# hmetaxa/MVTopicModel

Hardware: AMD Instinct MI355X
Metric: gibbs_tokens_per_sec (higher is better)
Workload: dtype f64

## Files before the change

### include/mvhdp.h

```cpp
#ifndef MVHDP_H
#define MVHDP_H

#include <stddef.h>
#include <stdint.h>

#ifdef __cplusplus
extern "C" {
#endif

#define MVHDP_MAX_MODALITIES 8
#define MVHDP_MAX_TOPICS     2048
#define MVHDP_UNASSIGNED_TOPIC (-1)

typedef enum {
    MVHDP_OK = 0,
    MVHDP_ERR_INVALID_ARG   = -1,
    MVHDP_ERR_STATE         = -2,
    MVHDP_ERR_HIP           = -3,
    MVHDP_ERR_NO_DEVICE     = -4,
    MVHDP_ERR_NEGATIVE_COUNT= -5,
    MVHDP_ERR_UNSUPPORTED   = -6
} mvhdp_status;

typedef struct mvhdp_ctx* mvhdp_handle;
// ... 26 lines not shown
    int64_t word_ftree_mass_cnt;
    int64_t oov_skipped;
    int64_t aborted_docs;
    int64_t exact_fallbacks;
    int32_t activated_topic;
    int32_t activated_modality;
    int64_t activation_key;
    double  sweep_kernel_ms;
    double  total_ms;
    int32_t activations;
    int32_t reserved;
} mvhdp_sweep_stats;

#define MVHDP_ACT_DOC_SHIFT   34
#define MVHDP_ACT_VIEW_SHIFT  31
#define MVHDP_ACT_POS_SHIFT   11
#define MVHDP_ACT_TOPIC_MASK  0x7ffLL
#define MVHDP_ACT_VIEW_MASK   0x7LL
#define MVHDP_ACT_KEY(doc, view, pos, topic) \
    (((int64_t)(doc) << MVHDP_ACT_DOC_SHIFT) | ((int64_t)(view) << MVHDP_ACT_VIEW_SHIFT) | ((int64_t)(pos) << MVHDP_ACT_POS_SHIFT) | (int64_t)(topic))
#define MVHDP_ACT_KEY_TOPIC(key) ((int32_t)((key) & MVHDP_ACT_TOPIC_MASK))
#define MVHDP_ACT_KEY_VIEW(key)  ((int32_t)(((key) >> MVHDP_ACT_VIEW_SHIFT) & MVHDP_ACT_VIEW_MASK))
#define MVHDP_ACT_KEY_NONE INT64_MAX

typedef struct {
    double* tok_dbg[MVHDP_MAX_MODALITIES];
    int32_t n_trace;
    const int64_t* trace_doc;
    const int32_t* trace_view;
    const int32_t* trace_pos;
    double* trace_out;
} mvhdp_debug;

#define MVHDP_SWEEP_REUSE_TREES 0x1u
#define MVHDP_SWEEP_NO_APPLY    0x2u
#define MVHDP_SWEEP_EXACT_CHAIN 0x4u
#define MVHDP_SWEEP_GENERIC_KERNEL 0x8u
#define MVHDP_SWEEP_FROZEN      0x10u

#define MVHDP_SWEEP_LIVE        0x20u
#define MVHDP_SWEEP_LIVE_SEGMENTS(n) (((uint32_t)(n) & 0xffu) << 16)

#define MVHDP_SWEEP_SEGMENT_APPLY 0x40u

#define MVHDP_SWEEP_SEGMENT_OVERLAP 0x80u

#define MVHDP_SWEEP_ONLY_SEGMENT(s) ((((uint32_t)(s) + 1u) & 0xffu) << 24)

#define MVHDP_SWEEP_SHARD_BIRTHS 0x200u

typedef enum {
    MVHDP_BUF_COUNTS = 0,
    MVHDP_BUF_DELTA  = 1,
    MVHDP_BUF_BIRTH_KEYS = 2
} mvhdp_buffer;

int mvhdp_create(const mvhdp_config* cfg, mvhdp_handle* out);
int mvhdp_destroy(mvhdp_handle h);
const char* mvhdp_last_error(mvhdp_handle h);
const char* mvhdp_version(void);

int mvhdp_set_corpus(mvhdp_handle h, int32_t m, int64_t num_docs,
                     const int64_t* doc_off , const int32_t* tokens );
int mvhdp_set_assignments(mvhdp_handle h, int32_t m, const int32_t* z );
int mvhdp_set_view_presence(mvhdp_handle h, int32_t m, const uint8_t* present );
int mvhdp_get_assignments(mvhdp_handle h, int32_t m, int32_t* z );

int mvhdp_set_hyper(mvhdp_handle h, const mvhdp_hyper* hy);
int mvhdp_get_alpha(mvhdp_handle h, double* alpha , uint8_t* inactive );
int mvhdp_build_counts(mvhdp_handle h);
int mvhdp_build_trees(mvhdp_handle h);
int mvhdp_build_inference_trees(mvhdp_handle h);
int mvhdp_init_assignments_from_trees(mvhdp_handle h, uint64_t seed);
int mvhdp_get_counts(mvhdp_handle h, int32_t m, int32_t* n_wk , int32_t* n_k );
int mvhdp_set_counts(mvhdp_handle h, int32_t m, const int32_t* n_wk, const int32_t* n_k);
int mvhdp_get_tree(mvhdp_handle h, int32_t m, int32_t type, double* tree );
int mvhdp_get_doc_topic_hist(mvhdp_handle h, int32_t m, int32_t* hist , int32_t hist_len,
                             int32_t* doc_len_counts , int32_t len_len);

int mvhdp_get_count_histogram(mvhdp_handle h, int32_t m, int32_t* hist, int32_t len);
int mvhdp_view_overlap_sums(mvhdp_handle h, double* sums );
int mvhdp_model_log_likelihood(mvhdp_handle h, double* log_likelihood );
int mvhdp_gamma_doc_statistics(mvhdp_handle h, int32_t m, double gamma_m, uint64_t seed, uint32_t round, double* qs, double* qw);
int mvhdp_dp_table_statistics(mvhdp_handle h, int32_t m, const int32_t* hist , int32_t hist_len, const double* conc ,
                              uint64_t seed, uint32_t round, double* mk , uint8_t* active );
int mvhdp_antoniak_draws(mvhdp_handle h, int32_t n, const int32_t* items , const double* conc , uint64_t seed, uint32_t round, int32_t* tables );
int mvhdp_doc_topic_proportions(mvhdp_handle h, const double* view_weights , int64_t d0, int64_t d1, double* out );

#define MVHDP_DIAG_MAX_TOP_WORDS 64
#define MVHDP_DIAG_PROPORTIONS   7
#define MVHDP_DIAG_TOKENS             0
#define MVHDP_DIAG_DOCUMENT_ENTROPY   1
#define MVHDP_DIAG_WORD_LENGTH        2
#define MVHDP_DIAG_COHERENCE          3
#define MVHDP_DIAG_NORM_DISCR_WEIGHT  4
#define MVHDP_DIAG_DISCR_WEIGHT       5
#define MVHDP_DIAG_UNIFORM_DIST       6
#define MVHDP_DIAG_CORPUS_DIST        7
#define MVHDP_DIAG_EFF_NUM_WORDS      8
#define MVHDP_DIAG_TOKEN_DOC_DIFF     9
#define MVHDP_DIAG_RANK_1_DOCS       10
#define MVHDP_DIAG_ALLOCATION_RATIO  11
#define MVHDP_DIAG_ALLOCATION_COUNT  12
#define MVHDP_DIAG_ROWS              13
typedef struct {
    int32_t num_top_words;
    const int32_t* word_length;
// ... 162 lines not shown
```

### mvtopicmodel_amd/csrc/mvhdp_api.hip

```cpp
#include "mvhdp_ctx.h"

static thread_local std::string g_create_error;

static std::mutex g_reg_mutex;
static std::set<mvhdp_ctx*>* g_live = nullptr;
static bool g_exiting = false, g_atexit_registered = false;
static void release_device_resources(mvhdp_ctx* h);

static void mvhdp_at_exit()
{
    std::lock_guard<std::mutex> lk(g_reg_mutex);
    g_exiting = true;
    if (g_live) for (mvhdp_ctx* h : *g_live) release_device_resources(h);
}

static void register_handle(mvhdp_ctx* h)
{
    std::lock_guard<std::mutex> lk(g_reg_mutex);
    if (!g_live) g_live = new std::set<mvhdp_ctx*>();
    g_live->insert(h);
    if (!g_atexit_registered) { atexit(mvhdp_at_exit); g_atexit_registered = true; }
}

bool mvhdp_is_live(mvhdp_ctx* h)
{
    std::lock_guard<std::mutex> lk(g_reg_mutex);
    return g_live && g_live->count(h) != 0;
}

static void read_environment(mvhdp_ctx* h)
{
    if (const char* f = getenv("MVHDP_FORCE_RMAX")) { const int v = atoi(f); if (v == 1 || v == 2 || v == 4 || v == 8 || v == 16 || v == 32) h->tu.force_primary = v; }
    if (const char* f = getenv("MVHDP_NARROW")) h->tu.narrow = atoi(f) != 0 ? -1 : 0;
    if (const char* f = getenv("MVHDP_SINGLE_STREAM")) h->tu.single_stream = atoi(f) != 0;
    if (const char* f = getenv("MVHDP_SIDE_PRIORITY")) h->side_priority = atoi(f);
    if (const char* f = getenv("MVHDP_LIVE16")) h->tu.live16 = atoi(f);
    if (const char* f = getenv("MVHDP_LIVE_OVERLAP")) h->tu.live_overlap = atoi(f);
    if (const char* f = getenv("MVHDP_LIVE_ROWS")) h->tu.live_rows = atoi(f);
    if (const char* f = getenv("MVHDP_LIVE_ROWS_THETA")) h->tu.live_rows_theta = atof(f);
    if (const char* f = getenv("MVHDP_COEF_LDS_KB")) h->tu.coef_lds_max_bytes = std::max(0, std::min(64, atoi(f))) * 1024;
    if (const char* f = getenv("MVHDP_LIVE_ROWS_SEGMENTS")) h->tu.live_rows_segments = std::max(1, std::min(255, atoi(f)));
    if (const char* f = getenv("MVHDP_WIDEST_ON_MAIN")) h->tu.widest_on_main = atoi(f) != 0;
    if (const char* f = getenv("MVHDP_NARROW_WIDE")) h->tu.narrow_wide = atoi(f) != 0;
    if (const char* f = getenv("MVHDP_LIVE_TREE_EVERY")) h->live_tree_every = std::max(1, atoi(f));
    if (const char* f = getenv("MVHDP_GATE_PCT")) { const int v = atoi(f); if (v >= 5 && v <= 95) h->gate_pct = v; }
    if (const char* f = getenv("MVHDP_FOUR_ROUND_ON_C")) h->tu.four_round_on_c = atoi(f);
    if (const char* f = getenv("MVHDP_DELTA16")) h->tu.delta16 = atoi(f) != 0;
    if (const char* f = getenv("MVHDP_FORK_DELAY_US")) h->tu.fork_delay_us = std::max(0, std::min(1000, atoi(f)));
    if (const char* f = getenv("MVHDP_FORCE_MODE")) { if (!strcmp(f, "serial")) h->tu.single_stream = 1; }
    if (const char* f = getenv("MVHDP_PRIMARY_MIN_SHARE")) { const double v = atof(f); if (v > 0.0 && v <= 1.0) h->tu.primary_min_share = v; }
    if (const char* t = getenv("MVHDP_WALK_THETA")) {
        int m = 0;
        for (const char* q = t; *q && m < MVHDP_MAXM; m++) {
            h->tu.walk_theta[m] = atof(q);
            while (*q && *q != ',') q++;
            if (*q == ',') q++;
        }
        for (; m < MVHDP_MAXM; m++) h->tu.walk_theta[m] = 0.0;
        h->tu.walk_fixed = 1;
    }
    h->dbg_env = getenv("MVHDP_DEBUG") != nullptr;
}

extern "C" const char* mvhdp_version(void) { return "mvhdp 0.1 (gfx950)"; }

extern "C" const char* mvhdp_last_error(mvhdp_handle h) { return (h && mvhdp_is_live(h)) ? h->err.c_str() : g_create_error.c_str(); }

extern "C" int mvhdp_create(const mvhdp_config* cfg, mvhdp_handle* out)
{
    if (!cfg || !out) { g_create_error = "null argument"; return MVHDP_ERR_INVALID_ARG; }
    *out = nullptr;
    const int K = cfg->num_topics, M = cfg->num_modalities;
    if (K < 1 || K > MVHDP_MAX_TOPICS || M < 1 || M > MVHDP_MAX_MODALITIES) {
        g_create_error = "num_topics must be in [1,2048] and num_modalities in [1,8]";
        return MVHDP_ERR_INVALID_ARG;
    }
    for (int m = 0; m < M; m++) if (cfg->num_types[m] < 1) { g_create_error = "num_types[m] must be >= 1"; return MVHDP_ERR_INVALID_ARG; }
    for (int m = 0; m < M; m++) if (cfg->num_types[m] >= (1 << 29)) { g_create_error = "num_types[m] must be below 2^29"; return MVHDP_ERR_INVALID_ARG; }
    if (cfg->doc_id_base < 0 || cfg->doc_id_base >= (1LL << 29)) { g_create_error = "doc_id_base out of range"; return MVHDP_ERR_INVALID_ARG; }
    int ndev = 0;
    if (hipGetDeviceCount(&ndev) != hipSuccess || ndev <= 0 || cfg->device < 0 || cfg->device >= ndev) {
        g_create_error = "no usable HIP device (the sweep has no CPU fallback)";
        return MVHDP_ERR_NO_DEVICE;
    }
    hipDeviceProp_t prop;
    if (hipGetDeviceProperties(&prop, cfg->device) != hipSuccess) { g_create_error = "hipGetDeviceProperties failed"; return MVHDP_ERR_HIP; }
    if (strncmp(prop.gcnArchName, "gfx950", 6) != 0) {
        g_create_error = std::string("device is ") + prop.gcnArchName + ", this library is built for gfx950 only";
        return MVHDP_ERR_NO_DEVICE;
    }
    mvhdp_ctx* h = new mvhdp_ctx();
    register_handle(h);
    h->cfg = *cfg;
    h->device = cfg->device;
    h->num_cus = prop.multiProcessorCount;
    h->max_lds = 160 * 1024;
// ... 10 lines not shown
    CREATE_HIP(hipStreamCreateWithFlags(&h->stream, hipStreamNonBlocking));
    h->own_stream = true;
    for (auto& e : h->ev) CREATE_HIP(hipEventCreate(&e));
    const int64_t nrows = mm.rowbase[M];
    const size_t cbytes = (size_t)(nrows * K + (int64_t)M * K + MVHDP_TAIL_WORDS) * sizeof(int32_t);
    CREATE_HIP(hipMalloc(&mm.counts, cbytes));
    CREATE_HIP(hipMalloc(&mm.delta, cbytes));
    CREATE_HIP(hipMemset(mm.counts, 0, cbytes));
    CREATE_HIP(hipMalloc(&mm.counts16, (size_t)nrows * K * sizeof(uint16_t) + 64));
    CREATE_HIP(hipMemset(mm.counts16, 0, (size_t)nrows * K * sizeof(uint16_t)));
    CREATE_HIP(hipMalloc(&mm.delta16, (size_t)(nrows * K + 2) * sizeof(uint16_t)));
    CREATE_HIP(hipMemsetD16(mm.delta16, (unsigned short)0x8000, (size_t)(nrows * K + 2)));
    CREATE_HIP(hipMalloc(&mm.heavy, (size_t)nrows));
    CREATE_HIP(hipMemset(mm.heavy, 1, (size_t)nrows));
    CREATE_HIP(hipMemset(mm.delta, 0, cbytes));
    CREATE_HIP(hipMalloc(&mm.trees, (size_t)nrows * 2 * K * sizeof(double)));
    CREATE_HIP(hipMalloc(&mm.root, (size_t)nrows * sizeof(double)));
    CREATE_HIP(hipMalloc(&mm.mass0, (size_t)nrows * sizeof(float)));
    CREATE_HIP(hipMemset(mm.mass0, 0, (size_t)nrows * sizeof(float)));
    CREATE_HIP(hipMalloc(&mm.coef, (size_t)M * (((K + 7) & ~7) + K + 8) * sizeof(float)));
    {
        const int nlev = (K > 1) ? (32 - __builtin_clz((unsigned)(K - 1))) : 0;
        mm.dt_f = nlev ? ((nlev - 1) % 3) + 1 : 0;
        mm.dt_nbd = 1; mm.dt_base[0] = 0; mm.dt_depth[0] = 0;
        int nblk = 1;
        for (int dep = mm.dt_f; nlev && dep < nlev; dep += 3) {
            mm.dt_base[mm.dt_nbd] = nblk; mm.dt_depth[mm.dt_nbd] = dep; mm.dt_nbd++;
            nblk += 1 << dep;
        }
        mm.dt_nblk = nblk;
        CREATE_HIP(hipMalloc(&mm.dtab, (size_t)nrows * nblk * 8 * sizeof(double)));
    }
    CREATE_HIP(hipMalloc(&h->d_alpha, (size_t)M * (K + 1) * sizeof(double)));
    CREATE_HIP(hipMalloc(&h->d_inactive, (size_t)K));
    CREATE_HIP(hipMemset(h->d_inactive, 0, (size_t)K));
    CREATE_HIP(hipMalloc(&h->d_births, (size_t)(2 + 2 * K) * sizeof(int32_t)));
    CREATE_HIP(hipMemset(h->d_births, 0, (size_t)(2 + 2 * K) * sizeof(int32_t)));
    CREATE_HIP(hipMalloc(&h->d_birth_keys, (size_t)K * sizeof(long long)));
    CREATE_HIP(hipMalloc(&h->d_birth_table, (size_t)K * sizeof(long long)));
    {
        const std::vector<long long> none((size_t)K, LLONG_MAX);
        CREATE_HIP(hipMemcpy(h->d_birth_table, none.data(), (size_t)K * sizeof(long long), hipMemcpyHostToDevice));
    }
    CREATE_HIP(hipMalloc(&h->d_ctl, CTL_WORDS * sizeof(unsigned long long)));
    CREATE_HIP(hipMemset(h->d_ctl, 0, CTL_WORDS * sizeof(unsigned long long)));
    h->d_stats = h->d_ctl;
    h->d_act_key = (long long*)(h->d_ctl + ST_COUNT);
    h->d_ovf_meta = (unsigned int*)(h->d_ctl + ST_COUNT + 1);
    h->d_doc_counter = h->d_ctl + ST_COUNT + 1 + META_WORDS64;
    CREATE_HIP(hipHostMalloc((void**)&h->h_ctl, CTL_WORDS * sizeof(unsigned long long), hipHostMallocDefault));
    for (int c = 0; c < MVHDP_N_CLASSES; c++)
        for (int f = 0; f < 3; f++) { h->regs.regs[c][f] = mvhdp_sweep_kernel_regs(c, f); h->regs.regs_mix[c][f] = mvhdp_sweep_kernel_regs(c, f ? f : 1, true); }
    read_environment(h);
    mm.alpha = h->d_alpha;
    mm.inactive = h->d_inactive;
    h->h_alpha.assign((size_t)M * (K + 1), 0.0);
    h->h_inactive.assign((size_t)K, 0);
    h->wt.init_defaults(K);
    h->wt_mix.init_defaults(K);
    *out = h;
    return MVHDP_OK;
}

static void release_device_resources(mvhdp_ctx* h)
{
    if (h->device_released) return;
    h->device_released = true;
    hipSetDevice(h->device);
    if (h->stream) hipStreamSynchronize(h->stream);
    auto fr = [](auto*& p) { if (p) { hipFree((void*)p); p = nullptr; } };
    for (int m = 0; m < MVHDP_MAXM; m++) { fr(h->d_doc_off[m]); fr(h->d_tok[m]); fr(h->d_z[m]); fr(h->d_carry[m]); fr(h->d_present[m]); }
    fr(h->mm.counts); fr(h->mm.delta16); fr(h->mm.counts16); fr(h->mm.heavy); fr(h->mm.delta); fr(h->mm.trees); fr(h->mm.root); fr(h->mm.coef); fr(h->mm.mass0); fr(h->d_births); fr(h->d_birth_keys); fr(h->d_birth_table); fr(h->mm.dtab); fr(h->mm.p);
    fr(h->d_alpha); fr(h->d_inactive); fr(h->d_ctl);
    fr(h->d_mix); fr(h->d_mix32); h->mm.mix = nullptr; h->mm.mix32 = nullptr; h->mix_lambda = 0.0;
    mvhdp_emb_free(h);
    if (h->h_ctl) { hipHostFree(h->h_ctl); h->h_ctl = nullptr; }
    h->d_stats = nullptr; h->d_act_key = nullptr; h->d_doc_counter = nullptr; h->d_ovf_meta = nullptr;
    fr(h->d_doc_order); fr(h->d_lists); fr(h->d_nslots); fr(h->d_stats_many); fr(h->d_heavy_list); fr(h->d_heavy_ctl);
    if (h->ev_rf_go) { hipEventDestroy(h->ev_rf_go); h->ev_rf_go = nullptr; }
    if (h->ev_rf_done) { hipEventDestroy(h->ev_rf_done); h->ev_rf_done = nullptr; }
    if (h->rf_stream) { hipStreamDestroy(h->rf_stream); h->rf_stream = nullptr; }
    fr(h->ov.counts2); fr(h->ov.counts16_2); fr(h->ov.dtab2); fr(h->ov.root2); fr(h->ov.trees2); fr(h->ov.delta2); fr(h->ov.delta3); fr(h->ov.ctl2); fr(h->ov.lists2);
    for (auto& e : h->ov.ev_seg) if (e) { hipEventDestroy(e); e = nullptr; }
    if (h->ov.ev_start) { hipEventDestroy(h->ov.ev_start); h->ov.ev_start = nullptr; }
    if (h->ov.x1) { hipStreamDestroy(h->ov.x1); h->ov.x1 = nullptr; }
    if (h->ov.xa) { hipStreamDestroy(h->ov.xa); h->ov.xa = nullptr; }
    for (auto& e : h->ev_many) if (e) { hipEventDestroy(e); e = nullptr; }
    for (auto& e : h->ev) if (e) { hipEventDestroy(e); e = nullptr; }
    if (h->ev_fork) { hipEventDestroy(h->ev_fork); h->ev_fork = nullptr; }
    for (auto& e : h->ev_join) if (e) { hipEventDestroy(e); e = nullptr; }
    for (auto& st : h->side) if (st) { hipStreamDestroy(st); st = nullptr; }
    if (h->own_stream && h->stream) hipStreamDestroy(h->stream);
    h->stream = nullptr;
}

extern "C" int mvhdp_destroy(mvhdp_handle h)
{
    if (!h) return MVHDP_OK;
    bool exiting;
    {
        std::lock_guard<std::mutex> lk(g_reg_mutex);
        if (!g_live || g_live->erase(h) == 0) return MVHDP_ERR_INVALID_ARG;
        exiting = g_exiting;
    }
    if (!exiting) release_device_resources(h);
    delete h;
    return MVHDP_OK;
}

extern "C" int mvhdp_set_stream(mvhdp_handle h, void* hip_stream)
{
    CHECK_H(h);
    HIPC(h, hipSetDevice(h->device));
    HIPC(h, hipStreamSynchronize(h->stream));
    if (h->own_stream) { hipStreamDestroy(h->stream); h->own_stream = false; }
    if (hip_stream) h->stream = (hipStream_t)hip_stream;
    else { HIPC(h, hipStreamCreateWithFlags(&h->stream, hipStreamNonBlocking)); h->own_stream = true; }
    return MVHDP_OK;
}

extern "C" int mvhdp_synchronize(mvhdp_handle h)
{
    CHECK_H(h);
    HIPC(h, hipSetDevice(h->device));
    HIPC(h, hipStreamSynchronize(h->stream));
// ... 497 lines not shown
    if (activated_topic >= 0) {
        h->have_trees = false;
        int rc = apply_activation(h, activated_topic, activated_modality);
        if (rc) return rc;
    }
    if (neg) FAIL(h, MVHDP_ERR_NEGATIVE_COUNT, "a topic count went below zero (UPD:202-215)");
    return MVHDP_OK;
}

extern "C" int mvhdp_trees_current(mvhdp_handle h)
{
    CHECK_H(h);
    return h->have_trees ? 1 : 0;
}

static int ensure_slot_counts(mvhdp_ctx* h)
{
    MvModel& mm = h->mm;
    if (mm.D > 0 && !h->d_nslots) {
        HIPC(h, hipMalloc(&h->d_nslots, (size_t)mm.D * sizeof(uint16_t)));
        mm.nslots = h->d_nslots;
        h->nslots_valid = false;
    }
    if (h->nslots_valid) return MVHDP_OK;
    unsigned long long hist[MVHDP_HIST_BINS + MVHDP_ENT_BINS] = {0};
    HIPC(h, hipMemsetAsync(h->d_ovf_meta, 0, META_BYTES, h->stream));
    HIPC(h, mvhdp_launch_slot_hist(mm, (unsigned long long*)h->d_ovf_meta + META_HIST, h->stream));
    HIPC(h, hipMemcpyAsync(hist, (unsigned long long*)h->d_ovf_meta + META_HIST, sizeof hist, hipMemcpyDeviceToHost, h->stream));
    HIPC(h, hipStreamSynchronize(h->stream));
    std::copy(hist, hist + MVHDP_HIST_BINS, h->last_hist);
    std::copy(hist + MVHDP_HIST_BINS, hist + MVHDP_HIST_BINS + MVHDP_ENT_BINS, h->last_ent);
    h->nslots_valid = true;
    return MVHDP_OK;
}

static void fill_plan_in(mvhdp_ctx* h, uint32_t flags, bool debug, bool batch, PlanIn& in)
{
    const MvModel& mm = h->mm;
    in.K = mm.K; in.M = mm.M; in.D = mm.D;
    in.mdt = compute_max_doc_tokens(h);
    in.have_order = h->d_doc_order != nullptr && !h->tokens_desc.empty();
    for (int c = 0; c < 5; c++)
        in.n_longer[c] = in.have_order ? (int64_t)(std::upper_bound(h->tokens_desc.begin(), h->tokens_desc.end(), (int64_t)64 << c, std::greater<int64_t>()) - h->tokens_desc.begin()) : mm.D;
    std::copy(h->last_hist, h->last_hist + MVHDP_HIST_BINS, in.tok_hist);
    std::copy(h->last_ent, h->last_ent + MVHDP_ENT_BINS, in.ent_hist);
    in.flags = flags; in.debug = debug; in.batch = batch;
    in.trees_current = h->have_trees;
    in.unassigned = false;
    for (int m = 0; m < mm.M; m++) in.unassigned = in.unassigned || h->unassigned[m];
    in.first_inactive = mm.first_inactive;
    in.vectors_mix = mm.mix != nullptr && !(flags & MVHDP_SWEEP_FROZEN);
    in.num_cus = h->num_cus; in.max_lds = h->max_lds;
    in.regs = h->regs;
}

static int alloc_debug(mvhdp_ctx* h, const mvhdp_debug* dbg, DebugBufs& db)
{
    const int K = h->mm.K, M = h->mm.M;
    hipStream_t s = h->stream;
    for (int m = 0; m < M; m++) {
        if (dbg->tok_dbg[m] && h->N[m] > 0) {
            void* p = nullptr;
            hipError_t e = hipMalloc(&p, (size_t)h->N[m] * 4 * sizeof(double));
            if (e != hipSuccess) { db.release(); HIPC(h, e); }
            db.to_free.push_back(p);
            hipMemsetAsync(p, 0, (size_t)h->N[m] * 4 * sizeof(double), s);
            db.tok_dbg[m] = (double*)p;
        }
    }
    if (dbg->n_trace > 0) {
        void *a = nullptr, *b = nullptr, *c = nullptr, *o = nullptr;
        const size_t n = (size_t)dbg->n_trace;
        if (hipMalloc(&a, n * 8) != hipSuccess || hipMalloc(&b, n * 4) != hipSuccess ||
            hipMalloc(&c, n * 4) != hipSuccess || hipMalloc(&o, n * (K + 1) * 8) != hipSuccess) {
            for (void* q : {a, b, c, o}) if (q) hipFree(q);
            db.release(); FAIL(h, MVHDP_ERR_HIP, "debug trace allocation failed");
        }
        db.to_free.push_back(a); db.to_free.push_back(b); db.to_free.push_back(c); db.to_free.push_back(o);
        hipMemcpyAsync(a, dbg->trace_doc, n * 8, hipMemcpyHostToDevice, s);
        hipMemcpyAsync(b, dbg->trace_view, n * 4, hipMemcpyHostToDevice, s);
        hipMemcpyAsync(c, dbg->trace_pos, n * 4, hipMemcpyHostToDevice, s);
        hipMemsetAsync(o, 0, n * (K + 1) * 8, s);
        db.n_trace = dbg->n_trace;
        db.trace_doc = (const int64_t*)a; db.trace_view = (const int32_t*)b; db.trace_pos = (const int32_t*)c;
        db.trace_out = (double*)o;
    }
    return MVHDP_OK;
}

struct SegCtl {
    unsigned int* class_counts;
    unsigned long long* qheads;
    int32_t* lists;
};

static hipError_t launch_segment_kernels(mvhdp_ctx* h, const SweepPlan& p, const MvModel& mk_in, const SweepLaunch& sl, int seg, hipStream_t s,
                                         const SegCtl& ctl, unsigned long long* d_stats)
{
    const MvModel& mm = h->mm;
    MvModel mk = mk_in;
    if (p.frozen) { mk.mix = nullptr; mk.mix32 = nullptr; }
    const int nseg = p.nseg;
    hipError_t e = hipSuccess;
    auto step = [&](hipError_t r) { if (e == hipSuccess) e = r; };
    auto share = [&](int64_t P) -> int64_t { return P > seg ? (P - seg + nseg - 1) / nseg : 0; };
    const int64_t n_seg = share(mm.D);
// ... 412 lines not shown
}

static void learn_from_sweep(mvhdp_ctx* h, const SweepPlan& p, const unsigned long long* hs, const unsigned long long* meta_hist, double kernel_ms, bool comparable)
{
    const MvModel& mm = h->mm;
    bool any_walk = false;
    for (int c = 0; c < MVHDP_N_CLASSES; c++) any_walk = any_walk || (p.cls[c].used && p.cls[c].walk);
    WalkTuner& wt = walk_tuner_of(h, p.flags);
    if (any_walk) wt.measured(mm.M, p.nseg, hs + ST_VIEW_BASE);
    if (mm.D > 0 && p.only_seg >= 0) {
        if (meta_hist[MVHDP_HIST_BINS + MVHDP_N_CLASSES] != 0) h->nslots_valid = false;
    } else if (mm.D > 0) {
        std::copy(meta_hist, meta_hist + MVHDP_HIST_BINS, h->last_hist);
        std::copy(meta_hist + MVHDP_HIST_BINS, meta_hist + MVHDP_HIST_BINS + MVHDP_ENT_BINS, h->last_ent);
        h->nslots_valid = h->last_ent[MVHDP_N_CLASSES] == 0;
    }
    if (h->dbg_env) {
        fprintf(stderr, "[mvhdp] walk threshold %.2f (base %.2f, phase %d, dir %+d, group %d); tree branch %.4f of tokens, walked on demand %.4f; per view tree share:",
                (double)wt.walk_probe_i / MVHDP_WALK_BINS, (double)wt.walk_i / MVHDP_WALK_BINS, wt.walk_phase, wt.walk_dir, wt.walk_cls,
                (double)hs[ST_TREE] / std::max<double>(1.0, (double)hs[ST_TOKENS]), (double)hs[ST_ONDEMAND] / std::max<double>(1.0, (double)hs[ST_TOKENS]));
        for (int m = 0; m < mm.M; m++) {
            const double n = std::max<double>(1.0, (double)hs[ST_VIEW_BASE + m * MVHDP_VIEW_STATS]);
            fprintf(stderr, " %.3f", hs[ST_VIEW_BASE + m * MVHDP_VIEW_STATS + 1] / n);
        }
        fprintf(stderr, "\n");
        if (hs[ST_T_TOTAL])
            fprintf(stderr, "[mvhdp] wave cycles: queue %.1f%% prologue %.1f%% view setup %.1f%% chunk head %.1f%% tokens %.1f%% chunk end %.1f%% | %.0f cycles per token per wave\n",
                    100.0 * hs[ST_T_QUEUE] / hs[ST_T_TOTAL], 100.0 * hs[ST_T_PROLOGUE] / hs[ST_T_TOTAL], 100.0 * hs[ST_T_VIEW] / hs[ST_T_TOTAL],
                    100.0 * hs[ST_T_CHUNK_HEAD] / hs[ST_T_TOTAL], 100.0 * hs[ST_T_TOKENS] / hs[ST_T_TOTAL], 100.0 * hs[ST_T_CHUNK_END] / hs[ST_T_TOTAL],
                    (double)hs[ST_T_TOTAL] / std::max<double>(1.0, (double)hs[ST_TOKENS]));
        if (hs[ST_T_ROWS])
            fprintf(stderr, "[mvhdp] live rows: %.0f cycles per tree-branch token, %.0f of them until the row is there (%.1f%% of the waves' time; %llu such tokens)\n",
                    (double)hs[ST_T_ROWS] / std::max<double>(1.0, (double)hs[ST_ONDEMAND]), (double)hs[ST_T_ROWS_WAIT] / std::max<double>(1.0, (double)hs[ST_ONDEMAND]),
                    100.0 * hs[ST_T_ROWS] / hs[ST_T_TOTAL], hs[ST_ONDEMAND]);
        if (hs[ST_N_WAVES])
            fprintf(stderr, "[mvhdp] cycles per token in a wave's first / second / later entities: %.0f / %.0f / %.0f (tokens %llu / %llu / %llu); per wave: block init %.0f cycles, wait + flush at the end %.0f, whole wave %.0f\n",
                    (double)hs[ST_T_ENT0] / std::max<double>(1.0, (double)hs[ST_N_ENT0]), (double)hs[ST_T_ENT1] / std::max<double>(1.0, (double)hs[ST_N_ENT1]),
                    (double)hs[ST_T_ENT2] / std::max<double>(1.0, (double)hs[ST_N_ENT2]), hs[ST_N_ENT0], hs[ST_N_ENT1], hs[ST_N_ENT2],
                    (double)hs[ST_T_INIT] / hs[ST_N_WAVES], (double)hs[ST_T_FLUSH] / hs[ST_N_WAVES], (double)hs[ST_T_TOTAL] / hs[ST_N_WAVES]);
    }
    const double tokens = (double)hs[ST_TOKENS];
    wt.observe(comparable && tokens > 0, p.walk_cfg, mm.M, tokens > 0 ? kernel_ms * 1e6 / tokens : 0.0);
}

static void debug_print_plan(const mvhdp_ctx* h, const SweepPlan& p, uint32_t sweep_idx)
{
    double tot = 0, b1 = 0, b2 = 0;
    for (int b = 0; b < MVHDP_HIST_BINS; b++) { tot += (double)h->last_hist[b]; if (b < 1) b1 += (double)h->last_hist[b]; if (b < 2) b2 += (double)h->last_hist[b]; }
    fprintf(stderr, "[mvhdp] sweep %u: %s primary class %d, routed prefix %lld, S_cap %d, %d segment(s); tokens in lists <=64: %.4f <=128: %.4f; kernels:",
            sweep_idx, p.fast ? "register-resident" : "generic", p.pc, (long long)p.H, p.S_cap, p.nseg, b1 / std::max(1.0, tot), b2 / std::max(1.0, tot));
    for (int c = 0; c < MVHDP_N_CLASSES; c++)
        if (p.cls[c].used)
            fprintf(stderr, " [class %d %s grid %d wpb %d lds %zu stream %d%s%s theta0 %.2f ents %llu]", c, p.cls[c].fast ? "fast" : "generic", p.cls[c].grid, p.cls[c].wpb, p.cls[c].lds,
                    p.cls[c].stream, p.cls[c].walk ? " walk" : "", p.cls[c].narrow ? " narrow" : "", p.cls[c].theta[0], (unsigned long long)h->last_ent[c]);
    fprintf(stderr, "\n");
}

static int sweep_preconditions(mvhdp_ctx* h, uint32_t flags)
{
    if ((flags & MVHDP_SWEEP_SHARD_BIRTHS) && (!(flags & MVHDP_SWEEP_LIVE) || (flags & MVHDP_SWEEP_FROZEN) || (flags >> 24) != 0))
        FAIL(h, MVHDP_ERR_INVALID_ARG, "sweep: SHARD_BIRTHS goes with LIVE, not with FROZEN or ONLY_SEGMENT");
    int rc = require_corpus(h); if (rc) return rc;
    if (!h->have_hyper) FAIL(h, MVHDP_ERR_STATE, "sweep before set_hyper");
    if (!h->have_counts) FAIL(h, MVHDP_ERR_STATE, "sweep before build_counts/set_counts");
    if ((flags & (MVHDP_SWEEP_REUSE_TREES | MVHDP_SWEEP_FROZEN)) && !h->have_trees) FAIL(h, MVHDP_ERR_STATE, "REUSE_TREES / FROZEN without trees");
    if (h->rows_applied >= 0) FAIL(h, MVHDP_ERR_STATE, "sweep: an mvhdp_apply_delta_begin bracket is open (call mvhdp_apply_delta_end)");
    if (h->delta_pending && !(flags & MVHDP_SWEEP_FROZEN))
        FAIL(h, MVHDP_ERR_STATE, "sweep: the previous NO_APPLY sweep's deltas have not been applied (mvhdp_apply_delta)");
    if (h->counts_stale && !(flags & MVHDP_SWEEP_FROZEN))
        FAIL(h, MVHDP_ERR_STATE, "sweep: the assignments were replaced after the counts were built (call mvhdp_build_counts, mvhdp_set_counts or mvhdp_counts_written first)");
    return MVHDP_OK;
}

static int set_generic_lds(mvhdp_ctx* h, const SweepPlan& p)
{
    size_t lds = 0;
    for (int c = 0; c < MVHDP_N_CLASSES; c++) if (p.cls[c].used && !p.cls[c].fast) lds = std::max(lds, p.cls[c].lds);
    if (lds > 65536 && lds > h->lds_attr_set) { HIPC(h, mvhdp_sweep_set_max_lds(lds)); h->lds_attr_set = lds; }
    return MVHDP_OK;
}

int mvhdp_sweep_begin(mvhdp_ctx* h, uint32_t sweep_idx, uint64_t seed, uint32_t flags, const double* p_override, const mvhdp_debug* dbg, PendingSweep& ps)
{
    int rc = sweep_preconditions(h, flags); if (rc) return rc;
    HIPC(h, hipSetDevice(h->device));
    hipStream_t s = h->stream;
    rc = ensure_slot_counts(h); if (rc) return rc;
    ps.flags = flags; ps.dbg = dbg; ps.debug = dbg != nullptr; ps.oc = SweepOutcome();
    PlanIn in; fill_plan_in(h, flags, ps.debug, false, in);
    plan_sweep(in, h->tu, walk_tuner_of(h, flags), ps.p);
    if (ps.p.err) FAIL(h, ps.p.err, ps.p.msg);
    rc = set_generic_lds(h, ps.p); if (rc) return rc;
    if (h->dbg_env) debug_print_plan(h, ps.p, sweep_idx);
    if (ps.debug) { rc = alloc_debug(h, dbg, ps.db); if (rc) return rc; }
    HIPC(h, hipEventRecord(h->ev[0], s));
    ps.births = sweep_births(ps.p, flags, h->mm);
    rc = enqueue_sweep(h, ps.p, sweep_idx, seed, p_override, ps.debug ? &ps.db : nullptr, h->d_stats, h->ev[1], h->ev[2], ps.oc);
    if (rc) { ps.db.release(); return rc; }
    if ((flags & MVHDP_SWEEP_NO_APPLY) && !ps.p.frozen) {
        hipError_t e = mvhdp_launch_birth_table(ps.births ? h->d_births : nullptr, h->d_birth_keys, h->d_act_key, h->mm.K, h->d_birth_table, s);
        if (e != hipSuccess) { ps.db.release(); HIPC(h, e); }
    }
    hipError_t e = hipMemcpyAsync(h->h_ctl, h->d_ctl, (ST_COUNT + 1 + META_WORDS64) * sizeof(unsigned long long), hipMemcpyDeviceToHost, s);
    if (e != hipSuccess) { ps.db.release(); HIPC(h, e); }
    ps.open = true;
    return MVHDP_OK;
}
// ... 159 lines not shown
    return ret;
}

extern "C" int mvhdp_get_tuning(mvhdp_handle h, mvhdp_tuning* t)
{
    CHECK_H(h);
    if (!t) FAIL(h, MVHDP_ERR_INVALID_ARG, "get_tuning: null");
    memset(t, 0, sizeof *t);
    t->force_primary = h->tu.force_primary; t->narrow = h->tu.narrow; t->walk_fixed = h->tu.walk_fixed;
    t->single_stream = h->tu.single_stream; t->primary_min_share = h->tu.primary_min_share; t->live16 = h->tu.live16;
    t->single_wave = h->tu.single_wave; t->live_overlap = h->tu.live_overlap; t->live_rows = h->tu.live_rows;
    for (int m = 0; m < MVHDP_MAX_MODALITIES; m++) { t->walk_theta[m] = h->tu.walk_theta[m]; t->tree_branch_share[m] = h->wt.walk_f[m]; }
    for (int g = 0; g < WALK_GROUPS; g++) t->learnt_walk_step[g] = g == h->wt.walk_cls ? h->wt.walk_i : h->wt.walk_i_by[g];
    t->learnt_walk_step[3] = -1;
    return MVHDP_OK;
}

extern "C" int mvhdp_set_tuning(mvhdp_handle h, const mvhdp_tuning* t)
{
    CHECK_H(h);
    if (!t) FAIL(h, MVHDP_ERR_INVALID_ARG, "set_tuning: null");
    const int fp = t->force_primary;
    if (!(fp == 0 || fp == 1 || fp == 2 || fp == 4 || fp == 8 || fp == 16 || fp == 32)) FAIL(h, MVHDP_ERR_INVALID_ARG, "set_tuning: force_primary must be 0, 1, 2, 4, 8, 16 or 32");
    if (t->primary_min_share < 0.0 || t->primary_min_share > 1.0) FAIL(h, MVHDP_ERR_INVALID_ARG, "set_tuning: primary_min_share outside [0, 1]");
    for (int g = 0; g < WALK_GROUPS; g++) if (t->learnt_walk_step[g] < -1 || t->learnt_walk_step[g] > MVHDP_WALK_BINS) FAIL(h, MVHDP_ERR_INVALID_ARG, "set_tuning: learnt_walk_step outside [-1, 20]");
    h->tu.force_primary = fp; h->tu.narrow = t->narrow; h->tu.walk_fixed = t->walk_fixed ? 1 : 0;
    h->tu.single_stream = t->single_stream ? 1 : 0;
    h->tu.live16 = t->live16 < 0 ? -1 : (t->live16 ? 1 : 0);
    h->tu.single_wave = t->single_wave ? 1 : 0;
    h->tu.live_overlap = t->live_overlap < 0 ? -1 : (t->live_overlap ? 1 : 0);
    h->tu.live_rows = t->live_rows < 0 ? -1 : (t->live_rows ? 1 : 0);
    h->tu.primary_min_share = t->primary_min_share > 0.0 ? t->primary_min_share : 0.10;
    for (int m = 0; m < MVHDP_MAX_MODALITIES; m++) h->tu.walk_theta[m] = t->walk_theta[m];
    if (t->learnt_walk_step[0] >= 0 || t->learnt_walk_step[1] >= 0 || t->learnt_walk_step[2] >= 0) h->wt.restore(t->learnt_walk_step, t->tree_branch_share, h->mm.M);
    return MVHDP_OK;
}

extern "C" int mvhdp_plan_probe(const mvhdp_plan_input* pi, const mvhdp_tuning* t, mvhdp_plan_output* po)
{
    if (!pi || !po) return MVHDP_ERR_INVALID_ARG;
    PlanIn in;
    in.K = pi->num_topics; in.M = pi->num_modalities; in.D = pi->num_entities; in.mdt = pi->max_entity_tokens;
    if (in.K < 1 || in.K > MVHDP_MAX_TOPICS || in.M < 1 || in.M > MVHDP_MAX_MODALITIES || in.D < 0) return MVHDP_ERR_INVALID_ARG;
    in.have_order = true;
    for (int c = 0; c < 5; c++) in.n_longer[c] = pi->entities_longer_than[c];
    for (int b = 0; b < MVHDP_HIST_BINS; b++) in.tok_hist[b] = pi->tokens_by_list_rounds[b];
    for (int b = 0; b < MVHDP_ENT_BINS; b++) in.ent_hist[b] = pi->entities_by_class[b];
    in.flags = pi->flags; in.debug = pi->debug != 0; in.batch = pi->batch != 0; in.trees_current = pi->trees_current != 0;
    in.first_inactive = pi->inactive_topics ? 0 : -1;
    in.num_cus = pi->num_cus > 0 ? pi->num_cus : 256;
    for (int c = 0; c < MVHDP_N_CLASSES; c++) for (int f = 0; f < 3; f++) in.regs.regs[c][f] = pi->kernel_registers[c][f];
    for (int c = 0; c < MVHDP_N_CLASSES; c++) for (int f = 0; f < 3; f++) in.regs.regs_mix[c][f] = pi->kernel_registers_mix[c][f] > 0 ? pi->kernel_registers_mix[c][f] : pi->kernel_registers[c][f];
    in.vectors_mix = pi->vectors_mix != 0 && !(pi->flags & MVHDP_SWEEP_FROZEN);
    PlanTuning tu;
    WalkTuner wt;
    wt.init_defaults(in.K);
    if (t) {
        tu.force_primary = t->force_primary; tu.narrow = t->narrow; tu.walk_fixed = t->walk_fixed; tu.single_stream = t->single_stream;
        tu.live16 = t->live16; tu.single_wave = t->single_wave ? 1 : 0; tu.live_overlap = t->live_overlap; tu.live_rows = t->live_rows;
        if (t->primary_min_share > 0) tu.primary_min_share = t->primary_min_share;
        for (int m = 0; m < MVHDP_MAX_MODALITIES; m++) tu.walk_theta[m] = t->walk_theta[m];
        if (t->learnt_walk_step[0] >= 0 || t->learnt_walk_step[1] >= 0 || t->learnt_walk_step[2] >= 0) wt.restore(t->learnt_walk_step, t->tree_branch_share, in.M);
    }
    SweepPlan p;
    plan_sweep(in, tu, wt, p);
    memset(po, 0, sizeof *po);
    po->status = p.err;
    if (p.err) return MVHDP_OK;
    po->segments = p.nseg; po->primary_class = p.pc; po->routed_prefix = p.H; po->register_resident = p.fast ? 1 : 0;
    po->need_full_trees = p.need_full ? 1 : 0; po->dominant_class = p.dominant;
    for (int c = 0; c < MVHDP_N_CLASSES; c++) {
        po->class_used[c] = p.cls[c].used ? 1 : 0; po->class_map[c] = p.class_map[c];
        po->class_stream[c] = p.cls[c].stream; po->class_grid[c] = p.cls[c].grid; po->class_lds_bytes[c] = (int64_t)p.cls[c].lds;
        po->class_walk[c] = p.cls[c].walk; po->class_narrow[c] = p.cls[c].narrow; po->class_register_resident[c] = p.cls[c].fast ? 1 : 0;
        po->class_theta0[c] = p.cls[c].theta[0];
    }
    po->delta16 = p.delta16 ? 1 : 0;
    po->live_rows = p.live_rows ? 1 : 0;
    return MVHDP_OK;
}

extern "C" int mvhdp_tuner_probe(int32_t num_modalities, const double* tree_branch_share, const double* u1_hist, const double* ns_by_step ,
                                 int32_t n_sweeps, int32_t group, int32_t* steps_out )
{
    if (!tree_branch_share || !ns_by_step || !steps_out || num_modalities < 1 || num_modalities > MVHDP_MAX_MODALITIES || n_sweeps < 0) return MVHDP_ERR_INVALID_ARG;
    WalkTuner wt;
    if (group < 0 || group >= WALK_GROUPS) return MVHDP_ERR_INVALID_ARG;
    for (int m = 0; m < num_modalities; m++) wt.walk_f[m] = tree_branch_share[m];
    for (int b = 0; b < MVHDP_WALK_BINS; b++) wt.walk_hist[b] = u1_hist ? u1_hist[b] : 0.0;
    for (int i = 0; i < n_sweeps; i++) {
        double theta[WALK_GROUPS][MVHDP_MAXM]; bool measure;
        wt.propose(group, num_modalities, theta, &measure);
        steps_out[i] = wt.walk_probe_i;
        wt.observe(true, 1, num_modalities, ns_by_step[std::max(0, std::min(MVHDP_WALK_BINS, wt.walk_probe_i))]);
    }
    return MVHDP_OK;
}

extern "C" int mvhdp_get_view_weights(mvhdp_handle h, double* p)
{
    CHECK_H(h);
    MvModel& mm = h->mm;
    if (!p) FAIL(h, MVHDP_ERR_INVALID_ARG, "get_view_weights: null");
    if (mm.M == 1) { for (int64_t d = 0; d < mm.D; d++) p[d] = 1.0; return MVHDP_OK; }
    if (!mm.p) FAIL(h, MVHDP_ERR_STATE, "get_view_weights before the first sweep");
    HIPC(h, hipSetDevice(h->device));
    HIPC(h, hipStreamSynchronize(h->stream));
    HIPC(h, hipMemcpy(p, mm.p, (size_t)mm.D * mm.M * mm.M * sizeof(double), hipMemcpyDeviceToHost));
    return MVHDP_OK;
}

extern "C" int mvhdp_device_buffer(mvhdp_handle h, mvhdp_buffer which, void** dev_ptr, size_t* bytes)
{
    CHECK_H(h);
    if (!dev_ptr || !bytes) FAIL(h, MVHDP_ERR_INVALID_ARG, "device_buffer: null");
    size_t b = (size_t)counts_len(h) * sizeof(int32_t);
    if (which == MVHDP_BUF_COUNTS) { *dev_ptr = h->mm.counts; *bytes = b; return MVHDP_OK; }
    if (which == MVHDP_BUF_DELTA) { *dev_ptr = h->mm.delta; *bytes = b; return MVHDP_OK; }
    if (which == MVHDP_BUF_BIRTH_KEYS) { *dev_ptr = h->d_birth_table; *bytes = (size_t)h->mm.K * sizeof(long long); return MVHDP_OK; }
    FAIL(h, MVHDP_ERR_INVALID_ARG, "device_buffer: unknown buffer");
}

extern "C" int mvhdp_counts_written(mvhdp_handle h)
{
    CHECK_H(h);
    h->have_counts = true; h->have_trees = false; h->counts_stale = false;
    return MVHDP_OK;
}

static double log_gamma_stirling_host(double z)
{
    const double HALF_LOG_TWO_PI = std::log(6.283185307179586) / 2.0;
    int shift = 0;
    while (z < 2.0) { z = z + 1; shift++; }
    double result = HALF_LOG_TWO_PI + (z - 0.5) * std::log(z) - z + 1 / (12.0 * z) - 1 / (360.0 * z * z * z)
                    + 1 / (1260.0 * z * z * z * z * z);
    while (shift > 0) { shift--; z = z - 1; result = result - std::log(z); }
    return result;
}

extern "C" int mvhdp_get_count_histogram(mvhdp_handle h, int32_t m, int32_t* hist, int32_t len)
{
    CHECK_H(h);
    MvModel& mm = h->mm;
    if (m < 0 || m >= mm.M || !hist || len < 1) FAIL(h, MVHDP_ERR_INVALID_ARG, "get_count_histogram: bad argument");
    if (!h->have_counts) FAIL(h, MVHDP_ERR_STATE, "get_count_histogram before build_counts/set_counts");
    HIPC(h, hipSetDevice(h->device));
    int32_t* d = nullptr;
    HIPC(h, hipMalloc(&d, (size_t)len * sizeof(int32_t)));
    hipError_t e = mvhdp_launch_count_hist(mm, m, d, len, h->stream);
    if (e == hipSuccess) e = hipMemcpyAsync(hist, d, (size_t)len * sizeof(int32_t), hipMemcpyDeviceToHost, h->stream);
    if (e == hipSuccess) e = hipStreamSynchronize(h->stream);
    hipFree(d);
    HIPC(h, e);
    return MVHDP_OK;
}

int mvhdp_view_overlap_accumulate(mvhdp_ctx* h, double* acc)
{
    MvModel& mm = h->mm;
    int rc = require_corpus(h); if (rc) return rc;
    const int M = mm.M;
    if (mm.D == 0) return MVHDP_OK;
    HIPC(h, hipSetDevice(h->device));
    double* d = nullptr;
    const size_t n = (size_t)M * M * mm.D;
    HIPC(h, hipMalloc(&d, n * sizeof(double)));
    std::vector<double> host(n);
    hipError_t e = mvhdp_launch_view_overlap(mm, d, h->stream);
    if (e == hipSuccess) e = hipMemcpyAsync(host.data(), d, n * sizeof(double), hipMemcpyDeviceToHost, h->stream);
    if (e == hipSuccess) e = hipStreamSynchronize(h->stream);
    hipFree(d);
    HIPC(h, e);
// ... 206 lines not shown
```

### mvtopicmodel_amd/csrc/mvhdp_device.h

```cpp
#pragma once
#include <hip/hip_runtime.h>
#include <stdint.h>

#define MVHDP_MAXM 8
#define MVHDP_WALK_BINS 20
#define MVHDP_VIEW_STATS (2 + MVHDP_WALK_BINS)

struct MvModel {
    int32_t K, M;
    int32_t V[MVHDP_MAXM];
    int64_t rowbase[MVHDP_MAXM + 1];
    int64_t D;
    int64_t doc_id_base;
    const int64_t* doc_off[MVHDP_MAXM];
    const int32_t* tok[MVHDP_MAXM];
    int32_t* z[MVHDP_MAXM];
    const uint8_t* present[MVHDP_MAXM];
    uint16_t* nslots;
    int32_t* counts;
    uint16_t* delta16;
    uint16_t* counts16;
    uint8_t* heavy;
    int32_t* delta;
    double* trees;
    double* root;
    float* coef;
    float* mass0;
    double* dtab;
    int32_t dt_nblk, dt_nbd, dt_f;
    int32_t dt_base[6], dt_depth[6];
    const double* alpha;
    const uint8_t* inactive;
    double alpha_sum[MVHDP_MAXM], beta[MVHDP_MAXM], beta_sum[MVHDP_MAXM], gamma[MVHDP_MAXM];
    double p_a[MVHDP_MAXM][MVHDP_MAXM], p_b[MVHDP_MAXM][MVHDP_MAXM];
    double* p;
    int32_t first_inactive;
    const double* mix;
    const float* mix32;
    double oml;
};

#define MVHDP_SL_STRICT_LIVE 0x8000u
#define MVHDP_ROW_HEAVY 1
#define MVHDP_ROW_BIG 2

struct SweepLaunch {
    uint32_t sweep_idx;
    uint32_t seed_lo, seed_hi;
    uint32_t flags;
    int32_t  S_cap;
    int32_t  waves_per_block;
    uint32_t block_shared_bytes;
    int32_t  nk_global;
    uint32_t wave_bytes;
    unsigned long long* stats;
    long long* act_key;
    int32_t* births;
    long long* birth_keys;
    unsigned long long* doc_counter;
    const int32_t* q_list;
    const unsigned int* q_list_count;
    const int32_t* q_order;
    int64_t q_order_start, q_order_count, q_order_stride;
    double walk_theta[MVHDP_MAXM];
    int32_t walk;
    int32_t narrow;
    int32_t delta16;
    int32_t live16;
    int32_t live_rows;
    int32_t coef_lds;
    unsigned long long* slot_hist;
    double* tok_dbg[MVHDP_MAXM];
    int32_t n_trace;
    const int64_t* trace_doc; const int32_t* trace_view; const int32_t* trace_pos;
    double* trace_out;
};

enum {
    ST_TOKENS = 0, ST_CHANGED, ST_NEW, ST_DOC, ST_TREE, ST_OOV, ST_ABORT, ST_FALLBACK, ST_NEGATIVE, ST_MISCLASS, ST_ONDEMAND,
    ST_VIEW_BASE, ST_VIEW_LAST = ST_VIEW_BASE + MVHDP_VIEW_STATS * MVHDP_MAXM - 1,
    ST_T_QUEUE, ST_T_PROLOGUE, ST_T_VIEW, ST_T_CHUNK_HEAD, ST_T_TOKENS, ST_T_CHUNK_END, ST_T_TOTAL,
    ST_T_ENT0, ST_T_ENT1, ST_T_ENT2, ST_N_ENT0, ST_N_ENT1, ST_N_ENT2, ST_T_INIT, ST_T_FLUSH, ST_N_WAVES, ST_T_ROWS, ST_T_ROWS_WAIT,
    ST_COUNT
};

size_t mvhdp_sweep_wave_bytes(int M, int S_cap);

hipError_t mvhdp_launch_build_counts(const MvModel& mm, const int64_t* n_tokens_per_view, hipStream_t s);
hipError_t mvhdp_launch_build_trees(const MvModel& mm, bool inference_leaves, bool write_full, hipStream_t s, bool beside_samplers = false);
hipError_t mvhdp_launch_build_trees_rows(const MvModel& mm, bool inference_leaves, bool write_full, int64_t row_begin, int64_t row_end,
                                         bool apply_first, unsigned long long* negatives, hipStream_t s);
hipError_t mvhdp_launch_build_trees_from_mirror(const MvModel& mm, bool write_full, hipStream_t s, bool beside_samplers = false);
hipError_t mvhdp_launch_widen_mirror(const MvModel& mm, hipStream_t s);
hipError_t mvhdp_launch_live_rows_prepare(const MvModel& mm, bool from_mirror, bool with_heavy_trees, int32_t* heavy_list, unsigned int* heavy_ctl, int heavy_cap, int batch_cells, hipStream_t s);
hipError_t mvhdp_launch_heavy_refresh(const MvModel& mm, const int32_t* heavy_list, const unsigned int* ctl, int heavy_cap, int blocks, hipStream_t s);
hipError_t mvhdp_launch_set_u32(unsigned int* p, unsigned int v, hipStream_t s);
hipError_t mvhdp_launch_apply_nk(const MvModel& mm, unsigned long long* negatives, hipStream_t s);
// ... 119 lines not shown
```

### mvtopicmodel_amd/csrc/mvhdp_group.hip

```cpp
#include "mvhdp_ctx.h"

#include <dlfcn.h>
#include <rccl/rccl.h>

#include <map>

namespace {

struct Rccl {
    void* lib = nullptr;
    std::string path, why;
    ncclResult_t (*GetVersion)(int*) = nullptr;
    ncclResult_t (*GetUniqueId)(ncclUniqueId*) = nullptr;
    ncclResult_t (*CommInitRank)(ncclComm_t*, int, ncclUniqueId, int) = nullptr;
    ncclResult_t (*CommInitAll)(ncclComm_t*, int, const int*) = nullptr;
    ncclResult_t (*CommDestroy)(ncclComm_t) = nullptr;
    ncclResult_t (*AllReduce)(const void*, void*, size_t, ncclDataType_t, ncclRedOp_t, ncclComm_t, hipStream_t) = nullptr;
    ncclResult_t (*GroupStart)() = nullptr;
    ncclResult_t (*GroupEnd)() = nullptr;
    const char* (*GetErrorString)(ncclResult_t) = nullptr;
};

std::mutex g_rccl_mutex;
Rccl g_rccl;
// ... 18 lines not shown
        if (g_rccl.lib) break;
        void* l = dlopen(n.c_str(), RTLD_NOW | RTLD_LOCAL);
        if (!l) { errs += std::string(dlerror() ? dlerror() : "?") + "; "; continue; }
        g_rccl.lib = l; g_rccl.path = n;
    }
    if (!g_rccl.lib) { g_rccl.why = "RCCL could not be opened: " + errs; return nullptr; }
#define SYM(field, name) do { *(void**)(&g_rccl.field) = dlsym(g_rccl.lib, name); \
        if (!g_rccl.field) { g_rccl.why = std::string("RCCL lacks ") + name; dlclose(g_rccl.lib); g_rccl.lib = nullptr; return nullptr; } } while (0)
    SYM(GetVersion, "ncclGetVersion"); SYM(GetUniqueId, "ncclGetUniqueId"); SYM(CommInitRank, "ncclCommInitRank");
    SYM(CommInitAll, "ncclCommInitAll"); SYM(CommDestroy, "ncclCommDestroy"); SYM(AllReduce, "ncclAllReduce");
    SYM(GroupStart, "ncclGroupStart"); SYM(GroupEnd, "ncclGroupEnd"); SYM(GetErrorString, "ncclGetErrorString");
#undef SYM
    return &g_rccl;
}

__global__ __launch_bounds__(256) void add_into_kernel(int32_t* __restrict__ dst, const int32_t* __restrict__ src, int64_t n)
{
    const int64_t stride = (int64_t)gridDim.x * blockDim.x;
    for (int64_t i = (int64_t)blockIdx.x * blockDim.x + threadIdx.x; i < n; i += stride) dst[i] += src[i];
}

hipError_t launch_add_into(int32_t* dst, const int32_t* src, int64_t n, hipStream_t s)
{
    int grid = (int)std::min<int64_t>((n + 255) / 256, 8192);
    if (grid < 1) grid = 1;
    hipLaunchKernelGGL(add_into_kernel, dim3(grid), dim3(256), 0, s, dst, src, n);
    return hipGetLastError();
}

__global__ void set_word_kernel(int32_t* p, int32_t v) { *p = v; }

__global__ __launch_bounds__(256) void min_births_kernel(long long* __restrict__ dst, const long long* __restrict__ src, int K, int first)
{
    const int k = blockIdx.x * blockDim.x + threadIdx.x;
    if (k >= K) return;
    const long long v = src ? src[k] : 0x7fffffffffffffffLL;
    dst[k] = first ? v : (v < dst[k] ? v : dst[k]);
}

hipError_t launch_min_births(long long* dst, const long long* src, int K, bool first, hipStream_t s)
{
    hipLaunchKernelGGL(min_births_kernel, dim3((K + 255) / 256), dim3(256), 0, s, dst, src, K, first ? 1 : 0);
    return hipGetLastError();
}

__global__ __launch_bounds__(256) void pack_rows_kernel(const int32_t* __restrict__ delta, const uint8_t* __restrict__ heavy, const int64_t* __restrict__ woff,
                                                        int32_t* __restrict__ xp, int64_t r0, int64_t r1, int K)
{
    const int lane = threadIdx.x & 63;
    const int64_t wstride = (int64_t)gridDim.x * (blockDim.x >> 6);
    for (int64_t row = r0 + (int64_t)blockIdx.x * (blockDim.x >> 6) + (threadIdx.x >> 6); row < r1; row += wstride) {
        const int32_t* d = delta + row * K;
        int32_t* o = xp + woff[row];
        if (heavy[row] == 0) {
            const int nw = (K + 1) >> 1;
            for (int j = lane; j < nw; j += 64) { const int a = d[2 * j], b = (2 * j + 1 < K) ? d[2 * j + 1] : 0; o[j] = a + b * 65536; }
        } else for (int k = lane; k < K; k += 64) o[k] = d[k];
    }
}

__global__ __launch_bounds__(256) void unpack_rows_kernel(int32_t* __restrict__ delta, const uint8_t* __restrict__ heavy, const int64_t* __restrict__ woff,
                                                          const int32_t* __restrict__ xp, int64_t r0, int64_t r1, int K)
{
    const int lane = threadIdx.x & 63;
    const int64_t wstride = (int64_t)gridDim.x * (blockDim.x >> 6);
    for (int64_t row = r0 + (int64_t)blockIdx.x * (blockDim.x >> 6) + (threadIdx.x >> 6); row < r1; row += wstride) {
        int32_t* d = delta + row * K;
        const int32_t* o = xp + woff[row];
        if (heavy[row] == 0) {
            const int nw = (K + 1) >> 1;
            for (int j = lane; j < nw; j += 64) {
                const int w = o[j];
                const int a = (int)(short)(w & 0xffff);
                d[2 * j] = a;
                if (2 * j + 1 < K) d[2 * j + 1] = (w - a) >> 16;
            }
        } else for (int k = lane; k < K; k += 64) d[k] = o[k];
    }
}

__global__ __launch_bounds__(256) void add_remote_kernel(int32_t* __restrict__ counts, const int32_t* __restrict__ sum, const int32_t* __restrict__ own, int64_t n)
{
    const int64_t stride = (int64_t)gridDim.x * blockDim.x;
    for (int64_t i = (int64_t)blockIdx.x * blockDim.x + threadIdx.x; i < n; i += stride) { const int d = sum[i] - own[i]; if (d) counts[i] += d; }
}

struct DeviceGuard {
    int prev = -1;
    DeviceGuard() { if (hipGetDevice(&prev) != hipSuccess) prev = -1; }
    ~DeviceGuard() { if (prev >= 0) hipSetDevice(prev); }
};

}

enum { XSCRATCH_BYTES = 1 << 20 };

struct mvhdp_group_ctx {
    std::vector<mvhdp_ctx*> members;
    std::vector<int> leader_of;
    std::vector<int> leaders;
    std::vector<ncclComm_t> comms;
    std::vector<hipEvent_t> ev_swept;
    std::vector<hipEvent_t> ev_reduced;
    std::vector<long long*> d_key;
    std::vector<long long*> d_btab;
    hipEvent_t ev_x0 = nullptr, ev_x1 = nullptr;
    int nranks = 1, rank0 = 0;
    bool multi_process = false;
    bool rccl_used = false;
    int rccl_version = 0;
    int chunks = 4;
    double last_exchange_ms = 0.0;
    long long sweeps = 0;
    std::vector<int32_t*> xbuf, sbuf;
    std::vector<hipStream_t> comm;
    std::vector<hipEvent_t> ev_xfer;
    bool async_pending = false;
    bool abort_raised = false;
    std::vector<int> by_entity;
    bool pack_on = false;
    bool pack_ready = false;
    bool pack_allowed = true;
// ... 268 lines not shown
        if (li == i) continue;
        mvhdp_ctx *h = g->members[i], *L = g->members[li];
        x.hip(hipSetDevice(L->device), "hipSetDevice");
        x.hip(hipStreamWaitEvent(L->stream, g->ev_swept[i], 0), "hipStreamWaitEvent");
        x.hip(launch_add_into(counts ? L->mm.counts : L->mm.delta, counts ? h->mm.counts : h->mm.delta, counts_len_of(L), L->stream), "add_into_kernel");
    }
    return x.rc;
}

static int allreduce_range(mvhdp_group_ctx* g, bool counts, int64_t e0, int64_t e1)
{
    if (e1 <= e0 || g->comms.empty()) return MVHDP_OK;
    XErr x{g};
    leaders_allreduce(g, x, (size_t)(e1 - e0), ncclInt32, ncclSum, "ncclAllReduce", [&](size_t l) {
        mvhdp_ctx* L = g->members[g->leaders[l]];
        return (counts ? L->mm.counts : L->mm.delta) + e0;
    });
    return x.rc;
}

static int fan_out_range(mvhdp_group_ctx* g, bool counts, int64_t e0, int64_t e1)
{
    if (e1 <= e0 || g->members.size() == g->leaders.size()) return MVHDP_OK;
    XErr x{g};
    for (size_t l = 0; l < g->leaders.size(); l++) {
        mvhdp_ctx* L = g->members[g->leaders[l]];
        x.hip(hipSetDevice(L->device), "hipSetDevice");
        x.hip(hipEventRecord(g->ev_reduced[l], L->stream), "hipEventRecord");
        for (size_t i = 0; i < g->members.size(); i++) {
            if (g->leader_of[i] != g->leaders[l] || (int)i == g->leaders[l]) continue;
            mvhdp_ctx* h = g->members[i];
            x.hip(hipStreamWaitEvent(h->stream, g->ev_reduced[l], 0), "hipStreamWaitEvent");
            const int32_t* src = (counts ? L->mm.counts : L->mm.delta) + e0;
            int32_t* dst = (counts ? h->mm.counts : h->mm.delta) + e0;
            x.hip(hipMemcpyAsync(dst, src, (size_t)(e1 - e0) * sizeof(int32_t), hipMemcpyDeviceToDevice, h->stream), "hipMemcpyAsync");
            x.hip(hipEventRecord(g->ev_swept[i], h->stream), "hipEventRecord");
            x.hip(hipStreamWaitEvent(L->stream, g->ev_swept[i], 0), "hipStreamWaitEvent");
        }
    }
    return x.rc;
}

static int pack_prepare(mvhdp_group_ctx* g)
{
    if (g->pack_ready || !g->pack_allowed) return MVHDP_OK;
    for (mvhdp_ctx* h : g->members) for (int m = 0; m < h->mm.M; m++) if (h->unassigned[m]) return MVHDP_OK;
    mvhdp_ctx* L0 = g->members[g->leaders[0]];
    const int64_t rows = L0->mm.rowbase[L0->mm.M];
    const int K = L0->mm.K;
    if (rows <= 0) return MVHDP_OK;
    std::vector<uint8_t> cls((size_t)rows);
    GHIP(g, hipSetDevice(L0->device));
    GHIP(g, hipMemcpy(cls.data(), L0->mm.heavy, (size_t)rows, hipMemcpyDeviceToHost));
    g->woff.assign((size_t)rows + 1, 0);
    for (int64_t r = 0; r < rows; r++) g->woff[(size_t)r + 1] = g->woff[(size_t)r] + (cls[(size_t)r] == 0 ? (K + 1) / 2 : K);
    if (g->d_woff.empty()) { g->d_woff.assign(g->leaders.size(), nullptr); g->d_cls.assign(g->leaders.size(), nullptr); g->xpack.assign(g->leaders.size(), nullptr); }
    for (size_t l = 0; l < g->leaders.size(); l++) {
        mvhdp_ctx* L = g->members[g->leaders[l]];
        GHIP(g, hipSetDevice(L->device));
        if (!g->d_woff[l]) GHIP(g, hipMalloc(&g->d_woff[l], (size_t)(rows + 1) * sizeof(int64_t)));
        if (!g->d_cls[l]) GHIP(g, hipMalloc(&g->d_cls[l], (size_t)rows));
        if (!g->xpack[l]) GHIP(g, hipMalloc(&g->xpack[l], (size_t)rows * K * sizeof(int32_t)));
        GHIP(g, hipMemcpy(g->d_woff[l], g->woff.data(), (size_t)(rows + 1) * sizeof(int64_t), hipMemcpyHostToDevice));
        GHIP(g, hipMemcpy(g->d_cls[l], cls.data(), (size_t)rows, hipMemcpyHostToDevice));
    }
    g->pack_hash = (int32_t)(g->woff[(size_t)rows] % 4091) + 1;
    g->pack_ready = true;
    return MVHDP_OK;
}

static void pack_reset(mvhdp_group_ctx* g) { g->pack_on = false; g->pack_ready = false; g->pack_hash = 0; g->sweeps_since_counts = 0; }

static int allreduce_rows_packed(mvhdp_group_ctx* g, int64_t r0, int64_t r1)
{
    XErr x{g};
    const int64_t w0 = g->woff[(size_t)r0], w1 = g->woff[(size_t)r1];
    const int K = g->members[0]->mm.K;
    const int grid = (int)std::min<int64_t>((r1 - r0 + 3) / 4, 8192);
    for (size_t l = 0; l < g->leaders.size(); l++) {
        mvhdp_ctx* L = g->members[g->leaders[l]];
        x.hip(hipSetDevice(L->device), "hipSetDevice");
        hipLaunchKernelGGL(pack_rows_kernel, dim3(std::max(grid, 1)), dim3(256), 0, L->stream, L->mm.delta, g->d_cls[l], g->d_woff[l], g->xpack[l], r0, r1, K);
        x.hip(hipGetLastError(), "pack_rows_kernel");
    }
    if (!g->comms.empty() && w1 > w0)
        leaders_allreduce(g, x, (size_t)(w1 - w0), ncclInt32, ncclSum, "ncclAllReduce", [&](size_t l) { return g->xpack[l] + w0; });
    for (size_t l = 0; l < g->leaders.size(); l++) {
        mvhdp_ctx* L = g->members[g->leaders[l]];
        x.hip(hipSetDevice(L->device), "hipSetDevice");
        hipLaunchKernelGGL(unpack_rows_kernel, dim3(std::max(grid, 1)), dim3(256), 0, L->stream, L->mm.delta, g->d_cls[l], g->d_woff[l], g->xpack[l], r0, r1, K);
        x.hip(hipGetLastError(), "unpack_rows_kernel");
    }
    g->last_exchange_bytes += (w1 - w0) * (long long)sizeof(int32_t);
    return x.rc;
}

extern "C" int mvhdp_group_build_counts(mvhdp_group g)
{
    CHECK_G(g);
    DeviceGuard dg;
    if (g->async_pending) {
        for (size_t l = 0; l < g->leaders.size(); l++) { hipSetDevice(g->members[g->leaders[l]]->device); hipStreamSynchronize(g->comm[l]); }
        g->async_pending = false;
    }
    const int n = (int)g->members.size();
    const int64_t len = counts_len_of(g->members[0]);
// ... 600 lines not shown
```

### mvtopicmodel_amd/csrc/mvhdp_kernels.hip

```cpp
#include "mvhdp_device.h"
#include "../../include/mvhdp.h"

#include "mvhdp_wave.h"
#include <algorithm>

__global__ __launch_bounds__(256) void build_counts_kernel(MvModel mm, int m, int64_t n_tokens)
{
    extern __shared__ int nk_local[];
    const int K = mm.K;
    for (int i = threadIdx.x; i < K; i += blockDim.x) nk_local[i] = 0;
    __syncthreads();
    int32_t* nwk = mm.counts;
    const int64_t stride = (int64_t)gridDim.x * blockDim.x;
    for (int64_t i = (int64_t)blockIdx.x * blockDim.x + threadIdx.x; i < n_tokens; i += stride) {
        int topic = mm.z[m][i];
        if (topic == MVHDP_UNASSIGNED_TOPIC) continue;
        int type = mm.tok[m][i];
        if (type < 0 || type >= mm.V[m] || topic < 0 || topic >= K) continue;
        atomicAdd(&nk_local[topic], 1);
        atomicAdd(&nwk[(mm.rowbase[m] + type) * K + topic], 1);
    }
    __syncthreads();
    int32_t* nk = mm.counts + mm.rowbase[mm.M] * K + (int64_t)m * K;
    for (int i = threadIdx.x; i < K; i += blockDim.x)
        if (nk_local[i]) atomicAdd(&nk[i], nk_local[i]);
}

hipError_t mvhdp_launch_build_counts(const MvModel& mm, const int64_t* n_tokens, hipStream_t s)
{
    const int K = mm.K;
    size_t total = (size_t)(mm.rowbase[mm.M] * K + (int64_t)mm.M * K) * sizeof(int32_t);
    hipError_t e = hipMemsetAsync(mm.counts, 0, total, s);
    if (e != hipSuccess) return e;
    for (int m = 0; m < mm.M; m++) {
        if (n_tokens[m] <= 0) continue;
        int64_t blocks = (n_tokens[m] + 255) / 256;
        int grid = (int)(blocks < 2048 ? blocks : 2048);
        hipLaunchKernelGGL(build_counts_kernel, dim3(grid), dim3(256), (size_t)K * sizeof(int), s, mm, m, n_tokens[m]);
        e = hipGetLastError();
        if (e != hipSuccess) return e;
    }
    return hipSuccess;
}

template <bool COHERENT = false>
__device__ __forceinline__ void tree_from_leaves(const MvModel& mm, int64_t row, double* t, int lane, bool write_full)
{
    const int K = mm.K;
    if (lane == 0) t[0] = 0.0;
    __syncthreads();
    if (K > 1) {
        int dmax = 31 - __clz(K - 1);
        for (int d = dmax; d >= 0; d--) {
            int lo = 1 << d, hi = min(2 << d, K);
            for (int i = lo + lane; i < hi; i += WAVE) t[i] = t[2 * i] + t[2 * i + 1];
            __syncthreads();
        }
    }
    if (write_full) {
        double* out = mm.trees + row * 2 * K;
        for (int i = lane; i < 2 * K; i += WAVE) out[i] = t[i];
    }
    if (lane == 0) { if (COHERENT) __hip_atomic_store(&mm.root[row], t[1], __ATOMIC_RELAXED, __HIP_MEMORY_SCOPE_AGENT); else mm.root[row] = t[1]; }
    double* dt = mm.dtab + row * (int64_t)mm.dt_nblk * 8;
    double2* o = (double2*)dt;
    for (int u = lane; u < mm.dt_nblk * 4; u += WAVE) {
        const int x = u >> 2, j = u & 3;
        int base = 0, dep = 0;
        if (x >= 1) {
            base = 1; dep = mm.dt_f;
            while (x >= base + (1 << dep)) { base += 1 << dep; dep += 3; }
        }
        const int b = (1 << dep) + (x - base);
        double v2[2];
#pragma unroll
        for (int h = 0; h < 2; h++) {
            const int q = 2 * j + h;
            const int node = (q == 0) ? b : (q < 3) ? 2 * b + (q - 1) : 4 * b + (q - 3);
            v2[h] = (q == 7) ? ((x == 0) ? t[1] : 0.0) : ((node < K) ? t[2 * node] : 0.0);
        }
        if (COHERENT) {
            __hip_atomic_store(&dt[2 * u], v2[0], __ATOMIC_RELAXED, __HIP_MEMORY_SCOPE_AGENT);
            __hip_atomic_store(&dt[2 * u + 1], v2[1], __ATOMIC_RELAXED, __HIP_MEMORY_SCOPE_AGENT);
        } else o[u] = make_double2(v2[0], v2[1]);
    }
    __syncthreads();
}

template <int TB, bool MIX = false>
__global__ __launch_bounds__(64) void build_trees_kernel(MvModel mm, bool inference_leaves, bool write_full, int64_t row_begin, int64_t row_end,
                                                         bool apply_first, unsigned long long* negatives, bool from_mirror, bool only_heavy = false)
{
    extern __shared__ double t[];
    const int K = mm.K, lane = threadIdx.x;
    const int64_t nrows = mm.rowbase[mm.M];
    const int32_t* nk_all = mm.counts + nrows * K;
    int neg = 0;
    __builtin_amdgcn_s_setprio(3);
    for (int64_t row = row_begin + blockIdx.x; row < row_end; row += gridDim.x) {
        if (only_heavy && mm.heavy[row] != MVHDP_ROW_HEAVY) continue;
        int m = 0;
        while (m + 1 < mm.M && row >= mm.rowbase[m + 1]) m++;
        int32_t* cnt = mm.counts + row * K;
        int32_t* dl = mm.delta + row * K;
        const int32_t* nk = nk_all + (int64_t)m * K;
        const double* al = mm.alpha + (int64_t)m * (K + 1);
        const double beta = mm.beta[m], beta_sum = mm.beta_sum[m], gamma = mm.gamma[m];
        uint16_t* c16 = mm.counts16 + row * K;
        const bool light_src = from_mirror && mm.heavy[row] != MVHDP_ROW_HEAVY;
        const bool mixed = MIX && m == 0 && !inference_leaves;
        const double* mixrow = mixed ? mm.mix + row * K : nullptr;
        bool hv = false;
        if (!from_mirror) {
            long long sum = 0;
            for (int k0 = 0; k0 < K; k0 += WAVE * TB) {
                int cv[TB], dv[TB];
#pragma unroll
                for (int u = 0; u < TB; u++) {
                    const int k = k0 + u * WAVE + lane;
                    cv[u] = (k < K) ? cnt[k] : 0;
                    dv[u] = (apply_first && k < K) ? dl[k] : 0;
                }
#pragma unroll
                for (int u = 0; u < TB; u++) {
                    const int k = k0 + u * WAVE + lane;
                    if (k < K) {
                        int c = cv[u];
                        if (apply_first) {
                            const int d = dv[u];
                            if (d) { c += d; cnt[k] = c; dl[k] = 0; neg += c < 0; }
                        }
                        sum += c < 0 ? 70000 : c;
                    }
                }
            }
#pragma unroll
            for (int sft = 32; sft >= 1; sft >>= 1) sum += __shfl_xor(sum, sft, WAVE);
            hv = sum > 65534;
            if (lane == 0) mm.heavy[row] = hv ? MVHDP_ROW_HEAVY : (sum > 32767 ? MVHDP_ROW_BIG : 0);
        }
        for (int k0 = 0; k0 < K; k0 += WAVE * TB) {
            int cv[TB], nkv[TB];
            double alv[TB], mxv[TB];
            bool inact[TB];
#pragma unroll
            for (int u = 0; u < TB; u++) {
                const int k = k0 + u * WAVE + lane;
                const bool in = k < K;
                mxv[u] = (MIX && mixed && in) ? mixrow[k] : 0.0;
                cv[u] = in ? (light_src ? (int)c16[k] : cnt[k]) : 0;
                nkv[u] = in ? nk[k] : 0;
                alv[u] = (in && !inference_leaves) ? al[k] : 0.0;
                inact[u] = in && !inference_leaves && mm.inactive[k];
            }
#pragma unroll
            for (int u = 0; u < TB; u++) {
                const int k = k0 + u * WAVE + lane;
                if (k < K) {
                    const int c = cv[u];
                    if (light_src) cnt[k] = c;
                    else if (!from_mirror) c16[k] = hv ? (uint16_t)65535 : (uint16_t)c;
                    double leaf;
                    if (inference_leaves) {
                        leaf = ((double)c + beta) / ((double)nkv[u] + beta_sum);
                    } else if (inact[u]) {
                        leaf = 0.0;
                    } else {
                        double p_wt = ((double)c + beta) / ((double)nkv[u] + beta_sum);
                        if (MIX && mixed) p_wt = mxv[u] + mm.oml * p_wt;
                        leaf = gamma * alv[u] * p_wt;
                    }
                    t[K + k] = leaf;
                }
            }
        }
        tree_from_leaves(mm, row, t, lane, write_full);
    }
    if (apply_first && negatives) {
#pragma unroll
        for (int sft = 32; sft >= 1; sft >>= 1) neg += __shfl_xor(neg, sft, WAVE);
        if (lane == 0 && neg) atomicAdd(negatives, (unsigned long long)neg);
    }
}

#define LAUNCH_TREES(TB, ...) do { if (mm.mix) hipLaunchKernelGGL((build_trees_kernel<TB, true>), __VA_ARGS__); \
                                   else hipLaunchKernelGGL((build_trees_kernel<TB, false>), __VA_ARGS__); } while (0)

hipError_t mvhdp_launch_build_trees(const MvModel& mm, bool inference_leaves, bool write_full, hipStream_t s, bool beside_samplers)
{
    if (!beside_samplers) return mvhdp_launch_build_trees_rows(mm, inference_leaves, write_full, 0, mm.rowbase[mm.M], false, nullptr, s);
    const int64_t nrows = mm.rowbase[mm.M];
    if (nrows <= 0) return hipSuccess;
    int grid = (int)(nrows < 65536 ? nrows : 65536);
    LAUNCH_TREES(1, dim3(grid), dim3(64), (size_t)2 * mm.K * sizeof(double), s, mm, inference_leaves, write_full,
                       (int64_t)0, nrows, false, (unsigned long long*)nullptr, false);
    return hipGetLastError();
}

hipError_t mvhdp_launch_build_trees_rows(const MvModel& mm, bool inference_leaves, bool write_full, int64_t row_begin, int64_t row_end,
                                         bool apply_first, unsigned long long* negatives, hipStream_t s)
{
    int64_t nrows = row_end - row_begin;
    if (nrows <= 0) return hipSuccess;
    int grid = (int)(nrows < 65536 ? nrows : 65536);
    if (mm.K > 512)
        LAUNCH_TREES(8, dim3(grid), dim3(64), (size_t)2 * mm.K * sizeof(double), s, mm, inference_leaves, write_full,
                           row_begin, row_end, apply_first, negatives, false);
    else
        LAUNCH_TREES(4, dim3(grid), dim3(64), (size_t)2 * mm.K * sizeof(double), s, mm, inference_leaves, write_full,
                           row_begin, row_end, apply_first, negatives, false);
    return hipGetLastError();
}

hipError_t mvhdp_launch_build_trees_from_mirror(const MvModel& mm, bool write_full, hipStream_t s, bool beside_samplers)
{
    const int64_t nrows = mm.rowbase[mm.M];
    if (nrows <= 0) return hipSuccess;
    int grid = (int)(nrows < 65536 ? nrows : 65536);
    if (beside_samplers)
        LAUNCH_TREES(1, dim3(grid), dim3(64), (size_t)2 * mm.K * sizeof(double), s, mm, false, write_full,
                           (int64_t)0, nrows, false, (unsigned long long*)nullptr, true);
    else if (mm.K > 512)
        LAUNCH_TREES(8, dim3(grid), dim3(64), (size_t)2 * mm.K * sizeof(double), s, mm, false, write_full,
                           (int64_t)0, nrows, false, (unsigned long long*)nullptr, true);
    else
        LAUNCH_TREES(4, dim3(grid), dim3(64), (size_t)2 * mm.K * sizeof(double), s, mm, false, write_full,
                           (int64_t)0, nrows, false, (unsigned long long*)nullptr, true);
    return hipGetLastError();
}

__global__ __launch_bounds__(256) void apply2_nk_kernel(int32_t* nk_dst, const int32_t* __restrict__ dA, int32_t* __restrict__ dB, int n, unsigned long long* negatives)
{
    const int i = blockIdx.x * blockDim.x + threadIdx.x;
    if (i >= n) return;
    int d = dA[i];
    if (dB) { const int d2 = dB[i]; if (d2) { d += d2; dB[i] = 0; } }
    if (d) { const int c = nk_dst[i] + d; nk_dst[i] = c; if (c < 0 && negatives) atomicAdd(negatives, 1ull); }
}

__global__ __launch_bounds__(256) void apply2_counts_kernel(MvModel mm, const int32_t* __restrict__ dA, int32_t* __restrict__ dB, bool use_mirror,
                                                           int64_t n_cells, int64_t n_all, unsigned long long* negatives)
{
    const int64_t stride = (int64_t)gridDim.x * blockDim.x;
    unsigned int* m32 = (unsigned int*)mm.counts16;
    const int K = mm.K;
    int neg = 0;
    __builtin_amdgcn_s_setprio(3);
    for (int64_t i = (int64_t)blockIdx.x * blockDim.x + threadIdx.x; i < n_all; i += stride) {
        int d = dA[i];
        if (dB) { const int d2 = dB[i]; if (d2) { d += d2; dB[i] = 0; } }
        if (!d) continue;
        const int old = __hip_atomic_fetch_add(&mm.counts[i], d, __ATOMIC_RELAXED, __HIP_MEMORY_SCOPE_AGENT);
        neg += old + d < 0;
        if (use_mirror && i < n_cells && mm.heavy[i / K] != MVHDP_ROW_HEAVY) __hip_atomic_fetch_add(&m32[i >> 1], (unsigned int)d << ((i & 1) * 16), __ATOMIC_RELAXED, __HIP_MEMORY_SCOPE_AGENT);
    }
    if (neg && negatives) atomicAdd(negatives, (unsigned long long)neg);
}

hipError_t mvhdp_launch_apply2_counts(const MvModel& dst, const int32_t* dA, int32_t* dB, bool use_mirror, unsigned long long* negatives, hipStream_t s)
{
    const int64_t cells = dst.rowbase[dst.M] * dst.K, all = cells + (int64_t)dst.M * dst.K;
    int grid = (int)std::min<int64_t>((all + 255) / 256, 4096);
    if (grid < 1) grid = 1;
    hipLaunchKernelGGL(apply2_counts_kernel, dim3(grid), dim3(256), 0, s, dst, dA, dB, use_mirror, cells, all, negatives);
    return hipGetLastError();
}

__global__ __launch_bounds__(256) void apply_sparse_kernel(MvModel mm, int32_t* __restrict__ d, bool use_mirror, int64_t n_cells, int64_t n_all)
{
    const int64_t stride = (int64_t)gridDim.x * blockDim.x;
    unsigned int* m32 = (unsigned int*)mm.counts16;
    const int K = mm.K;
    for (int64_t i = (int64_t)blockIdx.x * blockDim.x + threadIdx.x; i < n_all; i += stride) {
        const int dl = d[i];
        if (!dl) continue;
        mm.counts[i] += dl;
        d[i] = 0;
        if (use_mirror && i < n_cells && mm.heavy[i / K] != MVHDP_ROW_HEAVY) __hip_atomic_fetch_add(&m32[i >> 1], (unsigned int)dl << ((i & 1) * 16), __ATOMIC_RELAXED, __HIP_MEMORY_SCOPE_AGENT);
    }
}

hipError_t mvhdp_launch_apply_sparse(const MvModel& dst, int32_t* d, bool use_mirror, hipStream_t s)
{
    const int64_t cells = dst.rowbase[dst.M] * dst.K, all = cells + (int64_t)dst.M * dst.K;
    int grid = (int)std::min<int64_t>((all + 255) / 256, 8192);
    if (grid < 1) grid = 1;
    hipLaunchKernelGGL(apply_sparse_kernel, dim3(grid), dim3(256), 0, s, dst, d, use_mirror, cells, all);
    return hipGetLastError();
}

__global__ __launch_bounds__(64) void gate_kernel(const unsigned long long* qhead, unsigned long long threshold)
{
    const unsigned long long t0 = __builtin_amdgcn_s_memrealtime();
    for (int i = 0; i < 4000000; i++) {
        const unsigned long long v = __hip_atomic_load(qhead, __ATOMIC_RELAXED, __HIP_MEMORY_SCOPE_AGENT);
        if (v >= threshold) break;
        if (__builtin_amdgcn_s_memrealtime() - t0 > 200000000ull) break;
        __builtin_amdgcn_s_sleep(32);
    }
}

hipError_t mvhdp_launch_gate(const unsigned long long* qhead, unsigned long long threshold, hipStream_t s)
{
    hipLaunchKernelGGL(gate_kernel, dim3(1), dim3(64), 0, s, qhead, threshold);
    return hipGetLastError();
}

__global__ __launch_bounds__(256) void widen_mirror_kernel(MvModel mm)
{
    const int K = mm.K;
    const int64_t nrows = mm.rowbase[mm.M];
    const int lane = threadIdx.x & 63;
    const int64_t wstride = (int64_t)gridDim.x * (blockDim.x >> 6);
    for (int64_t row = (int64_t)blockIdx.x * (blockDim.x >> 6) + (threadIdx.x >> 6); row < nrows; row += wstride) {
        if (mm.heavy[row] == MVHDP_ROW_HEAVY) continue;
        const uint16_t* c16 = mm.counts16 + row * K;
        int32_t* cnt = mm.counts + row * K;
        for (int k = lane; k < K; k += WAVE) cnt[k] = (int)c16[k];
    }
}

hipError_t mvhdp_launch_widen_mirror(const MvModel& mm, hipStream_t s)
{
    const int64_t nrows = mm.rowbase[mm.M];
    if (nrows <= 0) return hipSuccess;
    int64_t blocks = (nrows + 3) / 4;
    hipLaunchKernelGGL(widen_mirror_kernel, dim3((unsigned int)(blocks < 16384 ? blocks : 16384)), dim3(256), 0, s, mm);
    return hipGetLastError();
}

__global__ __launch_bounds__(64) void live_coef_kernel(MvModel mm)
{
    const int K = mm.K, Kp = (K + 7) & ~7, m = blockIdx.x;
    const int32_t* nk = mm.counts + mm.rowbase[mm.M] * K + (int64_t)m * K;
    float* cf = mm.coef + (int64_t)m * Kp;
    float* smp = mm.coef + (int64_t)mm.M * Kp + (int64_t)m * K;
    for (int k = threadIdx.x; k < Kp; k += blockDim.x)
        cf[k] = (k >= K || mm.inactive[k]) ? 0.0f : (float)(mm.gamma[m] * mm.alpha[(int64_t)m * (K + 1) + k] / ((double)nk[k] + mm.beta_sum[m]));
    __syncthreads();
    if (threadIdx.x == 0) {
        const float beta32 = (float)mm.beta[m];
        float run = 0.0f;
        for (int k = 0; k < K; k++) { run += cf[k] * beta32; smp[k] = run; }
    }
}

template <int TB>
__global__ __launch_bounds__(64) void live_rows_prepare_kernel(MvModel mm, bool from_mirror, int32_t* heavy_list, unsigned int* heavy_n, int heavy_cap, int batch_cells)
{
    const int K = mm.K, lane = threadIdx.x;
    const int64_t nrows = mm.rowbase[mm.M];
    for (int64_t row = blockIdx.x; row < nrows; row += gridDim.x) {
        int m = 0;
        while (m + 1 < mm.M && row >= mm.rowbase[m + 1]) m++;
        const int32_t* cnt = mm.counts + row * K;
        uint16_t* c16 = mm.counts16 + row * K;
        const int Kp = (K + 7) & ~7;
        const float* cf = mm.coef + (int64_t)m * Kp;
        const float smp_total = mm.coef[(int64_t)mm.M * Kp + (int64_t)m * K + K - 1];
        const bool light_src = from_mirror && mm.heavy[row] != MVHDP_ROW_HEAVY;
        bool hv = false;
        if (!from_mirror) {
            long long sum = 0;
            for (int k0 = 0; k0 < K; k0 += WAVE * TB) {
                int cv[TB];
#pragma unroll
                for (int u = 0; u < TB; u++) { const int k = k0 + u * WAVE + lane; cv[u] = (k < K) ? cnt[k] : 0; }
#pragma unroll
                for (int u = 0; u < TB; u++) sum += cv[u] < 0 ? 70000 : cv[u];
            }
#pragma unroll
            for (int sft = 32; sft >= 1; sft >>= 1) sum += __shfl_xor(sum, sft, WAVE);
            hv = sum > 65534;
            if (lane == 0) mm.heavy[row] = hv ? MVHDP_ROW_HEAVY : (sum > 32767 ? MVHDP_ROW_BIG : 0);
        }
        double acc = 0.0, acc0 = 0.0;
        for (int k0 = 0; k0 < K; k0 += WAVE * TB) {
            int cv[TB];
            float fv[TB];
#pragma unroll
            for (int u = 0; u < TB; u++) {
                const int k = k0 + u * WAVE + lane;
                const bool in = k < K;
                cv[u] = in ? (light_src ? (int)c16[k] : cnt[k]) : 0;
                fv[u] = in ? cf[k] : 0.0f;
            }
#pragma unroll
            for (int u = 0; u < TB; u++) {
                const int k = k0 + u * WAVE + lane;
                if (k < K) {
                    if (!from_mirror) c16[k] = hv ? (uint16_t)65535 : (uint16_t)cv[u];
                    const double t = (double)fv[u] * (double)cv[u];
                    acc += t;
                    if (k < batch_cells) acc0 += t;
                }
            }
        }
#pragma unroll
        for (int sft = 32; sft >= 1; sft >>= 1) { acc += __shfl_xor(acc, sft, WAVE); acc0 += __shfl_xor(acc0, sft, WAVE); }
        if (lane == 0) { mm.root[row] = (double)smp_total + acc; mm.mass0[row] = (float)acc0; }
        if (lane == 0 && heavy_list && mm.heavy[row] == MVHDP_ROW_HEAVY) {
            const unsigned int i = atomicAdd(heavy_n, 1u);
            if ((int)i < heavy_cap) heavy_list[i] = (int32_t)row;
        }
    }
}

__global__ __launch_bounds__(64) void heavy_refresh_kernel(MvModel mm, const int32_t* heavy_list, const unsigned int* ctl , int heavy_cap, bool write_full)
{
    extern __shared__ double t[];
    const int K = mm.K, lane = threadIdx.x;
    const int64_t nrows = mm.rowbase[mm.M];
    const int32_t* nk_all = mm.counts + nrows * K;
    const unsigned long long t0 = __builtin_amdgcn_s_memrealtime();
    const int n = min((int)__hip_atomic_load(&ctl[0], __ATOMIC_RELAXED, __HIP_MEMORY_SCOPE_AGENT), heavy_cap);
#ifdef MVHDP_REFRESH_PRINT
    if (blockIdx.x == 0 && lane == 0) printf("[refresher] %d heavy rows\n", n);
#endif
    for (int pass = 0; pass < 1000000; pass++) {
        for (int i = blockIdx.x; i < n; i += gridDim.x) {
            const int64_t row = heavy_list[i];
            int m = 0;
            while (m + 1 < mm.M && row >= mm.rowbase[m + 1]) m++;
            const int32_t* cnt = mm.counts + row * K;
            const int32_t* nk = nk_all + (int64_t)m * K;
            const double* al = mm.alpha + (int64_t)m * (K + 1);
            const double beta = mm.beta[m], beta_sum = mm.beta_sum[m], gamma = mm.gamma[m];
            for (int k = lane; k < K; k += WAVE) {
                const int c = __hip_atomic_load(&cnt[k], __ATOMIC_RELAXED, __HIP_MEMORY_SCOPE_AGENT);
                t[K + k] = mm.inactive[k] ? 0.0 : gamma * al[k] * (((double)c + beta) / ((double)nk[k] + beta_sum));
            }
            tree_from_leaves<true>(mm, row, t, lane, write_full);
        }
#ifdef MVHDP_REFRESH_SLEEP_ONLY
        if (__builtin_amdgcn_s_memrealtime() - t0 > 300000ull) break;
        __builtin_amdgcn_s_sleep(127);
        continue;
#endif
        if (n <= (int)blockIdx.x) break;
        if (__hip_atomic_load(&ctl[1], __ATOMIC_RELAXED, __HIP_MEMORY_SCOPE_AGENT) != 0u) break;
        if (__builtin_amdgcn_s_memrealtime() - t0 > 200000000ull) break;
    }
}

hipError_t mvhdp_launch_heavy_refresh(const MvModel& mm, const int32_t* heavy_list, const unsigned int* ctl, int heavy_cap, int blocks, hipStream_t s)
{
    hipLaunchKernelGGL(heavy_refresh_kernel, dim3(blocks), dim3(64), (size_t)2 * mm.K * sizeof(double), s, mm, heavy_list, ctl, heavy_cap, getenv("MVHDP_REFRESH_FULL") != nullptr);
    return hipGetLastError();
}

__global__ void set_u32_kernel(unsigned int* p, unsigned int v) { __hip_atomic_store(p, v, __ATOMIC_RELAXED, __HIP_MEMORY_SCOPE_AGENT); }
hipError_t mvhdp_launch_set_u32(unsigned int* p, unsigned int v, hipStream_t s)
{
    hipLaunchKernelGGL(set_u32_kernel, dim3(1), dim3(1), 0, s, p, v);
// ... 873 lines not shown
```

### mvtopicmodel_amd/csrc/mvhdp_plan.h

```cpp
#pragma once
#include <stdint.h>
#include <stddef.h>
#include <algorithm>
#include <cmath>
#include <cstring>

#include "mvhdp_device.h"
#include "../../include/mvhdp.h"

enum { PLAN_STREAM_MAIN = 0, PLAN_STREAM_A = 1, PLAN_STREAM_B = 2, PLAN_STREAM_C = 3, PLAN_STREAM_D = 4, PLAN_N_STREAMS = 5 };

struct PlanRegs { int regs[MVHDP_N_CLASSES][3]; int regs_mix[MVHDP_N_CLASSES][3]; };

struct PlanIn {
    int K = 0, M = 0;
    int64_t D = 0;
    int64_t mdt = 0;
    int64_t n_longer[5] = {0, 0, 0, 0, 0};
    bool have_order = false;
    unsigned long long tok_hist[MVHDP_HIST_BINS] = {0};
    unsigned long long ent_hist[MVHDP_ENT_BINS] = {0};
    uint32_t flags = 0;
    bool debug = false;
    bool batch = false;
    bool trees_current = false;
    bool unassigned = false;
    int first_inactive = -1;
    bool vectors_mix = false;
    int num_cus = 256;
    size_t max_lds = 160 * 1024;
    PlanRegs regs{};
};

struct ClassLaunch {
    bool used = false;
    bool fast = false;
    int r = 0;
    int S_cap = 0;
    uint32_t wave_bytes = 0;
    int wpb = 0;
    size_t lds = 0;
    int grid = 0;
    int stream = PLAN_STREAM_MAIN;
    int walk = 0, narrow = 0;
    double theta[MVHDP_MAXM] = {0};
};

struct SweepPlan {
    int err = 0;
    const char* msg = "";
    uint32_t flags = 0;
    bool live = false, seg_apply = false, frozen = false, debug = false;
    bool overlap = false;
    int nseg = 1;
    int only_seg = -1;
    int S_cap = 0;
    bool fast = false;
    int pc = 0;
    bool route = false;
    int64_t H = 0;
    ClassLaunch cls[MVHDP_N_CLASSES];
    int class_map[MVHDP_N_CLASSES] = {0, 1, 2, 3, 4, 5};
    bool need_full = false;
    int nk_global = 0;
    uint32_t block_shared_bytes = 0;
    bool delta16 = false;
    bool live16 = false;
    bool live_rows = false;
    bool coef_lds = false;
    int dominant = 0;
    int walk_cfg = 0;
};

static inline double plan_class_tokens(const unsigned long long* tok_hist, int c)
{
    double t = 0;
    for (int b = 0; b < MVHDP_HIST_BINS; b++) {
        const int rounds = b + 1;
        int cb = 0;
        while (cb < 5 && rounds > (1 << cb)) cb++;
        if (b == MVHDP_HIST_BINS - 1) cb = 5;
        if (cb == c) t += (double)tok_hist[b];
    }
    return t;
}

static inline int plan_blocks_per_cu(int regs, int threads, size_t lds)
{
    int r = (regs + 7) / 8 * 8;
    int waves_simd = r > 0 ? 512 / r : 8;
    waves_simd = std::max(1, std::min(8, waves_simd));
    const int wpb = threads / 64;
    int b = waves_simd * 4 / wpb;
    b = std::min(b, (int)((160 * 1024) / (lds > 0 ? lds : 1)));
    b = std::min(b, 32 / wpb);
    return std::max(1, b);
}

size_t mvhdp_sweep_wave_bytes(int M, int S_cap);
size_t mvhdp_sweep_fast_wave_bytes(int M, int S_cap, int rmax);

struct PlanTuning {
    int force_primary = 0;
    int narrow = -1;
    int walk_fixed = 0;
    double walk_theta[MVHDP_MAXM] = {0};
    double primary_min_share = 0.10;
    int single_stream = 0;
    int four_round_on_c = -1;
    int delta16 = 1;
    int narrow_wide = 1;
    int fork_delay_us = 0;
    int widest_on_main = 0;
    int live_overlap = -1;
    int single_wave = 0;
    int live16 = -1;
    int live_rows = -1;
    int live_rows_segments = 1;
    int coef_lds_max_bytes = 12 * 1024;
    double live_rows_theta = 0.3;
};

enum { WALK_GROUPS = 3 };
struct WalkTuner {
    int walk_i = 0, walk_probe_i = 0, walk_b_i = 0, walk_phase = 0, walk_dir = 1, walk_fails = 0, walk_wait = 4, walk_cfg = -1, walk_maxj = 6;
    bool walk_far = false;
    double walk_ns_a1 = 0.0, walk_ns_b = 0.0;
    int walk_cls = 2, walk_i_by[WALK_GROUPS] = {-1, -1, -1};
    int walk_default[WALK_GROUPS] = {0, 0, 0};

    void init_defaults(int K)
    {
        if (K >= 256) { walk_default[0] = 6; walk_default[1] = MVHDP_WALK_BINS; walk_default[2] = 9; }
        walk_i = walk_default[walk_cls];
    }
    int stored(int g) const { return walk_i_by[g] >= 0 ? walk_i_by[g] : walk_default[g]; }
    double walk_cap = 0.004;
    long long walk_idle_until = 0, walk_refresh_at = 0, sweeps_done = 0;
    double walk_f[MVHDP_MAXM] = {-1, -1, -1, -1, -1, -1, -1, -1};
    double walk_hist[MVHDP_WALK_BINS] = {0};

    bool controlled(int m) const { return walk_f[m] >= 0.0 && walk_f[m] < 0.35; }
    bool any_controlled(int M) const { for (int m = 0; m < M; m++) if (controlled(m)) return true; return false; }
    bool any_unknown(int M) const { for (int m = 0; m < M; m++) if (walk_f[m] < 0.0) return true; return false; }

    void propose(int grp, int M, double theta[WALK_GROUPS][MVHDP_MAXM], bool* measure)
    {
        if (grp != walk_cls) {
            walk_i_by[walk_cls] = walk_i;
            walk_i = stored(grp);
            walk_cls = grp;
            walk_phase = 0; walk_far = false;
        }
        const bool any = any_controlled(M);
        const int top = MVHDP_WALK_BINS;
        walk_probe_i = walk_i;
        if (walk_phase == 1 && any) {
            if (walk_far && walk_i < 4) walk_far = false;
            if (walk_far) walk_dir = -1;
            if (walk_dir > 0 && walk_i >= top) walk_dir = -1;
            if (walk_dir < 0 && walk_i <= 0) walk_dir = 1;
            if (walk_dir > 0) {
                int j = 1;
                double extra = walk_hist[walk_i];
// ... 201 lines not shown
    auto walk_of = [&](int c) { const int g = group_of(c); bool w = measure || in.debug || mirror_pays || in.vectors_mix; for (int m = 0; m < M; m++) w = w || theta[g][m] > 0.0; return w ? 1 : 0; };

    ClassLaunch gen;
    if (!geometry(false, 5, 0, gen)) return fail(MVHDP_ERR_UNSUPPORTED, "per-entity LDS state exceeds 160 KiB (K * modalities too large)");
    gen.used = false;
    if (fast) {
        ClassLaunch pg;
        if (!geometry(true, pc, walk_of(pc), pg)) fast = false;
    }
    p.fast = fast;
    p.pc = fast ? pc : 5;
    const bool four_on_c = tu.four_round_on_c > 0 || (tu.four_round_on_c < 0 && !unknown && tok[2] < 0.03 * tot);
    const int stream_of[MVHDP_N_CLASSES] = {PLAN_STREAM_C, PLAN_STREAM_C, four_on_c ? PLAN_STREAM_C : PLAN_STREAM_D, PLAN_STREAM_B, PLAN_STREAM_A, PLAN_STREAM_A};
    if (!fast) {
        p.cls[5] = gen; p.cls[5].used = true; p.cls[5].stream = PLAN_STREAM_MAIN;
        for (int c = 0; c < MVHDP_N_CLASSES; c++) p.class_map[c] = 5;
        p.route = false; p.H = 0;
        p.need_full = true;
    } else {
        p.H = (S_cap > (64 << pc)) ? (in.have_order ? in.n_longer[pc] : in.D) : 0;
        if (view_16 && pc >= 3) p.H = in.have_order ? std::max<int64_t>(p.H, in.n_longer[4]) : in.D;
        p.route = p.H > 0;
        for (int c = pc; c < MVHDP_N_CLASSES; c++) {
            const bool reachable = c == pc || (p.route && (c <= c_max || (c == 5 && view_16)));
            const bool populated = c == pc || unknown || in.ent_hist[c] != 0 || (c == 5 && view_16);
            if (!(reachable && populated)) continue;
            ClassLaunch g;
            const int w = walk_of(c);
            if (c < 5 && geometry(true, c, w, g)) { g.walk = w; }
            else { g = gen; g.walk = 0; }
            g.used = true;
            g.stream = (c == pc || tu.single_stream || tu.single_wave) ? PLAN_STREAM_MAIN : stream_of[c];
            for (int m = 0; m < MVHDP_MAXM; m++) g.theta[m] = theta[group_of(c)][m];
            p.cls[c] = g;
        }
        if (!tu.single_stream && !tu.single_wave && tu.widest_on_main) {
            int next = PLAN_STREAM_MAIN;
            for (int c = MVHDP_N_CLASSES - 1; c >= pc; c--) if (p.cls[c].used) { p.cls[c].stream = next; next = std::min(next + 1, (int)PLAN_STREAM_D); }
        }
        for (int c = 0; c < MVHDP_N_CLASSES; c++) {
            int t = std::max(c, pc);
            while (t < MVHDP_N_CLASSES && !p.cls[t].used) t++;
            p.class_map[c] = t < MVHDP_N_CLASSES ? t : -1;
        }
        p.need_full = in.debug;
        for (int c = pc; c < MVHDP_N_CLASSES; c++) if (p.cls[c].used && !p.cls[c].fast) p.need_full = true;
        if (p.route && p.class_map[5] < 0 && (c_max == 5 || view_16)) {
            p.cls[5] = gen; p.cls[5].used = true; p.cls[5].stream = tu.single_stream ? PLAN_STREAM_MAIN : PLAN_STREAM_A; p.class_map[5] = 5; p.need_full = true;
        }
    }
    if (mirror_ok && !p.live && p.cls[0].used && p.cls[0].fast && p.cls[0].walk) p.cls[0].narrow = 1;
    if (mirror_ok && !p.live && tu.narrow_wide && tu.narrow != 1)
        for (int c = 1; c < 5; c++) if (p.cls[c].used && p.cls[c].fast && p.cls[c].walk) p.cls[c].narrow = 1;
    p.delta16 = tu.delta16 != 0 && mirror_ok && !p.live && !p.frozen && !p.seg_apply && nseg == 1 && p.only_seg < 0 &&
                !(flags & MVHDP_SWEEP_NO_APPLY) && !in.unassigned;
    if (want_live16) {
        bool all_fast = true;
        for (int c = 0; c < MVHDP_N_CLASSES; c++) if (p.cls[c].used && !p.cls[c].fast) all_fast = false;
        if (all_fast) {
            p.live16 = true;
            for (int c = 0; c < MVHDP_N_CLASSES; c++) if (p.cls[c].used) { p.cls[c].walk = 1; p.cls[c].narrow = 1; }
        }
    }
    if (want_rows) {
        bool all_fast = p.fast;
        for (int c = 0; c < MVHDP_N_CLASSES; c++) if (p.cls[c].used && !p.cls[c].fast) all_fast = false;
        if (all_fast) {
            p.live_rows = true;
            p.need_full = false;
            for (int c = 0; c < MVHDP_N_CLASSES; c++)
                if (p.cls[c].used) {
                    p.cls[c].walk = 1;
                    for (int m = 0; m < MVHDP_MAXM; m++) p.cls[c].theta[m] = (m < M && wt.controlled(m)) ? tu.live_rows_theta : 0.0;
                }
        } else p.coef_lds = false;
    } else p.coef_lds = false;
    p.walk_cfg = (in.vectors_mix ? 1 << 21 : 0) + (p.live_rows ? 1 << 20 : 0) + (p.fast ? (1 << p.dominant) : 32) * 2 + (p.route ? 1 : 0) + 64 * nseg + (p.live ? 1 << 16 : 0) + (p.seg_apply ? 1 << 17 : 0) + (p.live16 ? 1 << 18 : 0) + (p.overlap ? 1 << 19 : 0);
}
```

### mvtopicmodel_amd/csrc/mvhdp_sweep_fast.hip

```cpp
#include "mvhdp_device.h"
#include "../../include/mvhdp.h"
#include "mvhdp_wave.h"

size_t mvhdp_sweep_fast_wave_bytes(int M, int S_cap, int rmax)
{
    size_t counts = (size_t)M * S_cap * (rmax >= 8 ? 2 : 4);
    size_t b = (size_t)(64 + 64 + 64 + 16 + S_cap) * 4 + counts;
    b += (size_t)M * M * 12;
    return (b + 15) & ~(size_t)15;
}

#ifndef MVHDP_LB1
#define MVHDP_LB1 1
#endif
#ifndef MVHDP_LB1W
#define MVHDP_LB1W 7
#endif
#ifndef MVHDP_LB2
#define MVHDP_LB2 7
#endif
#ifndef MVHDP_LB2_ROOMY
#define MVHDP_LB2_ROOMY 6
#endif
#ifndef MVHDP_LB4
#define MVHDP_LB4 4
#endif
#ifndef MVHDP_NB2_FROM
#define MVHDP_NB2_FROM 4
#endif
#ifndef MVHDP_LB16
#define MVHDP_LB16 1
#endif
#ifndef MVHDP_LB_ROWS
#define MVHDP_LB_ROWS 7
#endif
#ifndef MVHDP_LB_MIX
#define MVHDP_LB_MIX 6
#endif
#ifndef MVHDP_LB8
#define MVHDP_LB8 1
#endif
#ifndef MVHDP_GATHER_SC
#define MVHDP_GATHER_SC 0
#endif
template <typename T>
__device__ __forceinline__ int gather_cell(gptr_t p)
{
    const __attribute__((address_space(1))) T* q = (const __attribute__((address_space(1))) T*)p;
#if MVHDP_GATHER_SC == 1
    return (int)__hip_atomic_load(q, __ATOMIC_RELAXED, __HIP_MEMORY_SCOPE_AGENT);
#elif MVHDP_GATHER_SC == 3
    return (int)__hip_atomic_load(q, __ATOMIC_RELAXED, __HIP_MEMORY_SCOPE_SYSTEM);
#elif MVHDP_GATHER_SC == 4
    return (int)__builtin_nontemporal_load(q);
#else
    return (int)*q;
#endif
}
template <typename T>
__device__ __forceinline__ T gather_mix(gptr_t p) { return *(const __attribute__((address_space(1))) T*)p; }
#define W_HEAVY 0x40000000
#define W_BIG   0x20000000
#define W_ROW(w) ((w) & 0x1fffffff)
typedef unsigned int rowq_t __attribute__((ext_vector_type(4), aligned(4)));
typedef float coefq_t __attribute__((ext_vector_type(4)));

__device__ __forceinline__ int smoothing_sample_live(const float* __restrict__ smp, int K, float t, int lane)
{
    for (int k0 = 0; k0 < K; k0 += WAVE) {
        const int k = k0 + lane;
        const float p = (k < K) ? smp[k] : 3.0e38f;
        const unsigned long long hit = __builtin_amdgcn_ballot_w64(p > t && k < K);
        if (hit) return k0 + (int)__builtin_ctzll(hit);
    }
    return K - 1;
}

template <bool CELL16>
__device__ __forceinline__ rowq_t row_batch_load(gptr_t rowp, int K, int b, int lane)
{
    constexpr int CPL = CELL16 ? 8 : 4;
    const int k = (b * WAVE + lane) * CPL;
    rowq_t q = {0u, 0u, 0u, 0u};
    if (k < K) q = *(const __attribute__((address_space(1))) rowq_t*)(rowp + (unsigned int)k * (CELL16 ? 2u : 4u));
    return q;
}

typedef float f2_t __attribute__((ext_vector_type(2)));
template <bool CELL16>
__device__ __forceinline__ int row_batch_pick(rowq_t q, coefq_t c0, coefq_t c1, int kb, float base, float target, bool force, float& tot, bool& any)
{
    constexpr int CPL = CELL16 ? 8 : 4, NS = CPL / 2;
    f2_t n2[NS], k2[NS], A[NS];
    if (CELL16) {
        n2[0] = f2_t{(float)(q.x & 0xffffu), (float)(q.x >> 16)}; n2[1] = f2_t{(float)(q.y & 0xffffu), (float)(q.y >> 16)};
        n2[NS - 2] = f2_t{(float)(q.z & 0xffffu), (float)(q.z >> 16)}; n2[NS - 1] = f2_t{(float)(q.w & 0xffffu), (float)(q.w >> 16)};
        k2[0] = f2_t{c0.x, c0.y}; k2[1] = f2_t{c0.z, c0.w}; k2[NS - 2] = f2_t{c1.x, c1.y}; k2[NS - 1] = f2_t{c1.z, c1.w};
    } else {
        n2[0] = f2_t{(float)(int)q.x, (float)(int)q.y}; n2[NS - 1] = f2_t{(float)(int)q.z, (float)(int)q.w};
        k2[0] = f2_t{c0.x, c0.y}; k2[NS - 1] = f2_t{c0.z, c0.w};
    }
    A[0] = n2[0] * k2[0];
#pragma unroll
    for (int s = 1; s < NS; s++) A[s] = __builtin_elementwise_fma(n2[s], k2[s], A[s - 1]);
    const float ev = A[NS - 1].x;
    const float acc = ev + A[NS - 1].y;
    const float incl = wave_incl_scan_f_dpp(acc);
    tot = bcast_f(incl, 63);
    const unsigned long long pos = __builtin_amdgcn_ballot_w64(acc > 0.0f);
    any = pos != 0;
    if (!pos || !(force || base + tot > target)) return -1;
    const unsigned long long hit = force ? 0ull : (__builtin_amdgcn_ballot_w64(base + incl > target) & pos);
    const int hl = hit ? (int)__builtin_ctzll(hit) : 63 - (int)__builtin_clzll(pos);
    const float thr = target - (base + (hl > 0 ? bcast_f(incl, hl - 1) : 0.0f));
    int cnt = 0;
#pragma unroll
// ... 34 lines not shown
            c0 = *(const __attribute__((address_space(3))) coefq_t*)(cf_lds + kl);
            if (CELL16) c1 = *(const __attribute__((address_space(3))) coefq_t*)(cf_lds + kl + 4);
        }
        float tot; bool any;
#ifdef MVHDP_TIMING
        { unsigned int probe = q0.x; asm volatile("v_mov_b32 %0, %0" : "+v"(probe)); *t_after_wait = __builtin_amdgcn_s_memtime(); }
#endif
        const int r = row_batch_pick<CELL16>(q0, c0, c1, bq * WAVE * CPL, bbase, target, false, tot, any);
        if (r >= 0) return r;
        if (nb == 1) {
            if (any) return row_batch_pick<CELL16>(q0, c0, c1, 0, 0.0f, 0.0f, true, tot, any);
            return smoothing_sample_live(smp, K, u2f * S, lane);
        }
    } else if (TWOB && nb == 2) {
        const rowq_t q = have_q0 ? q0 : row_batch_load<CELL16>(rowp, K, bq, lane);
        const int kl = (bq * WAVE + lane) * CPL;
        coefq_t c0 = {0.0f, 0.0f, 0.0f, 0.0f}, c1 = {0.0f, 0.0f, 0.0f, 0.0f};
        if (kl >= K) { }
        else if (in_lds) {
            c0 = *(const __attribute__((address_space(3))) coefq_t*)(cf_lds + kl);
            if (CELL16) c1 = *(const __attribute__((address_space(3))) coefq_t*)(cf_lds + kl + 4);
        } else {
            c0 = *(const __attribute__((address_space(1))) coefq_t*)(cf_g + kl);
            if (CELL16) c1 = *(const __attribute__((address_space(1))) coefq_t*)(cf_g + kl + 4);
        }
        float tot; bool any;
        const int r = row_batch_pick<CELL16>(q, c0, c1, bq * WAVE * CPL, bbase, target, false, tot, any);
        if (r >= 0) return r;
    }
    for (int pass = 0; pass < 2; pass++) {
        for (int b = (pass ? lastb : 0); b < (pass ? lastb + 1 : nb); b++) {
            const rowq_t q = (b == bq && have_q0) ? q0 : row_batch_load<CELL16>(rowp, K, b, lane);
            const int kl = (b * WAVE + lane) * CPL;
            coefq_t c0 = {0.0f, 0.0f, 0.0f, 0.0f}, c1 = {0.0f, 0.0f, 0.0f, 0.0f};
            if (kl >= K) { }
            else if (in_lds) {
                c0 = *(const __attribute__((address_space(3))) coefq_t*)(cf_lds + kl);
                if (CELL16) c1 = *(const __attribute__((address_space(3))) coefq_t*)(cf_lds + kl + 4);
            } else {
                c0 = *(const __attribute__((address_space(1))) coefq_t*)(cf_g + kl);
                if (CELL16) c1 = *(const __attribute__((address_space(1))) coefq_t*)(cf_g + kl + 4);
            }
            float tot; bool any;
            const int r = row_batch_pick<CELL16>(q, c0, c1, b * WAVE * CPL, base, target, pass != 0, tot, any);
            if (r >= 0) return r;
            if (any) lastb = b;
            base += tot;
        }
        if (lastb < 0) break;
    }
    return smoothing_sample_live(smp, K, u2f * S, lane);
}

template <int RMAX, bool DEBUG, bool WALK, bool NARROW, bool ROOMY = false, int LIVEROWS = 0, bool MIX = false>
__global__ __launch_bounds__(256, ((MIX && RMAX <= 2) ? MVHDP_LB_MIX : RMAX == 8 ? MVHDP_LB8 : (RMAX == 4 ? MVHDP_LB4 : (RMAX == 2 ? (ROOMY ? MVHDP_LB2_ROOMY : (LIVEROWS ? MVHDP_LB_ROWS : MVHDP_LB2)) : (RMAX == 1 ? (LIVEROWS ? MVHDP_LB_ROWS : WALK ? MVHDP_LB1W : MVHDP_LB1) : MVHDP_LB16))))) void sweep_fast_kernel(MvModel mm, SweepLaunch sl)
{
    static_assert(!MIX || (WALK && LIVEROWS == 0 && !ROOMY), "the mix flavours: walk flavour, stored trees");
    extern __shared__ __align__(16) unsigned char smem[];
#ifdef MVHDP_TIMING
    const unsigned long long t_begin0 = __builtin_amdgcn_s_memtime();
#endif
    const int lane = threadIdx.x & 63;
    const int wave = uniform_i(threadIdx.x >> 6);
    const int K = mm.K, M = mm.M, S = sl.S_cap;
    const int NW = (K + 31) >> 5;
    const bool exact_only = (sl.flags & MVHDP_SWEEP_EXACT_CHAIN) != 0;
    if (RMAX >= 8) __builtin_amdgcn_s_setprio(3);

    const int nkd_len = sl.nk_global ? 0 : M * K;
    int* nkd = (int*)smem;
    unsigned int* hist_s = (unsigned int*)(nkd + nkd_len);
    unsigned int* ent_s = hist_s + MVHDP_HIST_BINS;
    unsigned int* vstat_s = ent_s + MVHDP_ENT_BINS;
    for (int i = threadIdx.x; i < nkd_len + MVHDP_HIST_BINS + MVHDP_ENT_BINS + (WALK ? MVHDP_MAXM * MVHDP_VIEW_STATS : 0); i += blockDim.x) nkd[i] = 0;
    const int Kp = (K + 7) & ~7;
    float* const coef_s = (LIVEROWS && sl.coef_lds) ? (float*)(((uintptr_t)(vstat_s + MVHDP_MAXM * MVHDP_VIEW_STATS) + 15) & ~(uintptr_t)15) : nullptr;
    if (LIVEROWS && coef_s) for (int i = threadIdx.x; i < M * Kp; i += blockDim.x) coef_s[i] = mm.coef[i];
    int32_t* const dnk_g = mm.delta + mm.rowbase[M] * K;
    __syncthreads();
#ifdef MVHDP_TIMING
    const unsigned long long t_init_end = __builtin_amdgcn_s_memtime();
#endif

    unsigned char* wb = smem + sl.block_shared_bytes + (size_t)wave * sl.wave_bytes;
    uint32_t* bitmap = (uint32_t*)wb;
    uint32_t* prefix = bitmap + 64;
    uint32_t* bitmap2 = prefix + 64;
    int* wlen = (int*)(bitmap2 + 64);
    double* qsh = (double*)(wlen + 16);
    float* wsh = (float*)(qsh + M * M);
    int* sk = (int*)(wsh + M * M);
    constexpr bool PACK = RMAX >= 8;
    constexpr bool SCREEN = !DEBUG;
    typedef typename std::conditional<SCREEN, float, double>::type mixg_t;
    constexpr int MIXSH = SCREEN ? 0 : 1;
    int* sn = sk + S;
#define sn_get(idx) (PACK ? (int)((const unsigned short*)sn)[(idx)] : sn[(idx)])
#define sn_set(idx, v) do { if (PACK) ((unsigned short*)sn)[(idx)] = (unsigned short)(v); else sn[(idx)] = (v); } while (0)

    const int32_t* nwk = mm.counts;
    const uint16_t* nwk16 = mm.counts16;
    const int32_t* nk_all = mm.counts + mm.rowbase[M] * K;
    int32_t* dnwk = mm.delta;

    unsigned int n_tok = 0, n_chg = 0, c_new = 0, c_tree = 0, n_oov = 0, n_abort = 0, n_fb = 0, n_od = 0;

    const long long q_n1 = sl.q_list_count ? (long long)*sl.q_list_count : 0;
    const long long q_total = q_n1 + sl.q_order_count;
    unsigned int n_misclass = 0;
#ifdef MVHDP_TIMING
// ... 151 lines not shown
            };
            float rden32[RMAX], brden32[RMAX], oth32[RMAX];
            const float beta32 = (float)beta_m, scale32 = (float)scale_m;
            const bool mixv = MIX && m == 0;
            const double oml = MIX ? mm.oml : 1.0;
            const float oml32 = (float)oml;
            const char* const mix_v = MIX ? (SCREEN ? (const char*)mm.mix32 : (const char*)mm.mix) : nullptr;
            const char* const mix64_v = MIX ? (const char*)mm.mix : nullptr;
            const float* const smp_m = mm.coef + (int64_t)M * Kp + (int64_t)m * K;
            const float smS = LIVEROWS ? uniform_f(smp_m[K - 1]) : 0.0f;
#pragma unroll
            for (int r = 0; r < RMAX; r++) {
                cn[r] = 0;
                const int i = lane * R_eff + r;
                const bool used = r < R_eff && i < S_used;
                if (SCREEN) {
                    float acc = 0.0f;
                    double dn = 1.0;
                    if (used) {
                        const int k = koff[r] >> 2;
                        cn[r] = sn_get(m * S + i);
                        for (int j = 0; j < M; j++) {
                            if (j == m) continue;
                            const int cj = sn_get(j * S + i);
                            if (cj != 0) onz |= 1u << r;
                            acc = __builtin_fmaf(wsh[m * M + j], (float)cj + (float)(mm.gamma[j] * mm.alpha[(int64_t)j * (K + 1) + k]), acc);
                        }
                        dn = (double)nk[k] + mm.beta_sum[m];
                    }
                    oth[r] = 0.0; den[r] = 1.0;
                    rden32[r] = __builtin_amdgcn_rcpf((float)dn);
                    brden32[r] = beta32 * rden32[r];
                    if (MIX && mixv) { rden32[r] *= oml32; brden32[r] *= oml32; }
                    oth32[r] = acc * scale32;
                } else {
                    if (used) {
                        cn[r] = sn_get(m * S + i);
                        for (int j = 0; j < M; j++) if (j != m && sn_get(j * S + i) != 0) onz |= 1u << r;
                    }
                    slot_consts(r, oth[r], den[r]);
                    rden32[r] = 0.0f; brden32[r] = 0.0f; oth32[r] = 0.0f;
                }
            }
            double newAll = 0.0;
            for (int j = 0; j < M; j++) newAll += qsh[m * M + j];
            newAll = newAll * scale_m;
            const double newMass = (mm.first_inactive < 0) ? 0.0 : newAll / (double)K;
            const float pmm32 = uniform_f((float)p_mm), newMass32 = uniform_f((float)newMass);

            const int64_t base = mm.doc_off[m][d];
            const int64_t row0 = mm.rowbase[m];
            const char* nwk_v = (const char*)(nwk + row0 * K);
            const char* nwk16_v = (const char*)(nwk16 + row0 * K);
            int koffh[RMAX];
#pragma unroll
            for (int r = 0; r < RMAX; r++) koffh[r] = koff[r] >> 1;
            const int Vm = mm.V[m];
            const double walk_theta = sl.walk_theta[m];
            const unsigned int v_tok0 = n_tok, v_tree0 = c_tree;
            unsigned int whist_l = 0;

            MVHDP_TMAIN(tv, te, te);
            for (int c0 = 0; c0 < lenm && !aborted; c0 += WAVE) {
                const int ti = c0 + lane;
                const bool tvalid = ti < lenm;
                int w_l = tvalid ? mm.tok[m][base + ti] : -1;
                int z_l = tvalid ? mm.z[m][base + ti] : -1;
                int so_l = -1;
                if (z_l >= 0) {
                    uint32_t w = bitmap[z_l >> 5];
                    so_l = prefix[z_l >> 5] + __popc(w & ((1u << (z_l & 31)) - 1u));
                }
                double u1_l, u2_l;
                {
                    uint32_t x[4];
                    philox4x32_10((uint32_t)ti, (uint32_t)m, (uint32_t)dg, sl.sweep_idx,
                                  sl.seed_lo, sl.seed_hi ^ (uint32_t)((unsigned long long)dg >> 32), x);
                    u1_l = bits_to_unit(x[0], x[1]);
                    u2_l = bits_to_unit(x[2], x[3]);
                }
                MVHDP_TSUB2(tp);
                if (w_l >= Vm) w_l = -1;
                if (NARROW && w_l >= 0) {
                    const int hv = mm.heavy[row0 + w_l];
                    if (hv) w_l |= (hv == MVHDP_ROW_HEAVY) ? (W_HEAVY | W_BIG) : W_BIG;
                }
                const float u1f_l = (float)u1_l;
                int znew_l = z_l;

                double root_l = 0.0;
                int zt_l = -1, st_l = -1;
                const bool heavy_l = NARROW && w_l >= 0 && (w_l & W_HEAVY);
                const bool walk_l = tvalid && w_l >= 0 && (!WALK || u1_l >= walk_theta) && (!LIVEROWS || heavy_l);
                const unsigned long long walked = WALK ? __ballot(walk_l) : ~0ull;
                const unsigned long long specm = LIVEROWS ? __ballot(tvalid && w_l >= 0 && !heavy_l && u1_l >= walk_theta) : 0ull;
                rowq_t rowq = {0u, 0u, 0u, 0u};
                if (WALK && tvalid && w_l >= 0 && !walk_l) root_l = mm.root[row0 + W_ROW(w_l)];
                {
                    const bool act = walk_l;
                    const double* __restrict__ dt = mm.dtab + (row0 + W_ROW(max(w_l, 0))) * (int64_t)mm.dt_nblk * 8;
                    double u = 0.0;
                    int i = 1;
                    for (int bd = 0; bd < mm.dt_nbd; bd++) {
                        if (act && (bd == 0 || i < K)) {
                            const double2* __restrict__ blk = (const double2*)(dt + (int64_t)(mm.dt_base[bd] + (i - (1 << mm.dt_depth[bd]))) * 8);
                            double2 q0, q1, q2, q3;
                            if (LIVEROWS) {
                                const double* bp = (const double*)blk;
                                q0.x = __hip_atomic_load(bp + 0, __ATOMIC_RELAXED, __HIP_MEMORY_SCOPE_AGENT); q0.y = __hip_atomic_load(bp + 1, __ATOMIC_RELAXED, __HIP_MEMORY_SCOPE_AGENT);
                                q1.x = __hip_atomic_load(bp + 2, __ATOMIC_RELAXED, __HIP_MEMORY_SCOPE_AGENT); q1.y = __hip_atomic_load(bp + 3, __ATOMIC_RELAXED, __HIP_MEMORY_SCOPE_AGENT);
                                q2.x = __hip_atomic_load(bp + 4, __ATOMIC_RELAXED, __HIP_MEMORY_SCOPE_AGENT); q2.y = __hip_atomic_load(bp + 5, __ATOMIC_RELAXED, __HIP_MEMORY_SCOPE_AGENT);
                                q3.x = __hip_atomic_load(bp + 6, __ATOMIC_RELAXED, __HIP_MEMORY_SCOPE_AGENT); q3.y = __hip_atomic_load(bp + 7, __ATOMIC_RELAXED, __HIP_MEMORY_SCOPE_AGENT);
                            } else { q0 = blk[0]; q1 = blk[1]; q2 = blk[2]; q3 = blk[3]; }
                            const int levels = (bd == 0) ? mm.dt_f : 3;
                            if (bd == 0) { root_l = q3.y; u = u2_l * root_l; }
                            int path = 0;
                            if (i < K && levels > 0) {
                                const double l = q0.x;
                                if (u < l) { i = 2 * i; } else { u = u - l; i = 2 * i + 1; path = 1; }
                            }
                            if (i < K && levels > 1) {
                                const double l = path ? q1.x : q0.y;
                                if (u < l) { i = 2 * i; path = 2 * path; } else { u = u - l; i = 2 * i + 1; path = 2 * path + 1; }
                                if (i < K && levels > 2) {
                                    const double l3 = (path == 0) ? q1.y : (path == 1) ? q2.x : (path == 2) ? q2.y : q3.x;
                                    if (u < l3) { i = 2 * i; } else { u = u - l3; i = 2 * i + 1; }
                                }
                            }
                        }
                    }
                    if (act) {
                        zt_l = i - K;
                        const uint32_t wbit = bitmap[zt_l >> 5];
                        if ((wbit >> (zt_l & 31)) & 1u) st_l = (int)(prefix[zt_l >> 5] + __popc(wbit & ((1u << (zt_l & 31)) - 1u)));
                    }
                }

                MVHDP_TSUB2(tv);
                const float root32_l = (float)root_l;
                const float u2f_l = LIVEROWS ? (float)u2_l : 0.0f;
                unsigned long long bselm = 0ull;
                if (LIVEROWS == 2) {
                    constexpr int BCELLS = WAVE * (NARROW ? 8 : 4);
                    if (K > BCELLS && K <= 2 * BCELLS) {
                        float mass0_l = 0.0f;
                        if (tvalid && w_l >= 0 && !heavy_l) mass0_l = mm.mass0[row0 + W_ROW(w_l)];
                        bselm = __ballot(tvalid && w_l >= 0 && !heavy_l && (u2f_l * root32_l) - smS >= mass0_l);
                    }
                }
                MVHDP_TMAIN(th, te, tt);
                constexpr int NB = (RMAX >= MVHDP_NB2_FROM) ? 2 : 1;
                int gn[RMAX], gn2[RMAX];
                mixg_t gm[RMAX], gm2[RMAX];
                unsigned long long rem = __ballot(tvalid && w_l >= 0);
                n_oov += (unsigned int)__popcll(__ballot(tvalid && w_l < 0));
                n_tok += (unsigned int)__popcll(rem);
                const int t_first = rem ? (int)__builtin_ctzll(rem) : 0;
#pragma unroll
                for (int a = 0; a < NB; a++) {
                    const unsigned long long ra = (a == 0) ? rem : (rem & (rem - 1));
                    const int w0 = bcast_i(w_l, ra ? (int)__builtin_ctzll(ra) : t_first);
                    const unsigned int r0 = (unsigned int)W_ROW(max(w0, 0));
                    const bool h0 = w0 >= 0 && (w0 & W_HEAVY);
                    if (NARROW && !h0) {
                        const gptr_t c0q = scalar_row(nwk16_v, r0, (unsigned int)K * 2u);
#pragma unroll
                        for (int r = 0; r < RMAX; r++) { const int v = gather_cell<uint16_t>(c0q + (unsigned int)koffh[r]); if (a == 0) gn[r] = v; else gn2[r] = v; }
                    } else {
                        const gptr_t c0p = scalar_row(nwk_v, r0, (unsigned int)K * 4u);
#pragma unroll
                        for (int r = 0; r < RMAX; r++) { const int v = gather_cell<int32_t>(c0p + (unsigned int)koff[r]); if (a == 0) gn[r] = v; else gn2[r] = v; }
                    }
                    if (MIX && mixv) {
                        const gptr_t m0p = scalar_row(mix_v, r0, (unsigned int)K * (unsigned int)sizeof(mixg_t));
#pragma unroll
                        for (int r = 0; r < RMAX; r++) { const mixg_t v = gather_mix<mixg_t>(m0p + ((unsigned int)koff[r] << MIXSH)); if (a == 0) gm[r] = v; else gm2[r] = v; }
                    }
                }

                while (rem) {
                    const int t = (int)__builtin_ctzll(rem);
                    rem &= ~(1ull << t);
#define TOK_T t
#define TOK_G gn
#define TOK_MG gm
#include "mvhdp_sweep_fast_token.inc"
#undef TOK_T
#undef TOK_G
#undef TOK_MG
                    if (NB == 2 && rem) {
                        const int t1 = (int)__builtin_ctzll(rem);
                        rem &= ~(1ull << t1);
#define TOK_T t1
#define TOK_G gn2
#define TOK_MG gm2
#include "mvhdp_sweep_fast_token.inc"
#undef TOK_T
#undef TOK_G
#undef TOK_MG
                    }
                }

                MVHDP_TMAIN(tt, te, te);
                {
                    const bool chg = tvalid && (w_l >= 0) && (znew_l != z_l) && !(sl.flags & MVHDP_SWEEP_FROZEN);
                    n_chg += (unsigned int)__popcll(__ballot(chg));
                    if (chg) {
                        const int64_t rowK = (row0 + W_ROW(w_l)) * K;
                        if (NARROW && sl.live16 && !(w_l & W_HEAVY)) {
                            unsigned int* m32 = (unsigned int*)mm.counts16;
                            if (z_l >= 0) { const int64_t c = rowK + z_l; __hip_atomic_fetch_add(&m32[c >> 1], 0u - (1u << ((c & 1) * 16)), __ATOMIC_RELAXED, __HIP_MEMORY_SCOPE_AGENT); }
                            { const int64_t c = rowK + znew_l; __hip_atomic_fetch_add(&m32[c >> 1], 1u << ((c & 1) * 16), __ATOMIC_RELAXED, __HIP_MEMORY_SCOPE_AGENT); }
                        } else if (NARROW && sl.delta16 && !(w_l & W_BIG)) {
                            unsigned int* d32 = (unsigned int*)mm.delta16;
                            if (z_l >= 0) { const int64_t c = rowK + z_l; __hip_atomic_fetch_add(&d32[c >> 1], 0u - (1u << ((c & 1) * 16)), __ATOMIC_RELAXED, __HIP_MEMORY_SCOPE_AGENT); }
                            { const int64_t c = rowK + znew_l; __hip_atomic_fetch_add(&d32[c >> 1], 1u << ((c & 1) * 16), __ATOMIC_RELAXED, __HIP_MEMORY_SCOPE_AGENT); }
                        } else {
#ifdef MVHDP_PROBE
                            const int probe = (int)((sl.flags >> 16) & 7u);
                            int64_t c_old = rowK + z_l, c_new = rowK + znew_l;
// ... 56 lines not shown
#pragma unroll
            for (int sft = 32; sft >= 1; sft >>= 1) c2 += __shfl_xor(c2, sft, WAVE);
            if (lane == 0) {
                mm.nslots[d] = aborted ? (uint16_t)MVHDP_NSLOTS_UNKNOWN : (uint16_t)c2;
                if (sl.slot_hist) {
                    if (c2 > 0) atomicAdd(&hist_s[min((c2 + 63) >> 6, MVHDP_HIST_BINS) - 1], (unsigned int)doc_tokens);
                    atomicAdd(&ent_s[aborted ? MVHDP_N_CLASSES : mvhdp_class_of(c2, longest_view > 65535)], 1u);
                }
            }
        }
        LDS_FENCE();
#ifdef MVHDP_TIMING
        { const int b = e_ord < 2 ? e_ord : 2; t_ent[b] += __builtin_amdgcn_s_memtime() - t_e0; n_ent[b] += n_tok - n_tok_e0; e_ord++; }
#endif
      }
    }

#ifdef MVHDP_TIMING
    const unsigned long long t_loop_end = __builtin_amdgcn_s_memtime();
#endif
    __syncthreads();
    for (int i = threadIdx.x; i < nkd_len; i += blockDim.x)
        if (nkd[i]) atomicAdd(&dnk_g[i], nkd[i]);
    if (sl.slot_hist && threadIdx.x < MVHDP_HIST_BINS + MVHDP_ENT_BINS && hist_s[threadIdx.x]) atomicAdd(&sl.slot_hist[threadIdx.x], (unsigned long long)hist_s[threadIdx.x]);
    if (WALK && threadIdx.x < MVHDP_MAXM * MVHDP_VIEW_STATS && vstat_s[threadIdx.x])
        atomicAdd(&sl.stats[ST_VIEW_BASE + threadIdx.x], (unsigned long long)vstat_s[threadIdx.x]);
    if (lane == 0) {
        if (n_tok) atomicAdd(&sl.stats[ST_TOKENS], (unsigned long long)n_tok);
        if (n_chg) atomicAdd(&sl.stats[ST_CHANGED], (unsigned long long)n_chg);
        if (c_new) atomicAdd(&sl.stats[ST_NEW], (unsigned long long)c_new);
        const unsigned int c_doc = n_tok - c_new - c_tree;
        if (c_doc) atomicAdd(&sl.stats[ST_DOC], (unsigned long long)c_doc);
        if (c_tree) atomicAdd(&sl.stats[ST_TREE], (unsigned long long)c_tree);
        if (n_oov) atomicAdd(&sl.stats[ST_OOV], (unsigned long long)n_oov);
        if (n_abort) atomicAdd(&sl.stats[ST_ABORT], (unsigned long long)n_abort);
        if (n_fb) atomicAdd(&sl.stats[ST_FALLBACK], (unsigned long long)n_fb);
        if (n_od) atomicAdd(&sl.stats[ST_ONDEMAND], (unsigned long long)n_od);
        if (n_misclass) atomicAdd(&sl.stats[ST_MISCLASS], (unsigned long long)n_misclass);
#ifdef MVHDP_TIMING
        atomicAdd(&sl.stats[ST_T_QUEUE], tq); atomicAdd(&sl.stats[ST_T_PROLOGUE], tp); atomicAdd(&sl.stats[ST_T_VIEW], tv);
        atomicAdd(&sl.stats[ST_T_CHUNK_HEAD], th); atomicAdd(&sl.stats[ST_T_TOKENS], tt); atomicAdd(&sl.stats[ST_T_CHUNK_END], te);
        atomicAdd(&sl.stats[ST_T_TOTAL], (unsigned long long)__builtin_amdgcn_s_memtime() - t_begin);
        for (int b = 0; b < 3; b++) { atomicAdd(&sl.stats[ST_T_ENT0 + b], t_ent[b]); atomicAdd(&sl.stats[ST_N_ENT0 + b], n_ent[b]); }
        atomicAdd(&sl.stats[ST_T_INIT], t_init_end - t_begin0); atomicAdd(&sl.stats[ST_T_FLUSH], (unsigned long long)__builtin_amdgcn_s_memtime() - t_loop_end);
        atomicAdd(&sl.stats[ST_N_WAVES], 1ull);
        atomicAdd(&sl.stats[ST_T_ROWS], t_rows); atomicAdd(&sl.stats[ST_T_ROWS_WAIT], t_rows_wait);
#endif
    }
}

#undef sn_get
#undef sn_set

static bool roomy_build(int rmax, int K) { return rmax == 2 && K >= 512; }
static bool two_batch_rows(int K) { return K > 512 && K <= 1024; }

template <int RMAX>
static const void* fast_kernel_ptr_mix(bool debug, bool narrow)
{
    if (debug) return (const void*)sweep_fast_kernel<RMAX, true, true, false, false, 0, true>;
    return narrow ? (const void*)sweep_fast_kernel<RMAX, false, true, true, false, 0, true> : (const void*)sweep_fast_kernel<RMAX, false, true, false, false, 0, true>;
}

template <int RMAX>
static const void* fast_kernel_ptr(bool debug, bool walk, bool narrow, int K = 0, bool live_rows = false)
{
    if (live_rows && !debug) {
        if constexpr (RMAX == 2) { if (narrow && roomy_build(RMAX, K)) return (const void*)sweep_fast_kernel<2, false, true, true, true, 2>; }
        if (narrow && two_batch_rows(K)) return (const void*)sweep_fast_kernel<RMAX, false, true, true, false, 2>;
        return narrow ? (const void*)sweep_fast_kernel<RMAX, false, true, true, false, 1> : (const void*)sweep_fast_kernel<RMAX, false, true, false, false, 1>;
    }
    if (narrow && walk && !debug) {
        if constexpr (RMAX == 2) { if (roomy_build(RMAX, K)) return (const void*)sweep_fast_kernel<2, false, true, true, true>; }
        return (const void*)sweep_fast_kernel<RMAX, false, true, true>;
    }
    return debug ? (const void*)sweep_fast_kernel<RMAX, true, true, false>
                 : walk ? (const void*)sweep_fast_kernel<RMAX, false, true, false> : (const void*)sweep_fast_kernel<RMAX, false, false, false>;
}

template <int RMAX>
static hipError_t launch_fast(const MvModel& mm, const SweepLaunch& sl, int grid_blocks, bool debug, hipStream_t s)
{
    size_t lds = sl.block_shared_bytes + (size_t)sl.waves_per_block * sl.wave_bytes;
    dim3 block(64 * sl.waves_per_block);
    const bool narrow = sl.narrow && sl.walk && !debug;
    const bool rows = sl.live_rows && sl.walk && !debug;
    if (mm.mix) {
        if (rows || !sl.walk) return hipErrorInvalidValue;
        if (lds > 65536) {
            hipError_t e = hipFuncSetAttribute(fast_kernel_ptr_mix<RMAX>(debug, narrow), hipFuncAttributeMaxDynamicSharedMemorySize, (int)lds);
            if (e != hipSuccess) return e;
        }
        if (debug)       hipLaunchKernelGGL((sweep_fast_kernel<RMAX, true, true, false, false, 0, true>), dim3(grid_blocks), block, lds, s, mm, sl);
        else if (narrow) hipLaunchKernelGGL((sweep_fast_kernel<RMAX, false, true, true, false, 0, true>), dim3(grid_blocks), block, lds, s, mm, sl);
        else             hipLaunchKernelGGL((sweep_fast_kernel<RMAX, false, true, false, false, 0, true>), dim3(grid_blocks), block, lds, s, mm, sl);
        return hipGetLastError();
    }
    if (lds > 65536) {
        hipError_t e = hipFuncSetAttribute(fast_kernel_ptr<RMAX>(debug, sl.walk != 0, narrow, mm.K, rows), hipFuncAttributeMaxDynamicSharedMemorySize, (int)lds);
        if (e != hipSuccess) return e;
    }
    if (debug)        hipLaunchKernelGGL((sweep_fast_kernel<RMAX, true, true, false>), dim3(grid_blocks), block, lds, s, mm, sl);
    else if (rows) {
        if (narrow && roomy_build(RMAX, mm.K)) { if constexpr (RMAX == 2) hipLaunchKernelGGL((sweep_fast_kernel<2, false, true, true, true, 2>), dim3(grid_blocks), block, lds, s, mm, sl); }
        else if (narrow && two_batch_rows(mm.K)) hipLaunchKernelGGL((sweep_fast_kernel<RMAX, false, true, true, false, 2>), dim3(grid_blocks), block, lds, s, mm, sl);
        else if (narrow) hipLaunchKernelGGL((sweep_fast_kernel<RMAX, false, true, true, false, 1>), dim3(grid_blocks), block, lds, s, mm, sl);
        else             hipLaunchKernelGGL((sweep_fast_kernel<RMAX, false, true, false, false, 1>), dim3(grid_blocks), block, lds, s, mm, sl);
    }
    else if (narrow && roomy_build(RMAX, mm.K)) {
        if constexpr (RMAX == 2) hipLaunchKernelGGL((sweep_fast_kernel<2, false, true, true, true>), dim3(grid_blocks), block, lds, s, mm, sl);
    }
    else if (narrow)  hipLaunchKernelGGL((sweep_fast_kernel<RMAX, false, true, true>), dim3(grid_blocks), block, lds, s, mm, sl);
    else if (sl.walk) hipLaunchKernelGGL((sweep_fast_kernel<RMAX, false, true, false>), dim3(grid_blocks), block, lds, s, mm, sl);
    else              hipLaunchKernelGGL((sweep_fast_kernel<RMAX, false, false, false>), dim3(grid_blocks), block, lds, s, mm, sl);
    return hipGetLastError();
}

hipError_t mvhdp_launch_sweep_fast(const MvModel& mm, const SweepLaunch& sl, int rmax, int grid_blocks, bool debug, hipStream_t s)
{
    switch (rmax) {
    case 1: return launch_fast<1>(mm, sl, grid_blocks, debug, s);
    case 2: return launch_fast<2>(mm, sl, grid_blocks, debug, s);
    case 3:
    case 4: return launch_fast<4>(mm, sl, grid_blocks, debug, s);
    case 8: return launch_fast<8>(mm, sl, grid_blocks, debug, s);
    case 16: return launch_fast<16>(mm, sl, grid_blocks, debug, s);
    default: return hipErrorInvalidValue;
    }
}

static int blocks_per_cu_from(const void* func, int threads, size_t lds)
{
    hipFuncAttributes a;
    if (hipFuncGetAttributes(&a, func) != hipSuccess) return 1;
    int regs = (a.numRegs + 7) / 8 * 8;
    int waves_simd = regs > 0 ? 512 / regs : 8;
    if (waves_simd > 8) waves_simd = 8;
    if (waves_simd < 1) waves_simd = 1;
    int wpb = threads / 64;
    int by_regs = waves_simd * 4 / wpb;
    int by_lds = (int)((160 * 1024) / (lds > 0 ? lds : 1));
    int by_waves = 32 / wpb;
    int b = by_regs < by_lds ? by_regs : by_lds;
    if (by_waves < b) b = by_waves;
    return b < 1 ? 1 : b;
}

template <int RMAX>
static int occ_fast(bool debug, bool walk, int threads, size_t lds)
{
    return blocks_per_cu_from(fast_kernel_ptr<RMAX>(debug, walk, false), threads, lds);
}

int mvhdp_sweep_fast_occupancy(int rmax, bool debug, bool walk, int block_threads, size_t lds_bytes)
{
    switch (rmax) {
    case 1: return occ_fast<1>(debug, walk, block_threads, lds_bytes);
    case 2: return occ_fast<2>(debug, walk, block_threads, lds_bytes);
    case 3:
    case 4: return occ_fast<4>(debug, walk, block_threads, lds_bytes);
// ... 27 lines not shown
```

### mvtopicmodel_amd/csrc/mvhdp_sweep_fast_token.inc

```
{
                    int g[RMAX];
#pragma unroll
                    for (int r = 0; r < RMAX; r++) g[r] = TOK_G[r];
                    mixg_t mg[RMAX];
#pragma unroll
                    for (int r = 0; r < RMAX; r++) mg[r] = (MIX && mixv) ? TOK_MG[r] : (mixg_t)0;
                    const int wfull_t = LIVEROWS ? bcast_i(w_l, TOK_T) : 0;
                    const gptr_t rowp_t = !LIVEROWS ? (gptr_t)0 : NARROW ? scalar_row(nwk16_v, (unsigned int)W_ROW(wfull_t), (unsigned int)K * 2u)
                                                                         : scalar_row(nwk_v, (unsigned int)W_ROW(wfull_t), (unsigned int)K * 4u);
                    const bool spec_t = LIVEROWS && ((specm >> TOK_T) & 1ull);
                    const int bsel_t = (LIVEROWS == 2) ? (int)((bselm >> TOK_T) & 1ull) : 0;
                    if (LIVEROWS) {
#pragma unroll
                        for (int r = 0; r < RMAX; r++) asm volatile("" : "+v"(g[r]));
                        if (spec_t) rowq = row_batch_load<NARROW>(rowp_t, K, bsel_t, lane);
                    }
                    const unsigned long long rem_n = (NB == 2) ? (rem & (rem - 1)) : rem;
#pragma unroll
                    for (int r = 0; r < RMAX; r++) { touch_lane_off(koff[r]); if (NARROW) touch_lane_off(koffh[r]); }
                    if (NB == 2 || LIVEROWS || rem_n) {
                        const int wn = bcast_i(w_l, rem_n ? (int)__builtin_ctzll(rem_n) : TOK_T);
                        if (NARROW && !(wn & W_HEAVY)) {
                            const gptr_t cnq = scalar_row(nwk16_v, (unsigned int)W_ROW(wn), (unsigned int)K * 2u);
#pragma unroll
                            for (int r = 0; r < RMAX; r++) TOK_G[r] = gather_cell<uint16_t>(cnq + (unsigned int)koffh[r]);
                        } else {
                            const gptr_t cnp = scalar_row(nwk_v, (unsigned int)W_ROW(wn), (unsigned int)K * 4u);
#pragma unroll
                            for (int r = 0; r < RMAX; r++) TOK_G[r] = gather_cell<int32_t>(cnp + (unsigned int)koff[r]);
                        }
                        if (MIX && mixv) {
                            const gptr_t mnp = scalar_row(mix_v, (unsigned int)W_ROW(wn), (unsigned int)K * (unsigned int)sizeof(mixg_t));
#pragma unroll
                            for (int r = 0; r < RMAX; r++) TOK_MG[r] = gather_mix<mixg_t>(mnp + ((unsigned int)koff[r] << MIXSH));
                        }
                    }
                    const int w = W_ROW(bcast_i(w_l, TOK_T));
                    const int so = bcast_i(so_l, TOK_T);
                    const int64_t row = row0 + w;

                    if (so >= 0) {
                        const int rs = so & (R_eff - 1), ls = so >> lg;
#pragma unroll
                        for (int r = 0; r < RMAX; r++) {
                            if (rs == r) {
                                const int c = bcast_i(cn[r], ls) - 1;
                                cn[r] = wave_writelane(cn[r], c, ls);
                                if (c == 0 && !((bcast_i((int)onz, ls) >> r) & 1)) live_m[r] &= ~(1ull << ls);
                            }
                        }
                    }

                    double mass = 0.0, s0 = 0.0, s1 = 0.0, total = 0.0;
                    int branch = 2, slot_new = -1;
                    bool unsafe = false;
                    double term[RMAX] = {};
                    bool need64 = DEBUG || exact_only || !SCREEN;
                    if (SCREEN && !need64) {
                        const float u1f = bcast_f(u1f_l, TOK_T), rootf = bcast_f(root32_l, TOK_T);
                        float t32[RMAX], c32v[RMAX];
#pragma unroll
                        for (int r = 0; r < RMAX; r++) {
                            float pw = __builtin_fmaf((float)g[r], rden32[r], brden32[r]);
                            if (MIX && mixv) pw += (float)mg[r];
                            const float a32 = __builtin_fmaf(pmm32, (float)cn[r], oth32[r]);
                            t32[r] = __builtin_amdgcn_inverse_ballot_w64(live_m[r]) ? a32 * pw : 0.0f;
                        }
                        float ls = t32[0];
                        c32v[0] = ls;
#pragma unroll
                        for (int r = 1; r < RMAX; r++) { ls += t32[r]; c32v[r] = ls; }
                        const float incl = wave_incl_scan_f_dpp(ls);
                        const float excl = incl - ls;
#pragma unroll
                        for (int r = 0; r < RMAX; r++) c32v[r] = (r == RMAX - 1) ? incl : excl + c32v[r];
                        const float massf = bcast_f(incl, 63);
                        const float totalf = (newMass32 + massf) + rootf;
                        const float s0f = u1f * totalf;
                        const float tolf = totalf * 0x1.0p-17f;
                        bool close;
                        if (s0f < newMass32) {
                            branch = 0;
                            close = fabsf(s0f - newMass32) <= tolf;
                        } else {
                            const float s1f = s0f - newMass32;
                            close = (fabsf(s1f) <= tolf) || (fabsf(s1f - massf) <= tolf);
                            if (s1f < massf) {
                                branch = 1;
                                unsigned long long anyhit = 0, near = 0, hitr[RMAX];
#pragma unroll
// ... 141 lines not shown
                            if (sl.trace_doc[q] == d && sl.trace_view[q] == m && sl.trace_pos[q] == c0 + TOK_T) {
                                double* out = sl.trace_out + (int64_t)q * (K + 1);
                                const double* tr = mm.trees + row * 2 * K;
                                for (int k = lane; k < K; k += WAVE) out[k] = tr[K + k] / total;
                                __threadfence();
#pragma unroll
                                for (int r = 0; r < RMAX; r++)
                                    if (r < R_eff && __builtin_amdgcn_inverse_ballot_w64(live_m[r])) out[koff[r] >> 2] += term[r] / total;
                                if (lane == 0) out[K] = newMass / total;
                                __threadfence();
                            }
                        }
                    }

                    int znew;
                    if (branch == 1) {
                        if (slot_new < 0) {
                            aborted = true;
                            n_tok -= (unsigned int)__popcll(rem);
                            rem = 0;
                            znew = bcast_i(z_l, TOK_T);
                        } else {
                            const int rn = slot_new & (R_eff - 1), ln = slot_new >> lg;
                            int ksel = koff[0];
#pragma unroll
                            for (int r = 1; r < RMAX; r++) ksel = (rn == r) ? koff[r] : ksel;
                            znew = bcast_i(ksel, ln) >> 2;
                        }
                    } else if (branch == 0) {
                        c_new++;
                        znew = mm.first_inactive;
                        if (sl.births) {
                            const int bp_ = __hip_atomic_load(&sl.births[0], __ATOMIC_RELAXED, __HIP_MEMORY_SCOPE_AGENT);
                            znew = bp_ < sl.births[1] ? sl.births[2 + bp_] : -1;
                        }
                        if (znew < 0) znew = K - 1;
                        const uint32_t wbit = bitmap[znew >> 5];
                        slot_new = ((wbit >> (znew & 31)) & 1u) ? (int)(prefix[znew >> 5] + __popc(wbit & ((1u << (znew & 31)) - 1u))) : -1;
                        slot_new = uniform_i(slot_new);
                    } else {
                        c_tree++;
                        if (WALK) whist_l += (lane == min((int)(bcast_f(u1f_l, TOK_T) * MVHDP_WALK_BINS), MVHDP_WALK_BINS - 1)) ? 1u : 0u;
                        if (!WALK || ((walked >> TOK_T) & 1ull)) {
                            znew = bcast_i(zt_l, TOK_T);
                            slot_new = bcast_i(st_l, TOK_T);
                        } else if (LIVEROWS && !(NARROW && (wfull_t & W_HEAVY))) {
                            n_od++;
                            unsigned long long t_rs1 = 0;
#ifdef MVHDP_TIMING
                            const unsigned long long t_rs0 = __builtin_amdgcn_s_memtime();
#endif
                            if (sl.flags & 0x2000u) znew = bcast_i(z_l, TOK_T);
                            else
                            znew = uniform_i(row_sample_live<NARROW, LIVEROWS == 2>(rowq, spec_t, coef_s != nullptr, (const __attribute__((address_space(3))) float*)coef_s + m * Kp, mm.coef + (int64_t)m * Kp, smp_m, smS, rowp_t, K,
                                                                     bcast_f(u2f_l, TOK_T), bcast_f(root32_l, TOK_T), bsel_t, (LIVEROWS == 2 && bsel_t) ? mm.mass0[row] : 0.0f , lane, &t_rs1));
                            if (znew < 0) znew = K - 1;
#ifdef MVHDP_TIMING
                            t_rows += __builtin_amdgcn_s_memtime() - t_rs0;
                            if (t_rs1) t_rows_wait += t_rs1 - t_rs0;
#endif
                            const uint32_t wbit = bitmap[znew >> 5];
                            slot_new = ((wbit >> (znew & 31)) & 1u) ? (int)(prefix[znew >> 5] + __popc(wbit & ((1u << (znew & 31)) - 1u))) : -1;
                            slot_new = uniform_i(slot_new);
                        } else {
                            n_od++;
                            uint32_t x[4];
                            philox4x32_10((uint32_t)(c0 + TOK_T), (uint32_t)m, (uint32_t)dg, sl.sweep_idx,
                                          sl.seed_lo, sl.seed_hi ^ (uint32_t)((unsigned long long)dg >> 32), x);
                            znew = uniform_i(dtab_sample_uniform(mm, row, bits_to_unit(x[2], x[3])));
                            const uint32_t wbit = bitmap[znew >> 5];
                            slot_new = ((wbit >> (znew & 31)) & 1u) ? (int)(prefix[znew >> 5] + __popc(wbit & ((1u << (znew & 31)) - 1u))) : -1;
                            slot_new = uniform_i(slot_new);
                        }
                        if (znew < 0) znew = K - 1;
                    }
                    znew = uniform_i(znew);

                    znew_l = wave_writelane(znew_l, znew, TOK_T);
                    if (slot_new >= 0) {
                        const int rn = slot_new & (R_eff - 1), ln = slot_new >> lg;
#pragma unroll
                        for (int r = 0; r < RMAX; r++) if (rn == r) cn[r] = wave_writelane(cn[r], bcast_i(cn[r], ln) + 1, ln);
                    }
}
```

### mvtopicmodel_amd/native.py

```python
import atexit
import ctypes as C
import sys
import weakref
from dataclasses import dataclass, field

import numpy as np

from ._lib import (DIAG_MAX_TOP_WORDS, DIAG_PROPORTIONS, DIAG_ROWS, MAX_M, UNIQUE_ID_BYTES, Config, DebugC, DiagArgsC, DiagOutC,
                   EmbConfigC, EmbStatsC, GroupInfoC, HyperC, MvhdpError, SweepStatsC, TuningC, load_library)

SWEEP_REUSE_TREES = 0x1
SWEEP_NO_APPLY = 0x2
SWEEP_EXACT_CHAIN = 0x4
SWEEP_GENERIC_KERNEL = 0x8
SWEEP_FROZEN = 0x10
SWEEP_LIVE = 0x20
SWEEP_SEGMENT_APPLY = 0x40
SWEEP_SEGMENT_OVERLAP = 0x80
SWEEP_ASYNC_EXCHANGE = 0x100
SWEEP_SHARD_BIRTHS = 0x200


def SWEEP_LIVE_SEGMENTS(n):
    return (int(n) & 0xFF) << 16

def SWEEP_ONLY_SEGMENT(s):
    return ((int(s) + 1) & 0xFF) << 24


EMB_SERIAL = 0x1

BUF_COUNTS = 0
BUF_DELTA = 1
BUF_BIRTH_KEYS = 2
ACT_KEY_NONE = (1 << 63) - 1


def _ptr(a):
    return None if a is None else a.ctypes.data_as(C.c_void_p)


_live = weakref.WeakSet()


@atexit.register
def _close_all():
    for s in list(_live):
        try:
            s.close()
        except Exception:
            pass


@dataclass
class Hyper:
    alpha: np.ndarray
    alpha_sum: np.ndarray
    beta: np.ndarray
    beta_sum: np.ndarray
    gamma: np.ndarray
    p_a: np.ndarray
    p_b: np.ndarray
    inactive: np.ndarray = None

    @staticmethod
    def defaults(K, V, alpha=0.1, beta=0.01, p_a=0.31, p_b=1.0, inactive=None):
        M = len(V)
        return Hyper(alpha=np.full((M, K + 1), alpha, dtype=np.float64),
                     alpha_sum=np.full(M, K * alpha, dtype=np.float64),
                     beta=np.full(M, beta, dtype=np.float64),
                     beta_sum=np.array([beta * v for v in V], dtype=np.float64),
                     gamma=np.ones(M, dtype=np.float64),
                     p_a=np.full((M, M), p_a, dtype=np.float64),
                     p_b=np.full((M, M), p_b, dtype=np.float64),
                     inactive=None if inactive is None else np.asarray(inactive, dtype=np.uint8))


@dataclass
class SweepStats:
    tokens: int = 0
    changed: int = 0
    new_mass_cnt: int = 0
    topic_doc_mass_cnt: int = 0
    word_ftree_mass_cnt: int = 0
    oov_skipped: int = 0
    aborted_docs: int = 0
    exact_fallbacks: int = 0
# ... 609 lines not shown
```

Measured before the change: 6.770 billion.

## Add 12-bit packed word-topic count table for narrow walk sweeps

Adds a 12-bit packed counts table (85 cells per 128-byte line) that is filled during tree builds for rows whose maximum count fits in 12 bits, and flags those rows with a new SLIM bit in the row-class byte. Narrow walk sweep kernels get a NARROW==2 variant that gathers counts from this table for slim rows, falling back to the 16-bit or 32-bit mirrors otherwise. The aim is to cut memory traffic and cache footprint for the count gathers. In exchange it adds pack and unpack work, an extra table and extra syncs in the tree build, and call sites that previously compared the raw heavy byte now have to mask out the new bit.

```diff
diff --git a/include/mvhdp.h b/include/mvhdp.h
--- a/include/mvhdp.h
+++ b/include/mvhdp.h
@@ -102,7 +102,9 @@
 typedef enum {
     MVHDP_BUF_COUNTS = 0,
     MVHDP_BUF_DELTA  = 1,
-    MVHDP_BUF_BIRTH_KEYS = 2
+    MVHDP_BUF_BIRTH_KEYS = 2,
+    MVHDP_BUF_COUNTS12 = 3,
+    MVHDP_BUF_ROW_CLASS = 4
 } mvhdp_buffer;
 
 int mvhdp_create(const mvhdp_config* cfg, mvhdp_handle* out);
diff --git a/mvtopicmodel_amd/csrc/mvhdp_api.hip b/mvtopicmodel_amd/csrc/mvhdp_api.hip
--- a/mvtopicmodel_amd/csrc/mvhdp_api.hip
+++ b/mvtopicmodel_amd/csrc/mvhdp_api.hip
@@ -42,6 +42,7 @@
     if (const char* f = getenv("MVHDP_LIVE_ROWS_SEGMENTS")) h->tu.live_rows_segments = std::max(1, std::min(255, atoi(f)));
     if (const char* f = getenv("MVHDP_WIDEST_ON_MAIN")) h->tu.widest_on_main = atoi(f) != 0;
     if (const char* f = getenv("MVHDP_NARROW_WIDE")) h->tu.narrow_wide = atoi(f) != 0;
+    if (const char* f = getenv("MVHDP_SLIM")) h->tu.slim = std::max(0, std::min(2, atoi(f)));
     if (const char* f = getenv("MVHDP_LIVE_TREE_EVERY")) h->live_tree_every = std::max(1, atoi(f));
     if (const char* f = getenv("MVHDP_GATE_PCT")) { const int v = atoi(f); if (v >= 5 && v <= 95) h->gate_pct = v; }
     if (const char* f = getenv("MVHDP_FOUR_ROUND_ON_C")) h->tu.four_round_on_c = atoi(f);
@@ -158,6 +159,14 @@
     for (int c = 0; c < MVHDP_N_CLASSES; c++)
         for (int f = 0; f < 3; f++) { h->regs.regs[c][f] = mvhdp_sweep_kernel_regs(c, f); h->regs.regs_mix[c][f] = mvhdp_sweep_kernel_regs(c, f ? f : 1, true); }
     read_environment(h);
+    {
+        int vmax = 0;
+        for (int m = 0; m < M; m++) vmax = std::max(vmax, (int)cfg->num_types[m]);
+        if (plan_slim_table(K, vmax, h->tu.slim)) {
+            CREATE_HIP(hipMalloc(&mm.counts12, (size_t)nrows * mvhdp_slim_row_bytes(K)));
+            CREATE_HIP(hipMemset(mm.counts12, 0, (size_t)nrows * mvhdp_slim_row_bytes(K)));
+        }
+    }
     mm.alpha = h->d_alpha;
     mm.inactive = h->d_inactive;
     h->h_alpha.assign((size_t)M * (K + 1), 0.0);
@@ -176,7 +185,7 @@
     if (h->stream) hipStreamSynchronize(h->stream);
     auto fr = [](auto*& p) { if (p) { hipFree((void*)p); p = nullptr; } };
     for (int m = 0; m < MVHDP_MAXM; m++) { fr(h->d_doc_off[m]); fr(h->d_tok[m]); fr(h->d_z[m]); fr(h->d_carry[m]); fr(h->d_present[m]); }
-    fr(h->mm.counts); fr(h->mm.delta16); fr(h->mm.counts16); fr(h->mm.heavy); fr(h->mm.delta); fr(h->mm.trees); fr(h->mm.root); fr(h->mm.coef); fr(h->mm.mass0); fr(h->d_births); fr(h->d_birth_keys); fr(h->d_birth_table); fr(h->mm.dtab); fr(h->mm.p);
+    fr(h->mm.counts); fr(h->mm.delta16); fr(h->mm.counts16); fr(h->mm.counts12); fr(h->mm.heavy); fr(h->mm.delta); fr(h->mm.trees); fr(h->mm.root); fr(h->mm.coef); fr(h->mm.mass0); fr(h->d_births); fr(h->d_birth_keys); fr(h->d_birth_table); fr(h->mm.dtab); fr(h->mm.p);
     fr(h->d_alpha); fr(h->d_inactive); fr(h->d_ctl);
     fr(h->d_mix); fr(h->d_mix32); h->mm.mix = nullptr; h->mm.mix32 = nullptr; h->mix_lambda = 0.0;
     mvhdp_emb_free(h);
@@ -780,6 +789,9 @@
     in.vectors_mix = mm.mix != nullptr && !(flags & MVHDP_SWEEP_FROZEN);
     in.num_cus = h->num_cus; in.max_lds = h->max_lds;
     in.regs = h->regs;
+    in.slim_table = mm.counts12 != nullptr;
+    in.max_types = 0;
+    for (int m = 0; m < mm.M; m++) in.max_types = std::max(in.max_types, (int)mm.V[m]);
 }
 
 static int alloc_debug(mvhdp_ctx* h, const mvhdp_debug* dbg, DebugBufs& db)
@@ -1298,7 +1310,7 @@
     for (int c = 0; c < MVHDP_N_CLASSES; c++)
         if (p.cls[c].used)
             fprintf(stderr, " [class %d %s grid %d wpb %d lds %zu stream %d%s%s theta0 %.2f ents %llu]", c, p.cls[c].fast ? "fast" : "generic", p.cls[c].grid, p.cls[c].wpb, p.cls[c].lds,
-                    p.cls[c].stream, p.cls[c].walk ? " walk" : "", p.cls[c].narrow ? " narrow" : "", p.cls[c].theta[0], (unsigned long long)h->last_ent[c]);
+                    p.cls[c].stream, p.cls[c].walk ? " walk" : "", p.cls[c].narrow == 2 ? " slim" : p.cls[c].narrow ? " narrow" : "", p.cls[c].theta[0], (unsigned long long)h->last_ent[c]);
     fprintf(stderr, "\n");
 }
 
@@ -1564,6 +1576,7 @@
     for (int c = 0; c < MVHDP_N_CLASSES; c++) for (int f = 0; f < 3; f++) in.regs.regs[c][f] = pi->kernel_registers[c][f];
     for (int c = 0; c < MVHDP_N_CLASSES; c++) for (int f = 0; f < 3; f++) in.regs.regs_mix[c][f] = pi->kernel_registers_mix[c][f] > 0 ? pi->kernel_registers_mix[c][f] : pi->kernel_registers[c][f];
     in.vectors_mix = pi->vectors_mix != 0 && !(pi->flags & MVHDP_SWEEP_FROZEN);
+    in.slim_table = t && t->narrow == 2;
     PlanTuning tu;
     WalkTuner wt;
     wt.init_defaults(in.K);
@@ -1630,7 +1643,9 @@
     if (which == MVHDP_BUF_COUNTS) { *dev_ptr = h->mm.counts; *bytes = b; return MVHDP_OK; }
     if (which == MVHDP_BUF_DELTA) { *dev_ptr = h->mm.delta; *bytes = b; return MVHDP_OK; }
     if (which == MVHDP_BUF_BIRTH_KEYS) { *dev_ptr = h->d_birth_table; *bytes = (size_t)h->mm.K * sizeof(long long); return MVHDP_OK; }
-    FAIL(h, MVHDP_ERR_INVALID_ARG, "device_buffer: unknown buffer");
+    if (which == MVHDP_BUF_COUNTS12 && h->mm.counts12) { *dev_ptr = h->mm.counts12; *bytes = (size_t)h->mm.rowbase[h->mm.M] * mvhdp_slim_row_bytes(h->mm.K); return MVHDP_OK; }
+    if (which == MVHDP_BUF_ROW_CLASS) { *dev_ptr = h->mm.heavy; *bytes = (size_t)h->mm.rowbase[h->mm.M]; return MVHDP_OK; }
+    FAIL(h, MVHDP_ERR_INVALID_ARG, "device_buffer: unknown buffer (or a handle without that table)");
 }
 
 extern "C" int mvhdp_counts_written(mvhdp_handle h)
diff --git a/mvtopicmodel_amd/csrc/mvhdp_device.h b/mvtopicmodel_amd/csrc/mvhdp_device.h
--- a/mvtopicmodel_amd/csrc/mvhdp_device.h
+++ b/mvtopicmodel_amd/csrc/mvhdp_device.h
@@ -38,11 +38,14 @@
     const double* mix;
     const float* mix32;
     double oml;
+    uint8_t* counts12;
 };
 
 #define MVHDP_SL_STRICT_LIVE 0x8000u
 #define MVHDP_ROW_HEAVY 1
 #define MVHDP_ROW_BIG 2
+#define MVHDP_ROW_SLIM 4
+#define MVHDP_ROW_CLASS(h) ((h) & 3)
 
 struct SweepLaunch {
     uint32_t sweep_idx;
diff --git a/mvtopicmodel_amd/csrc/mvhdp_group.hip b/mvtopicmodel_amd/csrc/mvhdp_group.hip
--- a/mvtopicmodel_amd/csrc/mvhdp_group.hip
+++ b/mvtopicmodel_amd/csrc/mvhdp_group.hip
@@ -94,7 +94,7 @@
     for (int64_t row = r0 + (int64_t)blockIdx.x * (blockDim.x >> 6) + (threadIdx.x >> 6); row < r1; row += wstride) {
         const int32_t* d = delta + row * K;
         int32_t* o = xp + woff[row];
-        if (heavy[row] == 0) {
+        if (MVHDP_ROW_CLASS(heavy[row]) == 0) {
             const int nw = (K + 1) >> 1;
             for (int j = lane; j < nw; j += 64) { const int a = d[2 * j], b = (2 * j + 1 < K) ? d[2 * j + 1] : 0; o[j] = a + b * 65536; }
         } else for (int k = lane; k < K; k += 64) o[k] = d[k];
@@ -109,7 +109,7 @@
     for (int64_t row = r0 + (int64_t)blockIdx.x * (blockDim.x >> 6) + (threadIdx.x >> 6); row < r1; row += wstride) {
         int32_t* d = delta + row * K;
         const int32_t* o = xp + woff[row];
-        if (heavy[row] == 0) {
+        if (MVHDP_ROW_CLASS(heavy[row]) == 0) {
             const int nw = (K + 1) >> 1;
             for (int j = lane; j < nw; j += 64) {
                 const int w = o[j];
@@ -484,6 +484,7 @@
     std::vector<uint8_t> cls((size_t)rows);
     GHIP(g, hipSetDevice(L0->device));
     GHIP(g, hipMemcpy(cls.data(), L0->mm.heavy, (size_t)rows, hipMemcpyDeviceToHost));
+    for (auto& c : cls) c = (uint8_t)MVHDP_ROW_CLASS(c);
     g->woff.assign((size_t)rows + 1, 0);
     for (int64_t r = 0; r < rows; r++) g->woff[(size_t)r + 1] = g->woff[(size_t)r] + (cls[(size_t)r] == 0 ? (K + 1) / 2 : K);
     if (g->d_woff.empty()) { g->d_woff.assign(g->leaders.size(), nullptr); g->d_cls.assign(g->leaders.size(), nullptr); g->xpack.assign(g->leaders.size(), nullptr); }
diff --git a/mvtopicmodel_amd/csrc/mvhdp_kernels.hip b/mvtopicmodel_amd/csrc/mvhdp_kernels.hip
--- a/mvtopicmodel_amd/csrc/mvhdp_kernels.hip
+++ b/mvtopicmodel_amd/csrc/mvhdp_kernels.hip
@@ -1,4 +1,5 @@
 #include "mvhdp_device.h"
+#include "mvhdp_slim.h"
 #include "../../include/mvhdp.h"
 
 #include "mvhdp_wave.h"
@@ -98,7 +99,7 @@
     int neg = 0;
     __builtin_amdgcn_s_setprio(3);
     for (int64_t row = row_begin + blockIdx.x; row < row_end; row += gridDim.x) {
-        if (only_heavy && mm.heavy[row] != MVHDP_ROW_HEAVY) continue;
+        if (only_heavy && MVHDP_ROW_CLASS(mm.heavy[row]) != MVHDP_ROW_HEAVY) continue;
         int m = 0;
         while (m + 1 < mm.M && row >= mm.rowbase[m + 1]) m++;
         int32_t* cnt = mm.counts + row * K;
@@ -107,12 +108,13 @@
         const double* al = mm.alpha + (int64_t)m * (K + 1);
         const double beta = mm.beta[m], beta_sum = mm.beta_sum[m], gamma = mm.gamma[m];
         uint16_t* c16 = mm.counts16 + row * K;
-        const bool light_src = from_mirror && mm.heavy[row] != MVHDP_ROW_HEAVY;
+        const bool light_src = from_mirror && MVHDP_ROW_CLASS(mm.heavy[row]) != MVHDP_ROW_HEAVY;
         const bool mixed = MIX && m == 0 && !inference_leaves;
         const double* mixrow = mixed ? mm.mix + row * K : nullptr;
-        bool hv = false;
+        bool hv = false, slim = false;
         if (!from_mirror) {
             long long sum = 0;
+            int big = 0;
             for (int k0 = 0; k0 < K; k0 += WAVE * TB) {
                 int cv[TB], dv[TB];
 #pragma unroll
@@ -131,13 +133,15 @@
                             if (d) { c += d; cnt[k] = c; dl[k] = 0; neg += c < 0; }
                         }
                         sum += c < 0 ? 70000 : c;
+                        big = max(big, c < 0 ? 70000 : c);
                     }
                 }
             }
 #pragma unroll
-            for (int sft = 32; sft >= 1; sft >>= 1) sum += __shfl_xor(sum, sft, WAVE);
+            for (int sft = 32; sft >= 1; sft >>= 1) { sum += __shfl_xor(sum, sft, WAVE); big = max(big, __shfl_xor(big, sft, WAVE)); }
             hv = sum > 65534;
-            if (lane == 0) mm.heavy[row] = hv ? MVHDP_ROW_HEAVY : (sum > 32767 ? MVHDP_ROW_BIG : 0);
+            slim = mm.counts12 != nullptr && big <= MVHDP_SLIM_MAX;
+            if (lane == 0) mm.heavy[row] = (uint8_t)((hv ? MVHDP_ROW_HEAVY : (sum > 32767 ? MVHDP_ROW_BIG : 0)) | (slim ? MVHDP_ROW_SLIM : 0));
         }
         for (int k0 = 0; k0 < K; k0 += WAVE * TB) {
             int cv[TB], nkv[TB];
@@ -160,6 +164,7 @@
                     const int c = cv[u];
                     if (light_src) cnt[k] = c;
                     else if (!from_mirror) c16[k] = hv ? (uint16_t)65535 : (uint16_t)c;
+                    if (slim) ((int*)t)[k] = c;
                     double leaf;
                     if (inference_leaves) {
                         leaf = ((double)c + beta) / ((double)nkv[u] + beta_sum);
@@ -174,6 +179,23 @@
                 }
             }
         }
+        if (slim) {
+            __syncthreads();
+            const int* cs = (const int*)t;
+            unsigned int* out12 = (unsigned int*)(mm.counts12 + (size_t)row * mvhdp_slim_row_bytes(K));
+            const int nwords = (int)(mvhdp_slim_row_bytes(K) >> 2);
+            for (int w = lane; w < nwords; w += WAVE) {
+                const int j = w >> 5, bit0 = (w & 31) * 32;
+                unsigned int v = 0;
+#pragma unroll
+                for (int q = 0; q < 4; q++) {
+                    const int i = bit0 / 12 + q, k = j * MVHDP_SLIM_CELLS + i, sh = 12 * i - bit0;
+                    if (i < MVHDP_SLIM_CELLS && k < K && sh < 32) { const unsigned int c = (unsigned int)cs[k]; v |= sh >= 0 ? c << sh : c >> -sh; }
+                }
+                out12[w] = v;
+            }
+            __syncthreads();
+        }
         tree_from_leaves(mm, row, t, lane, write_full);
     }
     if (apply_first && negatives) {
@@ -252,7 +274,7 @@
         if (!d) continue;
         const int old = __hip_atomic_fetch_add(&mm.counts[i], d, __ATOMIC_RELAXED, __HIP_MEMORY_SCOPE_AGENT);
         neg += old + d < 0;
-        if (use_mirror && i < n_cells && mm.heavy[i / K] != MVHDP_ROW_HEAVY) __hip_atomic_fetch_add(&m32[i >> 1], (unsigned int)d << ((i & 1) * 16), __ATOMIC_RELAXED, __HIP_MEMORY_SCOPE_AGENT);
+        if (use_mirror && i < n_cells && MVHDP_ROW_CLASS(mm.heavy[i / K]) != MVHDP_ROW_HEAVY) __hip_atomic_fetch_add(&m32[i >> 1], (unsigned int)d << ((i & 1) * 16), __ATOMIC_RELAXED, __HIP_MEMORY_SCOPE_AGENT);
     }
     if (neg && negatives) atomicAdd(negatives, (unsigned long long)neg);
 }
@@ -276,7 +298,7 @@
         if (!dl) continue;
         mm.counts[i] += dl;
         d[i] = 0;
-        if (use_mirror && i < n_cells && mm.heavy[i / K] != MVHDP_ROW_HEAVY) __hip_atomic_fetch_add(&m32[i >> 1], (unsigned int)dl << ((i & 1) * 16), __ATOMIC_RELAXED, __HIP_MEMORY_SCOPE_AGENT);
+        if (use_mirror && i < n_cells && MVHDP_ROW_CLASS(mm.heavy[i / K]) != MVHDP_ROW_HEAVY) __hip_atomic_fetch_add(&m32[i >> 1], (unsigned int)dl << ((i & 1) * 16), __ATOMIC_RELAXED, __HIP_MEMORY_SCOPE_AGENT);
     }
 }
 
@@ -313,7 +335,7 @@
     const int lane = threadIdx.x & 63;
     const int64_t wstride = (int64_t)gridDim.x * (blockDim.x >> 6);
     for (int64_t row = (int64_t)blockIdx.x * (blockDim.x >> 6) + (threadIdx.x >> 6); row < nrows; row += wstride) {
-        if (mm.heavy[row] == MVHDP_ROW_HEAVY) continue;
+        if (MVHDP_ROW_CLASS(mm.heavy[row]) == MVHDP_ROW_HEAVY) continue;
         const uint16_t* c16 = mm.counts16 + row * K;
         int32_t* cnt = mm.counts + row * K;
         for (int k = lane; k < K; k += WAVE) cnt[k] = (int)c16[k];
@@ -358,7 +380,7 @@
         const int Kp = (K + 7) & ~7;
         const float* cf = mm.coef + (int64_t)m * Kp;
         const float smp_total = mm.coef[(int64_t)mm.M * Kp + (int64_t)m * K + K - 1];
-        const bool light_src = from_mirror && mm.heavy[row] != MVHDP_ROW_HEAVY;
+        const bool light_src = from_mirror && MVHDP_ROW_CLASS(mm.heavy[row]) != MVHDP_ROW_HEAVY;
         bool hv = false;
         if (!from_mirror) {
             long long sum = 0;
@@ -399,7 +421,7 @@
 #pragma unroll
         for (int sft = 32; sft >= 1; sft >>= 1) { acc += __shfl_xor(acc, sft, WAVE); acc0 += __shfl_xor(acc0, sft, WAVE); }
         if (lane == 0) { mm.root[row] = (double)smp_total + acc; mm.mass0[row] = (float)acc0; }
-        if (lane == 0 && heavy_list && mm.heavy[row] == MVHDP_ROW_HEAVY) {
+        if (lane == 0 && heavy_list && MVHDP_ROW_CLASS(mm.heavy[row]) == MVHDP_ROW_HEAVY) {
             const unsigned int i = atomicAdd(heavy_n, 1u);
             if ((int)i < heavy_cap) heavy_list[i] = (int32_t)row;
         }
diff --git a/mvtopicmodel_amd/csrc/mvhdp_plan.h b/mvtopicmodel_amd/csrc/mvhdp_plan.h
--- a/mvtopicmodel_amd/csrc/mvhdp_plan.h
+++ b/mvtopicmodel_amd/csrc/mvhdp_plan.h
@@ -6,6 +6,7 @@
 #include <cstring>
 
 #include "mvhdp_device.h"
+#include "mvhdp_slim.h"
 #include "../../include/mvhdp.h"
 
 enum { PLAN_STREAM_MAIN = 0, PLAN_STREAM_A = 1, PLAN_STREAM_B = 2, PLAN_STREAM_C = 3, PLAN_STREAM_D = 4, PLAN_N_STREAMS = 5 };
@@ -30,7 +31,13 @@
     int num_cus = 256;
     size_t max_lds = 160 * 1024;
     PlanRegs regs{};
+    bool slim_table = false;
+    int max_types = 0;
 };
+
+enum { PLAN_SLIM_MAX_CLASS = 2 };
+static inline bool plan_slim_table(int K, int max_types, int level) { return mvhdp_slim_pays(K, max_types, level) != 0; }
+
 
 struct ClassLaunch {
     bool used = false;
@@ -110,6 +117,7 @@
     int four_round_on_c = -1;
     int delta16 = 1;
     int narrow_wide = 1;
+    int slim = 1;
     int fork_delay_us = 0;
     int widest_on_main = 0;
     int live_overlap = -1;
@@ -417,6 +425,8 @@
     if (mirror_ok && !p.live && p.cls[0].used && p.cls[0].fast && p.cls[0].walk) p.cls[0].narrow = 1;
     if (mirror_ok && !p.live && tu.narrow_wide && tu.narrow != 1)
         for (int c = 1; c < 5; c++) if (p.cls[c].used && p.cls[c].fast && p.cls[c].walk) p.cls[c].narrow = 1;
+    if (mirror_ok && !p.live && !p.overlap && !in.vectors_mix && !in.debug && in.slim_table && plan_slim_table(K, in.max_types, tu.slim))
+        for (int c = 0; c <= PLAN_SLIM_MAX_CLASS; c++) if (p.cls[c].used && p.cls[c].fast && p.cls[c].narrow == 1) p.cls[c].narrow = 2;
     p.delta16 = tu.delta16 != 0 && mirror_ok && !p.live && !p.frozen && !p.seg_apply && nseg == 1 && p.only_seg < 0 &&
                 !(flags & MVHDP_SWEEP_NO_APPLY) && !in.unassigned;
     if (want_live16) {
diff --git a/mvtopicmodel_amd/csrc/mvhdp_slim.h b/mvtopicmodel_amd/csrc/mvhdp_slim.h
--- /dev/null
+++ b/mvtopicmodel_amd/csrc/mvhdp_slim.h
@@ -0,0 +1,35 @@
+#pragma once
+#include <stdint.h>
+#include <stddef.h>
+
+#if defined(__HIPCC__) || defined(__CUDACC__)
+#define MVHDP_SLIM_FN __host__ __device__ static inline
+#else
+#define MVHDP_SLIM_FN static inline
+#endif
+
+enum { MVHDP_SLIM_LINE = 128, MVHDP_SLIM_CELLS = 85, MVHDP_SLIM_MAX = 4095 };
+
+MVHDP_SLIM_FN size_t mvhdp_slim_row_bytes(int K) { return (size_t)MVHDP_SLIM_LINE * (size_t)((K + MVHDP_SLIM_CELLS - 1) / MVHDP_SLIM_CELLS); }
+MVHDP_SLIM_FN unsigned int mvhdp_slim_byte(int k) { const unsigned int j = (unsigned int)k / MVHDP_SLIM_CELLS, i = (unsigned int)k - j * MVHDP_SLIM_CELLS; return MVHDP_SLIM_LINE * j + ((3u * i) >> 1); }
+MVHDP_SLIM_FN unsigned int mvhdp_slim_shift(int k) { return 4u * (((unsigned int)k % MVHDP_SLIM_CELLS) & 1u); }
+
+MVHDP_SLIM_FN unsigned int mvhdp_slim_get(const unsigned char* row, int k)
+{
+    const unsigned char* p = row + mvhdp_slim_byte(k);
+    return ((((unsigned int)p[1] << 8) | (unsigned int)p[0]) >> mvhdp_slim_shift(k)) & 0xfffu;
+}
+MVHDP_SLIM_FN void mvhdp_slim_put(unsigned char* row, int k, unsigned int v)
+{
+    unsigned char* p = row + mvhdp_slim_byte(k);
+    const unsigned int w = (v & 0xfffu) << mvhdp_slim_shift(k);
+    p[0] = (unsigned char)(p[0] | (w & 0xffu));
+    p[1] = (unsigned char)(p[1] | (w >> 8));
+}
+
+MVHDP_SLIM_FN int mvhdp_slim_pays(int K, int max_types, int level)
+{
+    if (level == 0 || max_types >= (1 << 28)) return 0;
+    if ((K + MVHDP_SLIM_CELLS - 1) / MVHDP_SLIM_CELLS >= (K + 63) / 64) return 0;
+    return (level >= 2 || K >= 256) ? 1 : 0;
+}
diff --git a/mvtopicmodel_amd/csrc/mvhdp_sweep_fast.hip b/mvtopicmodel_amd/csrc/mvhdp_sweep_fast.hip
--- a/mvtopicmodel_amd/csrc/mvhdp_sweep_fast.hip
+++ b/mvtopicmodel_amd/csrc/mvhdp_sweep_fast.hip
@@ -1,6 +1,7 @@
 #include "mvhdp_device.h"
 #include "../../include/mvhdp.h"
 #include "mvhdp_wave.h"
+#include "mvhdp_slim.h"
 
 size_t mvhdp_sweep_fast_wave_bytes(int M, int S_cap, int rmax)
 {
@@ -61,7 +62,14 @@
 __device__ __forceinline__ T gather_mix(gptr_t p) { return *(const __attribute__((address_space(1))) T*)p; }
 #define W_HEAVY 0x40000000
 #define W_BIG   0x20000000
-#define W_ROW(w) ((w) & 0x1fffffff)
+#define W_SLIM  0x10000000
+#define W_ROW(w) ((w) & (NARROW == 2 ? 0x0fffffff : 0x1fffffff))
+typedef unsigned short u16_any_t __attribute__((aligned(1)));
+__device__ __forceinline__ int gather_slim(gptr_t row, int packed)
+{
+    return (int)*(const __attribute__((address_space(1))) u16_any_t*)(row + ((unsigned int)packed >> 5));
+}
+__device__ __forceinline__ int slim_cell(int raw, int packed) { return (int)__builtin_amdgcn_ubfe((unsigned int)raw, (unsigned int)packed, 12u); }
 typedef unsigned int rowq_t __attribute__((ext_vector_type(4), aligned(4)));
 typedef float coefq_t __attribute__((ext_vector_type(4)));
 
@@ -202,10 +210,11 @@
     return smoothing_sample_live(smp, K, u2f * S, lane);
 }
 
-template <int RMAX, bool DEBUG, bool WALK, bool NARROW, bool ROOMY = false, int LIVEROWS = 0, bool MIX = false>
+template <int RMAX, bool DEBUG, bool WALK, int NARROW, bool ROOMY = false, int LIVEROWS = 0, bool MIX = false>
 __global__ __launch_bounds__(256, ((MIX && RMAX <= 2) ? MVHDP_LB_MIX : RMAX == 8 ? MVHDP_LB8 : (RMAX == 4 ? MVHDP_LB4 : (RMAX == 2 ? (ROOMY ? MVHDP_LB2_ROOMY : (LIVEROWS ? MVHDP_LB_ROWS : MVHDP_LB2)) : (RMAX == 1 ? (LIVEROWS ? MVHDP_LB_ROWS : WALK ? MVHDP_LB1W : MVHDP_LB1) : MVHDP_LB16))))) void sweep_fast_kernel(MvModel mm, SweepLaunch sl)
 {
     static_assert(!MIX || (WALK && LIVEROWS == 0 && !ROOMY), "the mix flavours: walk flavour, stored trees");
+    static_assert(NARROW != 2 || (WALK && !DEBUG && LIVEROWS == 0 && !MIX), "the 12-bit image: deferred sweeps of the walk flavour only");
     extern __shared__ __align__(16) unsigned char smem[];
 #ifdef MVHDP_TIMING
     const unsigned long long t_begin0 = __builtin_amdgcn_s_memtime();
@@ -463,9 +472,14 @@
             const int64_t row0 = mm.rowbase[m];
             const char* nwk_v = (const char*)(nwk + row0 * K);
             const char* nwk16_v = (const char*)(nwk16 + row0 * K);
+            const char* nwk12_v = (NARROW == 2) ? (const char*)mm.counts12 + (size_t)row0 * mvhdp_slim_row_bytes(K) : nullptr;
+            const unsigned int row12_bytes = (unsigned int)mvhdp_slim_row_bytes(K);
             int koffh[RMAX];
 #pragma unroll
             for (int r = 0; r < RMAX; r++) koffh[r] = koff[r] >> 1;
+            int kslim[RMAX];
+#pragma unroll
+            for (int r = 0; r < RMAX; r++) { const int k = koff[r] >> 2; kslim[r] = (NARROW == 2) ? (int)((mvhdp_slim_byte(k) << 5) | mvhdp_slim_shift(k)) : 0; }
             const int Vm = mm.V[m];
             const double walk_theta = sl.walk_theta[m];
             const unsigned int v_tok0 = n_tok, v_tree0 = c_tree;
@@ -493,8 +507,9 @@
                 MVHDP_TSUB2(tp);
                 if (w_l >= Vm) w_l = -1;
                 if (NARROW && w_l >= 0) {
-                    const int hv = mm.heavy[row0 + w_l];
+                    const int hb = mm.heavy[row0 + w_l], hv = MVHDP_ROW_CLASS(hb);
                     if (hv) w_l |= (hv == MVHDP_ROW_HEAVY) ? (W_HEAVY | W_BIG) : W_BIG;
+                    if (NARROW == 2 && (hb & MVHDP_ROW_SLIM)) w_l |= W_SLIM;
                 }
                 const float u1f_l = (float)u1_l;
                 int znew_l = z_l;
@@ -573,10 +588,14 @@
                     const int w0 = bcast_i(w_l, ra ? (int)__builtin_ctzll(ra) : t_first);
                     const unsigned int r0 = (unsigned int)W_ROW(max(w0, 0));
                     const bool h0 = w0 >= 0 && (w0 & W_HEAVY);
-                    if (NARROW && !h0) {
+                    if (NARROW == 2 && w0 >= 0 && (w0 & W_SLIM)) {
+                        const gptr_t c0s = scalar_row(nwk12_v, r0, row12_bytes);
+#pragma unroll
+                        for (int r = 0; r < RMAX; r++) { const int v = gather_slim(c0s, kslim[r]); if (a == 0) gn[r] = v; else gn2[r] = v; }
+                    } else if (NARROW && !h0) {
                         const gptr_t c0q = scalar_row(nwk16_v, r0, (unsigned int)K * 2u);
 #pragma unroll
-                        for (int r = 0; r < RMAX; r++) { const int v = gather_cell<uint16_t>(c0q + (unsigned int)koffh[r]); if (a == 0) gn[r] = v; else gn2[r] = v; }
+                        for (int r = 0; r < RMAX; r++) { const int v = gather_cell<uint16_t>(c0q + (NARROW == 2 ? (unsigned int)koff[r] >> 1 : (unsigned int)koffh[r])); if (a == 0) gn[r] = v; else gn2[r] = v; }
                     } else {
                         const gptr_t c0p = scalar_row(nwk_v, r0, (unsigned int)K * 4u);
 #pragma unroll
@@ -739,6 +758,7 @@
 #undef sn_get
 #undef sn_set
 
+#define MVHDP_SLIM_RMAX 4
 static bool roomy_build(int rmax, int K) { return rmax == 2 && K >= 512; }
 static bool two_batch_rows(int K) { return K > 512 && K <= 1024; }
 
@@ -750,7 +770,7 @@
 }
 
 template <int RMAX>
-static const void* fast_kernel_ptr(bool debug, bool walk, bool narrow, int K = 0, bool live_rows = false)
+static const void* fast_kernel_ptr(bool debug, bool walk, bool narrow, int K = 0, bool live_rows = false, bool slim = false)
 {
     if (live_rows && !debug) {
         if constexpr (RMAX == 2) { if (narrow && roomy_build(RMAX, K)) return (const void*)sweep_fast_kernel<2, false, true, true, true, 2>; }
@@ -758,6 +778,12 @@
         return narrow ? (const void*)sweep_fast_kernel<RMAX, false, true, true, false, 1> : (const void*)sweep_fast_kernel<RMAX, false, true, false, false, 1>;
     }
     if (narrow && walk && !debug) {
+        if constexpr (RMAX <= MVHDP_SLIM_RMAX) {
+            if (slim) {
+                if constexpr (RMAX == 2) { if (roomy_build(RMAX, K)) return (const void*)sweep_fast_kernel<2, false, true, 2, true>; }
+                return (const void*)sweep_fast_kernel<RMAX, false, true, 2>;
+            }
+        }
         if constexpr (RMAX == 2) { if (roomy_build(RMAX, K)) return (const void*)sweep_fast_kernel<2, false, true, true, true>; }
         return (const void*)sweep_fast_kernel<RMAX, false, true, true>;
     }
@@ -772,6 +798,8 @@
     dim3 block(64 * sl.waves_per_block);
     const bool narrow = sl.narrow && sl.walk && !debug;
     const bool rows = sl.live_rows && sl.walk && !debug;
+    const bool slim = narrow && sl.narrow == 2;
+    if (slim && (RMAX > MVHDP_SLIM_RMAX || rows || sl.live16 || mm.mix || !mm.counts12)) return hipErrorInvalidValue;
     if (mm.mix) {
         if (rows || !sl.walk) return hipErrorInvalidValue;
         if (lds > 65536) {
@@ -784,7 +812,7 @@
         return hipGetLastError();
     }
     if (lds > 65536) {
-        hipError_t e = hipFuncSetAttribute(fast_kernel_ptr<RMAX>(debug, sl.walk != 0, narrow, mm.K, rows), hipFuncAttributeMaxDynamicSharedMemorySize, (int)lds);
+        hipError_t e = hipFuncSetAttribute(fast_kernel_ptr<RMAX>(debug, sl.walk != 0, narrow, mm.K, rows, slim), hipFuncAttributeMaxDynamicSharedMemorySize, (int)lds);
         if (e != hipSuccess) return e;
     }
     if (debug)        hipLaunchKernelGGL((sweep_fast_kernel<RMAX, true, true, false>), dim3(grid_blocks), block, lds, s, mm, sl);
@@ -793,6 +821,12 @@
         else if (narrow && two_batch_rows(mm.K)) hipLaunchKernelGGL((sweep_fast_kernel<RMAX, false, true, true, false, 2>), dim3(grid_blocks), block, lds, s, mm, sl);
         else if (narrow) hipLaunchKernelGGL((sweep_fast_kernel<RMAX, false, true, true, false, 1>), dim3(grid_blocks), block, lds, s, mm, sl);
         else             hipLaunchKernelGGL((sweep_fast_kernel<RMAX, false, true, false, false, 1>), dim3(grid_blocks), block, lds, s, mm, sl);
+    }
+    else if (slim) {
+        if constexpr (RMAX <= MVHDP_SLIM_RMAX) {
+            if (roomy_build(RMAX, mm.K)) { if constexpr (RMAX == 2) hipLaunchKernelGGL((sweep_fast_kernel<2, false, true, 2, true>), dim3(grid_blocks), block, lds, s, mm, sl); }
+            else hipLaunchKernelGGL((sweep_fast_kernel<RMAX, false, true, 2>), dim3(grid_blocks), block, lds, s, mm, sl);
+        }
     }
     else if (narrow && roomy_build(RMAX, mm.K)) {
         if constexpr (RMAX == 2) hipLaunchKernelGGL((sweep_fast_kernel<2, false, true, true, true>), dim3(grid_blocks), block, lds, s, mm, sl);
diff --git a/mvtopicmodel_amd/csrc/mvhdp_sweep_fast_token.inc b/mvtopicmodel_amd/csrc/mvhdp_sweep_fast_token.inc
--- a/mvtopicmodel_amd/csrc/mvhdp_sweep_fast_token.inc
+++ b/mvtopicmodel_amd/csrc/mvhdp_sweep_fast_token.inc
@@ -13,17 +13,21 @@
                     if (LIVEROWS) {
 #pragma unroll
                         for (int r = 0; r < RMAX; r++) asm volatile("" : "+v"(g[r]));
-                        if (spec_t) rowq = row_batch_load<NARROW>(rowp_t, K, bsel_t, lane);
+                        if (spec_t) rowq = row_batch_load<(NARROW != 0)>(rowp_t, K, bsel_t, lane);
                     }
                     const unsigned long long rem_n = (NB == 2) ? (rem & (rem - 1)) : rem;
 #pragma unroll
-                    for (int r = 0; r < RMAX; r++) { touch_lane_off(koff[r]); if (NARROW) touch_lane_off(koffh[r]); }
+                    for (int r = 0; r < RMAX; r++) { touch_lane_off(koff[r]); if (NARROW == 1) touch_lane_off(koffh[r]); if (NARROW == 2) touch_lane_off(kslim[r]); }
                     if (NB == 2 || LIVEROWS || rem_n) {
                         const int wn = bcast_i(w_l, rem_n ? (int)__builtin_ctzll(rem_n) : TOK_T);
-                        if (NARROW && !(wn & W_HEAVY)) {
+                        if (NARROW == 2 && (wn & W_SLIM)) {
+                            const gptr_t cns = scalar_row(nwk12_v, (unsigned int)W_ROW(wn), row12_bytes);
+#pragma unroll
+                            for (int r = 0; r < RMAX; r++) TOK_G[r] = gather_slim(cns, kslim[r]);
+                        } else if (NARROW && !(wn & W_HEAVY)) {
                             const gptr_t cnq = scalar_row(nwk16_v, (unsigned int)W_ROW(wn), (unsigned int)K * 2u);
 #pragma unroll
-                            for (int r = 0; r < RMAX; r++) TOK_G[r] = gather_cell<uint16_t>(cnq + (unsigned int)koffh[r]);
+                            for (int r = 0; r < RMAX; r++) TOK_G[r] = gather_cell<uint16_t>(cnq + (NARROW == 2 ? (unsigned int)koff[r] >> 1 : (unsigned int)koffh[r]));
                         } else {
                             const gptr_t cnp = scalar_row(nwk_v, (unsigned int)W_ROW(wn), (unsigned int)K * 4u);
 #pragma unroll
@@ -35,7 +39,12 @@
                             for (int r = 0; r < RMAX; r++) TOK_MG[r] = gather_mix<mixg_t>(mnp + ((unsigned int)koff[r] << MIXSH));
                         }
                     }
-                    const int w = W_ROW(bcast_i(w_l, TOK_T));
+                    const int wcur = bcast_i(w_l, TOK_T);
+                    const int w = W_ROW(wcur);
+                    if (NARROW == 2 && (wcur & W_SLIM)) {
+#pragma unroll
+                        for (int r = 0; r < RMAX; r++) g[r] = slim_cell(g[r], kslim[r]);
+                    }
                     const int so = bcast_i(so_l, TOK_T);
                     const int64_t row = row0 + w;
 
@@ -283,7 +292,7 @@
 #endif
                             if (sl.flags & 0x2000u) znew = bcast_i(z_l, TOK_T);
                             else
-                            znew = uniform_i(row_sample_live<NARROW, LIVEROWS == 2>(rowq, spec_t, coef_s != nullptr, (const __attribute__((address_space(3))) float*)coef_s + m * Kp, mm.coef + (int64_t)m * Kp, smp_m, smS, rowp_t, K,
+                            znew = uniform_i(row_sample_live<(NARROW != 0), LIVEROWS == 2>(rowq, spec_t, coef_s != nullptr, (const __attribute__((address_space(3))) float*)coef_s + m * Kp, mm.coef + (int64_t)m * Kp, smp_m, smS, rowp_t, K,
                                                                      bcast_f(u2f_l, TOK_T), bcast_f(root32_l, TOK_T), bsel_t, (LIVEROWS == 2 && bsel_t) ? mm.mass0[row] : 0.0f , lane, &t_rs1));
                             if (znew < 0) znew = K - 1;
 #ifdef MVHDP_TIMING
diff --git a/mvtopicmodel_amd/native.py b/mvtopicmodel_amd/native.py
--- a/mvtopicmodel_amd/native.py
+++ b/mvtopicmodel_amd/native.py
@@ -33,6 +33,8 @@
 BUF_COUNTS = 0
 BUF_DELTA = 1
 BUF_BIRTH_KEYS = 2
+BUF_COUNTS12 = 3
+BUF_ROW_CLASS = 4
 ACT_KEY_NONE = (1 << 63) - 1
 
 
```

Measured after the change: 6.967 billion (median of 6 runs). +2.9%, better.
